# OpenMendel/MendelIHT.jl

Measured on NVIDIA B200. Metric: iht_iterations_per_sec, higher is better.
Workload: dtype f64 (sweep: f32 LUT partials per slab of 640 samples (512 without the ternary copy), f64 across slabs; top-k candidates re-scored in f64)

## Files before the change

### mendeliht.jl_b200/csrc/common.cuh

```cuda
#pragma once
#include <cuda_runtime.h>
#include <stdint.h>
#include <stdio.h>
#include <memory>
#include <string>
#include <vector>
#include <stdexcept>
#include "../../include/ihtb200.h"

namespace ihtb {

struct Error : std::runtime_error {
    int code;
    Error(int c, const std::string& m) : std::runtime_error(m), code(c) {}
};
void set_last_error(const std::string& m);
const std::string& last_error();
struct LaunchCounter {
    int64_t v = 0;
    LaunchCounter& operator++(int) { __atomic_fetch_add(&v, 1, __ATOMIC_RELAXED); return *this; }
    operator int64_t() const { return __atomic_load_n(&v, __ATOMIC_RELAXED); }
};
LaunchCounter& launch_counter();
bool debug_sync();

#define IHTB_CUDA(call)                                                                      \
    do {                                                                                     \
        cudaError_t e__ = (call);                                                            \
        if (e__ != cudaSuccess)                                                              \
            throw ::ihtb::Error(IHTB_ECUDA, std::string(#call) + ": " + cudaGetErrorString(e__)); \
    } while (0)

#define IHTB_CHECK(cond, code, msg)                                  \
    do {                                                             \
        if (!(cond)) throw ::ihtb::Error((code), (msg));             \
    } while (0)

#define IHTB_LAUNCH(kernel, grid, block, smem, stream, ...)          \
    do {                                                             \
        kernel<<<(grid), (block), (smem), (stream)>>>(__VA_ARGS__);  \
        ::ihtb::launch_counter()++;                                  \
        IHTB_CUDA(cudaGetLastError());                               \
        if (::ihtb::debug_sync()) {                                  \
            cudaError_t e2__ = cudaStreamSynchronize(stream);        \
            if (e2__ != cudaSuccess)                                 \
                throw ::ihtb::Error(IHTB_ECUDA, std::string("kernel " #kernel " failed: ") + cudaGetErrorString(e2__)); \
        }                                                            \
    } while (0)

template <typename F>
static inline int32_t guard(F&& f) {
    try {
        f();
        return IHTB_OK;
    } catch (const Error& e) {
        set_last_error(e.what());
        return e.code;
    } catch (const std::bad_alloc&) {
        set_last_error("out of host memory");
        return IHTB_ENOMEM;
    } catch (const std::exception& e) {
        set_last_error(e.what());
        return IHTB_EINVAL;
    }
}

template <typename T>
struct DBuf {
    T* p = nullptr;
    size_t n = 0;
    DBuf() = default;
    explicit DBuf(size_t count) { alloc(count); }
    DBuf(const DBuf&) = delete;
    DBuf& operator=(const DBuf&) = delete;
    ~DBuf() { release(); }
    void alloc(size_t count) {
        release();
        n = count;
        if (count) {
            cudaError_t e = cudaMalloc((void**)&p, count * sizeof(T));
            if (e != cudaSuccess) {
                p = nullptr; n = 0;
                throw Error(IHTB_ENOMEM, std::string("cudaMalloc of ") + std::to_string(count * sizeof(T)) +
                                             " bytes failed: " + cudaGetErrorString(e));
            }
        }
    }
    void release() {
        if (p) cudaFree(p);
        p = nullptr; n = 0;
    }
    void zero(cudaStream_t s) { if (n) IHTB_CUDA(cudaMemsetAsync(p, 0, n * sizeof(T), s)); }
};

template <typename T>
struct HBuf {
    T* p = nullptr;
    size_t n = 0;
    HBuf() = default;
    HBuf(const HBuf&) = delete;
    HBuf& operator=(const HBuf&) = delete;
    ~HBuf() { if (p) cudaFreeHost(p); }
    void alloc(size_t count) {
        if (p) cudaFreeHost(p);
        p = nullptr; n = count;
        if (count) IHTB_CUDA(cudaMallocHost((void**)&p, count * sizeof(T)));
    }
};

static inline int64_t ceil_div(int64_t a, int64_t b) { return (a + b - 1) / b; }

bool smem_attr_needed(const void* kernel, int device);
template <typename K>
static inline void ensure_dynamic_smem(K kernel, int bytes) {
    int dev = 0;
    IHTB_CUDA(cudaGetDevice(&dev));
    if (!smem_attr_needed(reinterpret_cast<const void*>(kernel), dev)) return;
    IHTB_CUDA(cudaFuncSetAttribute(kernel, cudaFuncAttributeMaxDynamicSharedMemorySize, bytes));
}

struct TopkFuse;
ihtb_geno* dense_new_handle(int64_t n, int64_t p, int dtype, int standardize, int32_t den = 0);
void dense_upload(ihtb_geno* g, const void* x, int64_t ld_host, int64_t j_dst, int64_t ncols);
void dense_finalize(ihtb_geno* g);
int64_t dense_stream_bytes(const ihtb_geno* g);
void dense_decode_block(const ihtb_geno* g, int64_t i0, int64_t i1, int64_t j0, int64_t j1, double* d_out);
void dense_xt_v(const ihtb_geno* g, const double* dV, int64_t m, double* dOut, cudaStream_t s, DBuf<double>* part,
                const TopkFuse* tf);
void dense_sweep_kernel_only(const ihtb_geno* g, const double* dV, DBuf<double>* part, cudaStream_t s);
void dense_x_support(const ihtb_geno* g, const int64_t* d_idx, int64_t k, const double* d_coef, int64_t m,
                     double* d_out, cudaStream_t s);
void dense_xt_gather2(const ihtb_geno* g, const int64_t* d_cols_a, int64_t n_a, const int64_t* d_cols_b, int64_t n_b,
                      const double* d_v, int64_t m, double* d_out, cudaStream_t s);
void dense_init_beta_moments(const ihtb_geno* g, const double* d_w, const double* d_wy, double* d_sx, double* d_sxx,
                             double* d_sxy, cudaStream_t s);
void dense_decode_cols(const ihtb_geno* g, const int64_t* d_cols, int64_t k, double* d_out, cudaStream_t s);
const double* geno_bound_scale(const ihtb_geno* g);
double geno_bound_coef(const ihtb_geno* g, double plink_coef);

}

enum { GENO_PLINK = 0, GENO_DENSE = 1 };

struct ihtb_geno {
    int kind = 0;
    int device = 0;
    int64_t n = 0;
    int64_t p = 0;
    int64_t j0 = 0;
    int64_t nbytes = 0;
    int64_t stride = 0;
    int64_t cs_j = 0, cs_s = 0;
    int quad = 0;
    int64_t p4 = 0;
    int center = 1, scale = 1, impute = 1;
    int sm_count = 148;
    ihtb::DBuf<uint8_t> bed;
    ihtb::DBuf<uint8_t> tern;
    int64_t tern_slabs = 0;
    ihtb::DBuf<double> mu, sinv;
    ihtb::DBuf<double> sgn;
    ihtb::DBuf<int32_t> nmiss;
    ihtb::DBuf<int64_t> miss_ptr;
    ihtb::DBuf<int32_t> miss_idx;
    int64_t total_missing = 0;
    bool ready = false;
    int dtype = 0;
    int standardize = 0;
    int32_t den = 0;
    int64_t ld = 0;
    ihtb::DBuf<uint8_t> dense;
    ihtb::DBuf<double> dscale;
    double dcoef = 0.0;
    std::shared_ptr<void> bgen_stage;
};
static inline bool geno_is_dense(const ihtb_geno* g) { return g->kind == GENO_DENSE; }

static inline void geno_require_ready(const ihtb_geno* g) {
    IHTB_CHECK(g && g->ready, IHTB_EINVAL, "genotype handle is not finalized (ihtb_geno_finalize)");
}

struct GenoView {
    const uint8_t* bed;
    int64_t cs_j, cs_s, nbytes, stride, n, p;
    int quad;
    const double* mu;
    const double* sinv;
    const int32_t* nmiss;
    int impute;
};
static inline GenoView geno_view(const ihtb_geno* g) {
    return GenoView{g->bed.p, g->cs_j, g->cs_s, g->nbytes, g->stride, g->n, g->p, g->quad, g->mu.p, g->sinv.p,
                    g->nmiss.p, g->impute};
}
__device__ __forceinline__ const uint8_t* gv_ptr(const GenoView& g, int64_t j, int64_t b) {
    if (g.quad)
        return g.bed + (b >> 7) * g.cs_s + (j >> 2) * 512 + ((b & 127) >> 2) * 16 + (j & 3) * 4 + (b & 3);
    return g.bed + j * g.cs_j + (b >> 7) * g.cs_s + (b & 127);
}

namespace ihtb {

__device__ __forceinline__ double warp_sum(double v) {
#pragma unroll
    for (int o = 16; o > 0; o >>= 1) v += __shfl_xor_sync(0xffffffffu, v, o);
    return v;
}
__device__ __forceinline__ float warp_sum(float v) {
#pragma unroll
    for (int o = 16; o > 0; o >>= 1) v += __shfl_xor_sync(0xffffffffu, v, o);
    return v;
}
__device__ __forceinline__ int warp_sum(int v) {
#pragma unroll
    for (int o = 16; o > 0; o >>= 1) v += __shfl_xor_sync(0xffffffffu, v, o);
    return v;
}

__device__ __forceinline__ double block_sum(double v, double* sh) {
    v = warp_sum(v);
    int lane = threadIdx.x & 31, w = threadIdx.x >> 5;
    __syncthreads();
    if (lane == 0) sh[w] = v;
    __syncthreads();
    int nw = (blockDim.x + 31) >> 5;
    v = (threadIdx.x < nw) ? sh[threadIdx.x] : 0.0;
    if (w == 0) v = warp_sum(v);
    return v;
}

void sweep_xt_v(const ihtb_geno* g, const double* dV, int64_t m, double* dOut, int mode, cudaStream_t s,
                double* sweep_seconds);
void x_support(const ihtb_geno* g, const int64_t* d_idx_local, int64_t k, const double* d_coef, int64_t m,
               double* d_out, cudaStream_t s);
void xt_gather(const ihtb_geno* g, const int64_t* d_cols_local, int64_t ncols, const double* d_v, int64_t m,
               const double* d_vsum , double* d_out , cudaStream_t s);
void xt_gather2(const ihtb_geno* g, const int64_t* d_cols_a, int64_t n_a, const int64_t* d_cols_b, int64_t n_b,
                const double* d_v, int64_t m, const double* d_vsum, double* d_out, cudaStream_t s, bool blocked = false);

struct TopkFuse;
void dense_xt_v(const ihtb_geno* g, const double* dV, int64_t m, double* dOut, cudaStream_t s, void* scratch_any,
                const TopkFuse* tf);
void dense_x_support(const ihtb_geno* g, const int64_t* d_idx, int64_t k, const double* d_coef, int64_t m,
                     double* d_out, cudaStream_t s);
void dense_xt_gather2(const ihtb_geno* g, const int64_t* d_cols_a, int64_t n_a, const int64_t* d_cols_b, int64_t n_b,
                      const double* d_v, int64_t m, double* d_out, cudaStream_t s);
void dense_init_beta_moments(const ihtb_geno* g, const double* d_w, const double* d_wy, double* d_sx, double* d_sxx,
                             double* d_sxy, cudaStream_t s, void* scratch_any);
void dense_decode_cols(const ihtb_geno* g, const int64_t* d_cols, int64_t k, double* d_out, cudaStream_t s);
const double* geno_bound_scale(const ihtb_geno* g);
double geno_bound_coef(const ihtb_geno* g, double plink_coef);

}
```

### mendeliht.jl_b200/csrc/fit.cu

```cuda
#include "glm.cuh"
#include "topk.cuh"
#include "comm.cuh"
#include "debias.cuh"
#include "groups.cuh"
#include "pairer.cuh"
#include <algorithm>
#include <chrono>
#include <cmath>
#include <memory>
#include <mutex>
#include <string.h>
#include <unordered_map>

namespace ihtb {
void sweep_xt_v_with_means(const ihtb_geno* g, const double* dV, const double* vbar_host, int64_t m, double* dOut,
                           int mode, cudaStream_t s, void* scratch_any, float* sweep_ms, double* d_l2 = nullptr,
                           const TopkFuse* tf = nullptr);
void* sweep_scratch_create();
void sweep_scratch_destroy(void* p);
void sweep_class_sums(const ihtb_geno* g, const double* d_v, double* d_w1, double* d_w2, double* d_wm, cudaStream_t s,
                      void* scratch_any);
}

using namespace ihtb;

static const double kFastBound = 1.0 / 262144.0;
static const double kExactBound = 1e-13;
static const double kPairBound = 3.1 / 2048.0;

struct ihtb_fit {
    const ihtb_geno* g = nullptr;
    int device = 0;
    int64_t n = 0, p = 0, q = 0;
    ihtb_comm* comm = nullptr;
    int64_t j0 = 0, p_global = 0;
    std::vector<int64_t> shard_j0;
    DBuf<int64_t> d_selall, d_pack, d_packall;
    HBuf<int64_t> h_selall, h_packall;
    int capx = 512;
    ihtb_cfg cfg{};
    cudaStream_t s = nullptr;
    std::vector<uint8_t> zkeep;
    int zkeepn = 0;
    int cap = 4096;

    DBuf<unsigned> d_done;
    DBuf<double> d_y, d_z, d_w, d_xb, d_zc, d_mu, d_r, d_xs, d_dfa, d_part, d_scal, d_small, d_coef, d_gout,
        d_vbar;
    DBuf<uint8_t> d_mask;
    DBuf<uint32_t> d_keyL, d_keyU;
    DBuf<int> d_hist;
    DBuf<int64_t> d_sel;
    DBuf<int64_t> d_idx, d_cols;
    HBuf<double> h_scal, h_gout;
    HBuf<int64_t> h_sel;
    void* sweep_scratch = nullptr;
    cudaEvent_t ev0 = nullptr, ev1 = nullptr, tm0 = nullptr, tm1 = nullptr;
    bool sweep_pending = false;
    struct FusedStep {
        std::vector<int64_t> uni_loc;
        size_t maxsupp = 0;
        int M = 0;
        int winner = -1;
    };
    FusedStep* fz = nullptr;
    DBuf<double> d_pick;
    HBuf<double> h_pick;
    SweepPairer* pairer = nullptr;
    int pair_slot = 0;
    double sweep_coef = kFastBound;
    GlmCtx glm{};
    TopkCtx tk{};

    std::vector<int64_t> idx, idx0, best_idx;
    std::vector<double> b, b0, best_b;
    std::vector<double> c, c0, best_c, df2, h_y, h_mu;
    std::vector<uint8_t> idc, idc0;
    std::unordered_map<int64_t, double> df_exact;
    std::vector<double> wt;
    DBuf<double> d_wt;
    double w_at(int64_t j) const { return wt.empty() ? 1.0 : wt[(size_t)j]; }
    void set_weights(const double* w) {
        if (!w) { wt.clear(); tk.wt = nullptr; return; }
        for (int64_t j = 0; j < p_global; ++j)
            IHTB_CHECK(w[j] > 0.0 && std::isfinite(w[j]), IHTB_EDOMAIN, "weights must be positive and finite");
        wt.assign(w, w + p_global);
        if (d_wt.n < (size_t)p) d_wt.alloc((size_t)p);
        IHTB_CUDA(cudaMemcpyAsync(d_wt.p, wt.data() + j0, (size_t)p * sizeof(double), cudaMemcpyHostToDevice, s));
        sync();
        tk.wt = d_wt.p;
    }
    std::vector<int64_t> cand_cache;
    bool df_sparse = false;
    std::vector<int64_t> dfs_idx;
    std::vector<double> dfs_val;
    double rbar = 0.0, bound = 0.0, sum_w = 0.0, sum_wy = 0.0, last_dev = 0.0, denom_next = 0.0;
    bool denom_ready = false;
    bool inited = false;

    int64_t n_sweeps = 0, n_backtracks = 0, n_cand_iter = 0, n_pair_overflow = 0;
    int last_count = 0;
    double sweep_ms_total = 0.0;
    double pve = 0.0;

    ~ihtb_fit() {
        if (sweep_scratch) sweep_scratch_destroy(sweep_scratch);
        if (ev0) cudaEventDestroy(ev0);
        if (ev1) cudaEventDestroy(ev1);
        if (tm0) cudaEventDestroy(tm0);
        if (tm1) cudaEventDestroy(tm1);
        if (s) cudaStreamDestroy(s);
    }

    void sync() { IHTB_CUDA(cudaStreamSynchronize(s)); }
    void readback_scal(int nv) {
        IHTB_CUDA(cudaMemcpyAsync(h_scal.p, d_scal.p, nv * sizeof(double), cudaMemcpyDeviceToHost, s));
        sync();
    }
    template <typename T>
    void upload(T* dst, const T* src, size_t count) {
        if (count) IHTB_CUDA(cudaMemcpyAsync(dst, src, count * sizeof(T), cudaMemcpyHostToDevice, s));
    }

    bool is_local(int64_t j) const { return j >= j0 && j < j0 + p; }
    int nranks() const { return comm ? comm->nranks : 1; }

    void support_matvec(const std::vector<int64_t>& cols, const std::vector<double>& coef, double* d_out) {
        std::vector<int64_t> ii; std::vector<double> vv;
        for (size_t t = 0; t < cols.size(); ++t)
            if (coef[t] != 0.0 && is_local(cols[t])) { ii.push_back(cols[t] - j0); vv.push_back(coef[t]); }
        if (!ii.empty()) {
            upload(d_idx.p, ii.data(), ii.size());
            upload(d_coef.p, vv.data(), vv.size());
        }
        support_matvec_dev(ii.empty() ? nullptr : d_idx.p, (int64_t)ii.size(), d_coef.p, d_out);
    }

    void support_matvec_dev(const int64_t* d_idx_loc, int64_t k_loc, const double* d_coef_loc, double* d_out) {
        support_matvec_dev_m(d_idx_loc, k_loc, d_coef_loc, 1, d_out);
    }
    void support_matvec_dev_m(const int64_t* d_idx_loc, int64_t k_loc, const double* d_coef_loc, int m, double* d_out) {
        const size_t cnt = (size_t)n * (size_t)m;
        if (!comm) {
            if (k_loc > 0) x_support(g, d_idx_loc, k_loc, d_coef_loc, m, d_out, s);
            else IHTB_CUDA(cudaMemsetAsync(d_out, 0, cnt * sizeof(double), s));
            return;
        }
        if (m == 1 && p2p_pushall_ok(comm, cnt)) {
            if (k_loc > 0) x_support_push(g, d_idx_loc, k_loc, d_coef_loc, comm, s);
            else p2p_push(comm, nullptr, cnt, s);
            p2p_reduce(comm, d_out, cnt, s);
            return;
        }
        if (p2p_mapped(comm) && cnt <= comm->red_cap) {
            double* part = p2p_partial_ptr(comm);
            if (k_loc > 0) x_support(g, d_idx_loc, k_loc, d_coef_loc, m, part, s);
            else IHTB_CUDA(cudaMemsetAsync(part, 0, cnt * sizeof(double), s));
            p2p_allreduce_2phase(comm, cnt, d_out, s);
            return;
        }
        if (k_loc > 0) x_support(g, d_idx_loc, k_loc, d_coef_loc, m, d_out, s);
        else IHTB_CUDA(cudaMemsetAsync(d_out, 0, cnt * sizeof(double), s));
        comm_allreduce_sum_f64(comm, d_out, cnt, s);
    }

    void update_xb() { support_matvec(idx, b, d_xb.p); }

    double glm_update(int add_zc) {
        upload(d_small.p, c.data(), (size_t)q);
        glm_mu(glm, d_small.p, add_zc, s);
        readback_scal(3);
        double dev = h_scal.p[0], lp = h_scal.p[1], sw = h_scal.p[2];
        last_dev = dev;
        if (cfg.dist == IHTB_NORMAL) {
            double phi = dev / (double)n;
            double sigma = std::sqrt(phi);
            return -0.5 * (dev / phi) - sw * (0.5 * std::log(2.0 * M_PI) + std::log(sigma));
        }
        return lp;
    }

    static double digamma(double x) {
        double r = 0.0;
        while (x < 6.0) { r -= 1.0 / x; x += 1.0; }
        double f = 1.0 / (x * x);
        return r + std::log(x) - 0.5 / x -
               f * (1.0 / 12 - f * (1.0 / 120 - f * (1.0 / 252 - f * (1.0 / 240 - f * (1.0 / 132)))));
    }
    static double trigamma(double x) {
        double r = 0.0;
        while (x < 6.0) { r += 1.0 / (x * x); x += 1.0; }
        double f = 1.0 / (x * x);
        return r + 1.0 / x + f / 2 + f / x * (1.0 / 6 - f * (1.0 / 30 - f * (1.0 / 42 - f * (1.0 / 30))));
    }
    void fetch_mu() {
        h_mu.resize((size_t)n);
        IHTB_CUDA(cudaMemcpyAsync(h_mu.data(), d_mu.p, n * sizeof(double), cudaMemcpyDeviceToHost, s));
        sync();
    }
    double nb_logl(double r) {
        glm.nb_r = r;
        return glm_update(1);
    }
    void mle_for_r() {
        fetch_mu();
        const std::vector<double>& y = h_y;
        double r = glm.nb_r;
        if (cfg.est_r == 1) {
            double num = 0.0, den = 0.0;
            for (int64_t i = 0; i < n; ++i) {
                for (int64_t j = 0; j <= (int64_t)y[i] - 1; ++j) num += r / (r + (double)j);
                den += std::log(r / (r + h_mu[i]));
            }
            glm.nb_r = -num / den;
            return;
        }
        auto d1 = [&](double rr) {
            double a = 0.0;
            for (int64_t i = 0; i < n; ++i)
                a += -(y[i] + rr) / (h_mu[i] + rr) - std::log(h_mu[i] + rr) + 1.0 + std::log(rr) + digamma(rr + y[i]) -
                     digamma(rr);
            return a;
        };
        auto d2 = [&](double rr) {
            double a = 0.0;
            for (int64_t i = 0; i < n; ++i)
                a += (y[i] + rr) / ((h_mu[i] + rr) * (h_mu[i] + rr)) - 2.0 / (h_mu[i] + rr) + 1.0 / rr +
                     trigamma(rr + y[i]) - trigamma(rr);
            return a;
        };
        double new_r = 1.0, stepsize = 1.0;
        for (int it = 0; it < 100; ++it) {
            double dx = d1(r), dx2 = d2(r);
            double increment = dx2 < 0 ? dx / dx2 : dx;
            new_r = r - stepsize * increment;
            double old_logl = nb_logl(r);
            for (int j = 0; j < 20; ++j) {
                if (new_r <= 0) {
                    stepsize /= 2; new_r = r - stepsize * increment;
                } else {
                    double new_logl = nb_logl(new_r);
                    if (old_logl >= new_logl) { stepsize /= 2; new_r = r - stepsize * increment; }
                    else break;
                }
            }
            if (std::fabs(r - new_r) <= 1e-6) { glm.nb_r = new_r; return; }
            r = new_r;
        }
        glm.nb_r = r;
    }
    double mu_r_logl() {
        double l = glm_update(1);
        if (cfg.est_r != 0) {
            mle_for_r();
            l = glm_update(1);
        }
        return l;
    }

    void exact_df(const std::vector<int64_t>& cols, bool exchange = true) {
        std::vector<int64_t> need;
        for (int64_t j : cols)
            if (!df_exact.count(j) && (exchange || is_local(j))) need.push_back(j);
        if (need.empty()) { if (!exchange) sync(); return; }
        IHTB_CHECK((int64_t)need.size() <= (int64_t)d_cols.n, IHTB_ENUMERIC, "too many columns to re-score");
        std::vector<int64_t> loc(need.size());
        for (size_t t = 0; t < need.size(); ++t) loc[t] = is_local(need[t]) ? need[t] - j0 : -1;
        upload(d_cols.p, loc.data(), loc.size());
        xt_gather2(g, d_cols.p, (int64_t)need.size(), nullptr, 0, d_r.p, 1, d_vbar.p, d_gout.p, s,
                   false);
        if (exchange) comm_allreduce_sum_f64(comm, d_gout.p, need.size(), s);
        IHTB_CUDA(cudaMemcpyAsync(h_gout.p, d_gout.p, need.size() * sizeof(double), cudaMemcpyDeviceToHost, s));
        sync();
        for (size_t t = 0; t < need.size(); ++t) df_exact[need[t]] = h_gout.p[t];
        n_cand_iter += (int64_t)need.size();
    }

    void score_and_sweep() {
        glm_score(glm, s, d_vbar.p);
        IHTB_CUDA(cudaMemcpyAsync(h_scal.p, d_scal.p, (2 + q) * sizeof(double), cudaMemcpyDeviceToHost, s));
        IHTB_CUDA(cudaEventRecord(ev0, s));
        sweep_coef = geno_bound_coef(g, cfg.sweep_mode == IHTB_SWEEP_FAST ? kFastBound : kExactBound);
        const double t_sw = now();
        if (pairer && cfg.sweep_mode == IHTB_SWEEP_FAST) {
            IHTB_CHECK(!grouped() && !comm, IHTB_EUNSUPPORTED, "paired sweeps serve plain single-device fits only");
            if (pairer->sweep(pair_slot, g, d_r.p, d_vbar.p, d_dfa.p, s, sweep_scratch)) {
                sweep_coef = kPairBound;
                IHTB_CUDA(cudaMemcpyAsync(h_scal.p + 3 + q, pairer->d_l2 + pair_slot, sizeof(double), cudaMemcpyDeviceToHost, s));
            }
        } else if (cfg.k > 0 && !(grouped() && !init_plain)) {
            const TopkFuse tf = topk_absdf_fuse_begin(tk, geno_bound_scale(g), d_scal.p, sweep_coef);
            sweep_xt_v_with_means(g, d_r.p, d_vbar.p, 1, d_dfa.p, cfg.sweep_mode, s, sweep_scratch, nullptr, nullptr, &tf);
        } else {
            sweep_xt_v_with_means(g, d_r.p, d_vbar.p, 1, d_dfa.p, cfg.sweep_mode, s, sweep_scratch, nullptr);
        }
        IHTB_CUDA(cudaEventRecord(ev1, s));
        ++n_sweeps;
        const double t_sel = now();
        dbg[0] += t_sel - t_sw;
        select_rescore(false);
        dbg[1] += now() - t_sel;
    }

    void select_rescore(bool rerun) {
        if (grouped() && !init_plain) {
            select_groups(rerun);
            if (!rerun) finish_sweep_scalars(sweep_coef);
            return;
        }
        df_exact.clear(); cand_cache.clear();
        df_sparse = false;
        const double coef = sweep_coef;
        std::vector<std::pair<int64_t, double>> cvals;
        const bool fused = fz != nullptr && !rerun;
        std::vector<int64_t> supp_loc;
        if (fused) supp_loc = fz->uni_loc;
        else
            for (int64_t j : idx)
                if (is_local(j)) supp_loc.push_back(j - j0);
        const int nsupp = (int)supp_loc.size();
        const int64_t* d_supp = fused ? d_idx.p : d_cols.p;
        int glaunch = 0;
        if (cfg.k > 0) {
            const int64_t ksel = cfg.k + (int64_t)(fused ? fz->maxsupp : idx.size());
            const bool paired = coef == kPairBound;
            if (tk.fused_hist) topk_candidates_absdf_finish(tk, ksel, s);
            else
                topk_candidates_absdf(tk, d_dfa.p, paired ? g->sgn.p : geno_bound_scale(g), rerun ? nullptr : d_scal.p, coef, ksel, s,
                                      bound, (paired && !rerun) ? pairer->d_l2 + pair_slot : nullptr);
            const int64_t want = sweep_coef == kPairBound ? std::max<int64_t>(ksel + 1024, last_count + last_count / 4 + 256)
                                                          : ksel + 64;
            glaunch = (int)std::min<int64_t>(comm ? capx / 2 : cap, want);
        }
        if (nsupp && !fused) upload(d_cols.p, supp_loc.data(), supp_loc.size());
        xt_gather2(g, tk.cand, glaunch, d_supp, nsupp, d_r.p, 1, d_vbar.p, d_gout.p, s);
        denom_ready = false;
        if (!rerun) {
            if (fused) {
                glm_winner_coef(d_pick.p, d_coefM.p, nsupp, d_gout.p + glaunch, d_coef.p, d_cM.p, q, d_small.p + q, s);
                support_matvec_dev(d_supp, nsupp, d_coef.p, d_xs.p);
                IHTB_CUDA(cudaMemcpyAsync(h_pick.p, d_pick.p, (size_t)(1 + fz->M) * sizeof(double), cudaMemcpyDeviceToHost, s));
                IHTB_CUDA(cudaMemcpyAsync(h_scalM.p, d_scalM.p, (size_t)(3 * fz->M) * sizeof(double), cudaMemcpyDeviceToHost, s));
            } else {
                support_matvec_dev(d_supp, nsupp, d_gout.p + glaunch, d_xs.p);
                std::vector<double> mask((size_t)q);
                for (int64_t l = 0; l < q; ++l) mask[l] = idc[l] ? 1.0 : 0.0;
                upload(d_small.p + q, mask.data(), (size_t)q);
            }
            glm_stepsize(glm, d_scal.p + 2, d_xs.p, s, d_small.p + q, d_scal.p + 2 + q);
            IHTB_CUDA(cudaMemcpyAsync(h_scal.p + 2 + q, d_scal.p + 2 + q, sizeof(double), cudaMemcpyDeviceToHost, s));
            denom_ready = true;
        }
        if (!comm) {
            IHTB_CUDA(cudaMemcpyAsync(h_sel.p, d_sel.p, (2 + glaunch) * sizeof(int64_t), cudaMemcpyDeviceToHost, s));
            IHTB_CUDA(cudaMemcpyAsync(h_gout.p, d_gout.p, (glaunch + nsupp) * sizeof(double), cudaMemcpyDeviceToHost, s));
            sync();
            const double t_host = now();
            struct Acc { double& a; double t0; ~Acc() { a += now() - t0; } } acc_host{dbg[2], t_host};
            if (fused) adopt_winner();
            const TopkState* st = reinterpret_cast<const TopkState*>(h_sel.p);
            const int count = cfg.k > 0 ? st->count : 0;
            dbg[3] += (double)std::min(count, glaunch);
            if (count > cap && coef == kPairBound && !rerun) {
                ++n_pair_overflow;
                sweep_coef = kFastBound;
                sweep_xt_v_with_means(g, d_r.p, d_vbar.p, 1, d_dfa.p, IHTB_SWEEP_FAST, s, sweep_scratch, nullptr);
                IHTB_CUDA(cudaEventRecord(ev1, s));
                select_rescore(false);
                return;
            }
            IHTB_CHECK(count <= cap, IHTB_ENUMERIC,
                       "degenerate projection: more than " + std::to_string(cap) +
                           " entries lie within the sweep error bound of the k-th largest |gradient|");
            last_count = count;
            cvals.reserve((size_t)count);
            for (int t = 0; t < std::min(count, glaunch); ++t) cvals.push_back({h_sel.p[2 + t], h_gout.p[t]});
            for (int t = 0; t < nsupp; ++t) df_exact[supp_loc[t] + j0] = h_gout.p[glaunch + t];
            if (count > glaunch) {
                IHTB_CUDA(cudaMemcpyAsync(h_sel.p, d_sel.p, (2 + count) * sizeof(int64_t), cudaMemcpyDeviceToHost, s));
                sync();
                std::vector<int64_t> rest(h_sel.p + 2 + glaunch, h_sel.p + 2 + count);
                exact_df(rest);
                for (int64_t j : rest) cvals.push_back({j, df_exact.at(j)});
            }
        } else {
            const int nr = nranks();
            const size_t blk = 2 + 2 * (size_t)capx;
            IHTB_CHECK(nsupp <= capx / 2, IHTB_ENUMERIC, "support too large for the sharded candidate exchange");
            pack_sweep_candidates(d_pack.p, reinterpret_cast<const TopkState*>(d_sel.p), tk.cand, glaunch, d_gout.p,
                                  d_supp, nsupp, d_gout.p + glaunch, j0, capx, s);
            comm_allgather_i64(comm, d_pack.p, d_packall.p, blk, s);
            IHTB_CUDA(cudaMemcpyAsync(h_packall.p, d_packall.p, nr * blk * sizeof(int64_t), cudaMemcpyDeviceToHost, s));
            sync();
            if (fused) adopt_winner();
            for (int r = 0; r < nr; ++r) {
                const int64_t* b_ = h_packall.p + (size_t)r * blk;
                IHTB_CHECK(b_[0] <= glaunch, IHTB_ENUMERIC,
                           "degenerate projection: too many local candidates within the sweep error bound");
                const int half = capx / 2;
                auto take = [&](int t, bool is_cand) {
                    const int64_t j = b_[2 + t];
                    if (j < 0) return;
                    double v;
                    memcpy(&v, &b_[2 + capx + t], sizeof(double));
                    if (is_cand) cvals.push_back({j, v});
                    else df_exact[j] = v;
                };
                for (int t = 0; t < (int)b_[0]; ++t) take(t, true);
                for (int t = 0; t < (int)b_[1]; ++t) take(half + t, false);
            }
        }
        std::sort(cvals.begin(), cvals.end());
        cvals.erase(std::unique(cvals.begin(), cvals.end(), [](const std::pair<int64_t, double>& x, const std::pair<int64_t, double>& y) {
                        return x.first == y.first; }), cvals.end());
        n_cand_iter += (int64_t)cvals.size();
        std::vector<char> keep(cvals.size(), 1);
        if ((int64_t)cvals.size() > cfg.k) {
            std::vector<std::pair<double, size_t>> outside;
            outside.reserve(cvals.size());
            for (size_t t = 0; t < cvals.size(); ++t)
                if (!std::binary_search(idx.begin(), idx.end(), cvals[t].first))
                    outside.push_back({std::fabs(cvals[t].second) * w_at(cvals[t].first), t});
            if ((int64_t)outside.size() > cfg.k) {
                std::nth_element(outside.begin(), outside.begin() + (cfg.k - 1), outside.end(),
                                 [](const std::pair<double, size_t>& x, const std::pair<double, size_t>& y) {
                                     return x.first > y.first;
                                 });
                const double thr = outside[(size_t)cfg.k - 1].first * (1.0 - 1e-12);
                std::fill(keep.begin(), keep.end(), 0);
                for (const auto& e : outside)
                    if (e.first >= thr) keep[e.second] = 1;
            }
        }
        for (size_t t = 0; t < cvals.size(); ++t)
            if (keep[t]) {
                cand_cache.push_back(cvals[t].first);
                df_exact[cvals[t].first] = cvals[t].second;
            }
        if (rerun) return;
        finish_sweep_scalars(coef);
    }

    void finish_sweep_scalars(double coef) {
        float ms = 0.f;
        IHTB_CUDA(cudaEventElapsedTime(&ms, ev0, ev1));
        sweep_ms_total += ms;
        double rsum = h_scal.p[0], rl1 = h_scal.p[1];
        for (int64_t l = 0; l < q; ++l) df2[l] = h_scal.p[2 + l];
        denom_next = h_scal.p[2 + q];
        rbar = rsum / (double)n;
        bound = coef == kPairBound ? coef * h_scal.p[3 + q]
                                   : coef * (rl1 + std::fabs(rsum));
    }

    double df_at(int64_t j) const {
        if (df_sparse) {
            auto it = std::lower_bound(dfs_idx.begin(), dfs_idx.end(), j);
            return (it != dfs_idx.end() && *it == j) ? dfs_val[it - dfs_idx.begin()] : 0.0;
        }
        return df_exact.at(j);
    }

    double stepsize() {
        std::vector<double> coef(idx.size());
        double numer = 0.0;
        for (size_t t = 0; t < idx.size(); ++t) { coef[t] = df_at(idx[t]); numer += coef[t] * coef[t]; }
        if (denom_ready && !df_sparse) {
            denom_ready = false;
            for (int64_t l = 0; l < q; ++l)
                if (idc[l]) numer += df2[l] * df2[l];
            double eta = numer / denom_next;
            if (std::isinf(eta) || std::isnan(eta)) eta = 1e-8;
            return eta;
        }
        denom_ready = false;
        support_matvec(idx, coef, d_xs.p);
        std::vector<double> d2((size_t)q);
        for (int64_t l = 0; l < q; ++l) {
            d2[l] = idc[l] ? df2[l] : 0.0;
            if (idc[l]) numer += df2[l] * df2[l];
        }
        upload(d_small.p + q, d2.data(), (size_t)q);
        glm_stepsize(glm, d_small.p + q, d_xs.p, s);
        readback_scal(1);
        double denom = h_scal.p[0];
        double eta = numer / denom;
        if (std::isinf(eta) || std::isnan(eta)) eta = 1e-8;
        return eta;
    }

    static double b_lookup(const std::vector<int64_t>& ii, const std::vector<double>& vv, int64_t j) {
        auto it = std::lower_bound(ii.begin(), ii.end(), j);
        return (it != ii.end() && *it == j) ? vv[it - ii.begin()] : 0.0;
    }

    void gradstep(double eta) {
        if (grouped()) { gradstep_group(eta); return; }
        std::vector<int64_t> cand;
        cand = df_sparse ? dfs_idx : cand_cache;
        cand.insert(cand.end(), idx0.begin(), idx0.end());
        std::sort(cand.begin(), cand.end());
        cand.erase(std::unique(cand.begin(), cand.end()), cand.end());

        struct Item { double a; int64_t pos; double v; };
        std::vector<Item> items;
        items.reserve(cand.size() + (size_t)q);
        for (int64_t j : cand) {
            double v = b_lookup(idx0, b0, j) + eta * df_at(j);
            if (!wt.empty()) {
                const double w = wt[(size_t)j], a = v * w;
                items.push_back({std::fabs(a), j, a / w});
            } else {
                items.push_back({std::fabs(v), j, v});
            }
        }
        for (int64_t l = 0; l < q; ++l) {
            c[l] = c0[l] + eta * df2[l];
            if (!zkeep[l]) items.push_back({std::fabs(c[l]), p_global + l, c[l]});
        }
        int64_t k = cfg.k;
        std::sort(items.begin(), items.end(), [](const Item& x, const Item& y) {
            return x.a > y.a || (x.a == y.a && x.pos < y.pos);
        });
        idx.clear(); b.clear();
        const double thr = project_threshold(items, k);
        std::vector<std::pair<int64_t, double>> keep;
        for (size_t t = 0; t < items.size(); ++t) {
            const bool kept = items[t].a >= thr;
            if (items[t].pos >= p_global) {
                if (!kept) c[items[t].pos - p_global] = 0.0;
            } else if (kept && items[t].v != 0.0) {
                keep.push_back({items[t].pos, items[t].v});
            }
        }
        for (int64_t l = 0; l < q; ++l) idc[l] = c[l] != 0.0;
        choose_prune(keep);
        std::sort(keep.begin(), keep.end());
        for (auto& kv : keep) { idx.push_back(kv.first); b.push_back(kv.second); }
    }

    template <typename ItemT>
    static double project_threshold(const std::vector<ItemT>& sorted_items, int64_t k) {
        if (k <= 0) return INFINITY;
        return (int64_t)sorted_items.size() >= k ? sorted_items[(size_t)k - 1].a : 0.0;
    }
    void choose_prune(std::vector<std::pair<int64_t, double>>& keep) const {
        int64_t nonzero = (int64_t)keep.size() - zkeepn;
        for (int64_t l = 0; l < q; ++l) nonzero += idc[l] ? 1 : 0;
        const int64_t limit = cfg.k + zkeepn;
        if (nonzero <= limit) return;
        std::vector<std::pair<int64_t, double>> byabs = keep;
        std::sort(byabs.begin(), byabs.end(), [](const std::pair<int64_t, double>& x, const std::pair<int64_t, double>& y) {
            return std::fabs(x.second) < std::fabs(y.second) || (std::fabs(x.second) == std::fabs(y.second) && x.first > y.first);
        });
        const size_t excess = std::min<size_t>((size_t)(nonzero - limit), byabs.size());
        for (size_t t = 0; t < excess; ++t) keep.erase(std::find(keep.begin(), keep.end(), byabs[t]));
    }

    std::unique_ptr<GroupCtx> grpctx;
    bool init_plain = false;
    bool grouped() const { return (bool)grpctx; }
    void set_groups(const int32_t* group1, int J, const int64_t* ks, int64_t n_groups) {
        if (!group1) { grpctx.reset(); return; }
        IHTB_CHECK(J >= 0, IHTB_EINVAL, "Value of J (max number of groups) must be nonnegative!");
        std::unique_ptr<GroupCtx> gc(new GroupCtx());
        std::vector<double> h_sinv((size_t)p);
        IHTB_CUDA(cudaMemcpy(h_sinv.data(), geno_bound_scale(g), (size_t)p * sizeof(double), cudaMemcpyDeviceToHost));
        gc->build(p, j0, p_global, group1, J, ks, n_groups, cfg.k, h_sinv.data());
        grpctx = std::move(gc);
    }

    void select_groups(bool rerun) {
        GroupCtx& gc = *grpctx;
        df_exact.clear(); cand_cache.clear();
        df_sparse = false; denom_ready = false;
        const double coef = sweep_coef;
        group_topk(gc, d_dfa.p, geno_bound_scale(g), rerun ? nullptr : d_scal.p, coef, bound, cfg.k, s);
        const size_t G = (size_t)gc.G, nT = 2 * G + 1;
        const int nr = nranks();
        std::vector<double> TL(G), TU(G);
        bool overflow = false;
        if (comm) {
            if (gc.d_Tall.n < nT * (size_t)nr) { gc.d_Tall.alloc(nT * (size_t)nr); gc.h_Tall.alloc(nT * (size_t)nr); }
            comm_allgather_i64(comm, reinterpret_cast<const int64_t*>(gc.d_gT.p), gc.d_Tall.p, nT, s);
            IHTB_CUDA(cudaMemcpyAsync(gc.h_Tall.p, gc.d_Tall.p, nT * (size_t)nr * sizeof(int64_t), cudaMemcpyDeviceToHost, s));
            sync();
            std::fill(TL.begin(), TL.end(), 0.0); std::fill(TU.begin(), TU.end(), 0.0);
            for (int rk = 0; rk < nr; ++rk) {
                const double* T = reinterpret_cast<const double*>(gc.h_Tall.p) + (size_t)rk * nT;
                for (size_t gi = 0; gi < G; ++gi) { TL[gi] = std::max(TL[gi], T[gi]); TU[gi] += T[G + gi]; }
                overflow = overflow || T[2 * G] != 0.0;
            }
        } else {
            IHTB_CUDA(cudaMemcpyAsync(gc.h_gT.p, gc.d_gT.p, nT * sizeof(double), cudaMemcpyDeviceToHost, s));
            sync();
            for (size_t gi = 0; gi < G; ++gi) { TL[gi] = gc.h_gT.p[gi]; TU[gi] = gc.h_gT.p[G + gi]; }
            overflow = gc.h_gT.p[2 * G] != 0.0;
        }
        IHTB_CHECK(!overflow, IHTB_ENUMERIC,
                   "degenerate group projection: too many entries of one group lie within the sweep error bound of its "
                   "2k-th largest |gradient|");
        std::vector<char> has(G, 0);
        for (int64_t j : idx) has[(size_t)gc.grp[(size_t)j]] = 1;
        std::vector<int32_t> chosen;
        std::vector<double> lows;
        for (size_t gi = 0; gi < G; ++gi) {
            if (has[gi]) chosen.push_back((int32_t)gi);
            else lows.push_back(TL[gi]);
        }
        if (gc.J > 0 && !lows.empty()) {
            const size_t need = std::min<size_t>((size_t)gc.J, lows.size());
            std::nth_element(lows.begin(), lows.begin() + (need - 1), lows.end(), std::greater<double>());
            const double thr = lows[need - 1];
            for (size_t gi = 0; gi < G; ++gi)
                if (!has[gi] && TU[gi] >= thr) chosen.push_back((int32_t)gi);
        }
        IHTB_CHECK(chosen.size() <= 65536, IHTB_ENUMERIC, "degenerate group projection: too many groups tie at the J-th norm");
        std::sort(chosen.begin(), chosen.end());
        const int nc = (int)chosen.size();
        const int64_t nsupp = (int64_t)idx.size();
        const int64_t list_slots = (int64_t)nc * gc.lcap, slots = list_slots + nsupp;
        if (slots == 0) return;
        gc.ensure_chosen(std::max(nc, 1));
        if (gc.d_oidx.n < (size_t)slots) {
            gc.d_oidx.alloc((size_t)slots); gc.d_oval.alloc((size_t)slots);
            gc.h_oidx.alloc((size_t)slots); gc.h_oval.alloc((size_t)slots);
        }
        if (nc) {
            IHTB_CUDA(cudaMemcpyAsync(gc.d_chosen.p, chosen.data(), (size_t)nc * sizeof(int32_t), cudaMemcpyHostToDevice, s));
            group_take(gc, nc, s);
        }
        std::vector<int64_t> supp_loc((size_t)nsupp);
        for (int64_t t = 0; t < nsupp; ++t) supp_loc[(size_t)t] = is_local(idx[(size_t)t]) ? idx[(size_t)t] - j0 : -1;
        upload(gc.d_oidx.p + list_slots, supp_loc.data(), (size_t)nsupp);
        xt_gather(g, gc.d_oidx.p, slots, d_r.p, 1, d_vbar.p, gc.d_oval.p, s);
        auto take = [&](int64_t t, int64_t j, double v) {
            if (j < 0) return;
            df_exact[j] = v;
            if (t < list_slots) cand_cache.push_back(j);
        };
        if (comm) {
            const size_t blk = 2 * (size_t)slots;
            if (gc.d_blk.n < blk) gc.d_blk.alloc(blk);
            if (gc.d_blkall.n < blk * (size_t)nr) { gc.d_blkall.alloc(blk * (size_t)nr); gc.h_blkall.alloc(blk * (size_t)nr); }
            group_pack(gc.d_oidx.p, gc.d_oval.p, slots, j0, gc.d_blk.p, s);
            comm_allgather_i64(comm, gc.d_blk.p, gc.d_blkall.p, blk, s);
            IHTB_CUDA(cudaMemcpyAsync(gc.h_blkall.p, gc.d_blkall.p, blk * (size_t)nr * sizeof(int64_t), cudaMemcpyDeviceToHost, s));
            sync();
            for (int rk = 0; rk < nr; ++rk) {
                const int64_t* b_ = gc.h_blkall.p + (size_t)rk * blk;
                for (int64_t t = 0; t < slots; ++t) {
                    double v;
                    memcpy(&v, &b_[slots + t], sizeof(double));
                    take(t, b_[t], v);
                }
            }
        } else {
            IHTB_CUDA(cudaMemcpyAsync(gc.h_oidx.p, gc.d_oidx.p, (size_t)slots * sizeof(int64_t), cudaMemcpyDeviceToHost, s));
            IHTB_CUDA(cudaMemcpyAsync(gc.h_oval.p, gc.d_oval.p, (size_t)slots * sizeof(double), cudaMemcpyDeviceToHost, s));
            sync();
            for (int64_t t = 0; t < slots; ++t) take(t, gc.h_oidx.p[t], gc.h_oval.p[t]);
        }
        std::sort(cand_cache.begin(), cand_cache.end());
        cand_cache.erase(std::unique(cand_cache.begin(), cand_cache.end()), cand_cache.end());
        n_cand_iter += (int64_t)cand_cache.size();
    }

    struct GItem { double a; int64_t j; double v; int g; };
    std::vector<std::pair<int64_t, double>> project_groups(std::vector<GItem>& items) const {
// ... 846 lines not shown
```

### mendeliht.jl_b200/csrc/lut_common.cuh

```cuda
#pragma once
#include "common.cuh"
#include <cuda_fp16.h>

namespace ihtb {

constexpr int LUT_TABLE_BYTES = 131072;

__device__ __forceinline__ uint32_t smem_u32(const void* p) { return (uint32_t)__cvta_generic_to_shared(p); }
__device__ __forceinline__ void mbar_init(uint32_t bar, uint32_t count) {
    asm volatile("mbarrier.init.shared::cta.b64 [%0], %1;" ::"r"(bar), "r"(count));
}
__device__ __forceinline__ void mbar_arrive(uint32_t bar) {
    asm volatile("mbarrier.arrive.shared::cta.b64 _, [%0];" ::"r"(bar) : "memory");
}
__device__ __forceinline__ void mbar_expect_tx(uint32_t bar, uint32_t bytes) {
    asm volatile("mbarrier.arrive.expect_tx.shared::cta.b64 _, [%0], %1;" ::"r"(bar), "r"(bytes) : "memory");
}
__device__ __forceinline__ void mbar_wait(uint32_t bar, uint32_t parity) {
    asm volatile(
        "{\n\t.reg .pred p;\n"
        "W_%=:\n\t"
        "mbarrier.try_wait.parity.shared::cta.b64 p, [%0], %1;\n\t"
        "@!p bra W_%=;\n\t}"
        ::"r"(bar), "r"(parity) : "memory");
}
__device__ __forceinline__ void bulk_g2s(uint32_t dst, const void* src, uint32_t bytes, uint32_t bar) {
    asm volatile("cp.async.bulk.shared::cluster.global.mbarrier::complete_tx::bytes [%0], [%1], %2, [%3];"
                 ::"r"(dst), "l"(src), "r"(bytes), "r"(bar) : "memory");
}
__device__ __forceinline__ float lds_f32(uint32_t addr) {
    float v;
    asm volatile("ld.shared.f32 %0, [%1];" : "=f"(v) : "r"(addr));
    return v;
}
__device__ __forceinline__ uint32_t lds_u32(uint32_t addr) {
    uint32_t v;
    asm volatile("ld.shared.u32 %0, [%1];" : "=r"(v) : "r"(addr));
    return v;
}
__device__ __forceinline__ uint4 lds_u128(uint32_t addr) {
    uint4 v;
    asm volatile("ld.shared.v4.u32 {%0, %1, %2, %3}, [%4];" : "=r"(v.x), "=r"(v.y), "=r"(v.z), "=r"(v.w) : "r"(addr));
    return v;
}
template <uint32_t SEL>
__device__ __forceinline__ uint32_t prmt(uint32_t a, uint32_t b) {
    uint32_t d;
    asm("prmt.b32 %0, %1, %2, %3;" : "=r"(d) : "r"(a), "r"(b), "n"(SEL));
    return d;
}
__device__ __forceinline__ void sts_u32(uint32_t addr, uint32_t v) {
    asm volatile("st.shared.u32 [%0], %1;" ::"r"(addr), "r"(v) : "memory");
}
__device__ __forceinline__ void sts_f32(uint32_t addr, float v) {
    asm volatile("st.shared.f32 [%0], %1;" ::"r"(addr), "f"(v) : "memory");
}
template <int NT>
__device__ __forceinline__ void consumer_bar() {
    asm volatile("bar.sync 1, %0;" ::"n"(NT) : "memory");
}

template <int NT>
__device__ __forceinline__ void lut_build(uint32_t tab, const double* __restrict__ v, double vbar, int64_t n,
                                          int64_t slab, int tid) {
    constexpr int PARTS = NT / 128;
    constexpr int V3_PER = 4 / PARTS;
    const int group = tid & 127, part = tid >> 7;
    const int t = group >> 5, w = group & 31;
    float u[4];
#pragma unroll
    for (int s = 0; s < 4; ++s) {
        int64_t i = slab * 512 + 16 * w + 4 * t + s;
        u[s] = (i < n) ? __double2float_rn(__dsub_rn(v[i], vbar)) : 0.0f;
    }
    auto f = [&](int s, int code) -> float { return code == 2 ? u[s] : (code == 3 ? u[s] + u[s] : 0.0f); };
    const uint32_t rowbase = tab + (uint32_t)(t >> 1) * 65536u + (uint32_t)(t & 1) * 128u + 4u * (uint32_t)w;
#pragma unroll
    for (int c3 = 0; c3 < V3_PER; ++c3) {
        const int v3 = part * V3_PER + c3;
        const float a3 = (v3 == 2) ? u[3] : ((v3 == 3) ? u[3] + u[3] : 0.0f);
        const uint32_t base3 = rowbase + (uint32_t)v3 * (64u * 256u);
#pragma unroll
        for (int v2 = 0; v2 < 4; ++v2) {
            const float a2 = a3 + f(2, v2);
#pragma unroll
            for (int v1 = 0; v1 < 4; ++v1) {
                const float a1 = a2 + f(1, v1);
#pragma unroll
                for (int v0 = 0; v0 < 4; ++v0)
                    sts_f32(base3 + (uint32_t)(v2 << 4 | v1 << 2 | v0) * 256u, a1 + f(0, v0));
            }
        }
    }
}

template <int NT>
__device__ __forceinline__ void lut_build_tern(uint32_t tab, const double* __restrict__ v, double vbar, int64_t n,
                                               int64_t slab, int tid) {
    static_assert(NT == 512, "ternary tables are built by 512 threads");
    const int group = tid & 127, d4 = tid >> 7;
    if (d4 > 2) return;
    const int t = group >> 5, w = group & 31;
    float u[5];
#pragma unroll
    for (int s = 0; s < 5; ++s) {
        int64_t i = slab * 640 + 20 * w + 5 * t + s;
        u[s] = (i < n) ? __double2float_rn(__dsub_rn(v[i], vbar)) : 0.0f;
    }
    auto f = [&](int s, int d) -> float { return d == 1 ? u[s] : (d == 2 ? u[s] + u[s] : 0.0f); };
    const uint32_t rowbase = tab + (uint32_t)(t >> 1) * 65536u + (uint32_t)(t & 1) * 128u + 4u * (uint32_t)w;
    const float a4 = (d4 == 1) ? u[4] : ((d4 == 2) ? u[4] + u[4] : 0.0f);
    const uint32_t base4 = rowbase + (uint32_t)d4 * (81u * 256u);
#pragma unroll
    for (int d3 = 0; d3 < 3; ++d3) {
        const float a3 = a4 + f(3, d3);
#pragma unroll
        for (int d2 = 0; d2 < 3; ++d2) {
            const float a2 = a3 + f(2, d2);
#pragma unroll
            for (int d1 = 0; d1 < 3; ++d1) {
                const float a1 = a2 + f(1, d1);
#pragma unroll
                for (int d0 = 0; d0 < 3; ++d0)
                    sts_f32(base4 + (uint32_t)(27 * d3 + 9 * d2 + 3 * d1 + d0) * 256u, a1 + f(0, d0));
            }
        }
    }
}

__device__ __forceinline__ void lut_build_h2_tern(uint32_t tab, const double* __restrict__ v0, const double* __restrict__ v1,
                                                  double vbar0, double vbar1, float sc0, float sc1, int64_t n, int64_t slab,
                                                  int tid) {
    const int group = tid & 127, d4 = tid >> 7;
    if (d4 > 2) return;
    const int t = group >> 5, w = group & 31;
    float a[5], b[5];
#pragma unroll
    for (int s = 0; s < 5; ++s) {
        int64_t i = slab * 640 + 20 * w + 5 * t + s;
        const float x0 = (i < n) ? __double2float_rn(__dsub_rn(v0[i], vbar0)) * sc0 : 0.0f;
        const float x1 = (i < n) ? __double2float_rn(__dsub_rn(v1[i], vbar1)) * sc1 : 0.0f;
        a[s] = (w & 16) ? x1 : x0;
        b[s] = (w & 16) ? x0 : x1;
    }
    auto fa = [&](int s, int d) -> float { return d == 1 ? a[s] : (d == 2 ? a[s] + a[s] : 0.0f); };
    auto fb = [&](int s, int d) -> float { return d == 1 ? b[s] : (d == 2 ? b[s] + b[s] : 0.0f); };
    const uint32_t rowbase = tab + (uint32_t)(t >> 1) * 65536u + (uint32_t)(t & 1) * 128u + 4u * (uint32_t)w;
    const float a4 = fa(4, d4), b4 = fb(4, d4);
    const uint32_t base4 = rowbase + (uint32_t)d4 * (81u * 256u);
#pragma unroll
    for (int d3 = 0; d3 < 3; ++d3) {
        const float a3 = a4 + fa(3, d3), b3 = b4 + fb(3, d3);
#pragma unroll
        for (int d2 = 0; d2 < 3; ++d2) {
            const float a2 = a3 + fa(2, d2), b2 = b3 + fb(2, d2);
#pragma unroll
            for (int d1 = 0; d1 < 3; ++d1) {
                const float a1 = a2 + fa(1, d1), b1 = b2 + fb(1, d1);
#pragma unroll
                for (int d0 = 0; d0 < 3; ++d0) {
                    const __half2 h = __floats2half2_rn(a1 + fa(0, d0), b1 + fb(0, d0));
                    sts_u32(base4 + (uint32_t)(27 * d3 + 9 * d2 + 3 * d1 + d0) * 256u, *reinterpret_cast<const uint32_t*>(&h));
                }
            }
        }
    }
}

__device__ __forceinline__ void lut_build_h2(uint32_t tab, const double* __restrict__ v0, const double* __restrict__ v1,
                                             double vbar0, double vbar1, float sc0, float sc1, int64_t n, int64_t slab,
                                             int tid) {
    const int group = tid & 127, part = tid >> 7;
    const int t = group >> 5, w = group & 31;
    float a[4], b[4];
#pragma unroll
    for (int s = 0; s < 4; ++s) {
        int64_t i = slab * 512 + 16 * w + 4 * t + s;
        a[s] = (i < n) ? __double2float_rn(__dsub_rn(v0[i], vbar0)) * sc0 : 0.0f;
        b[s] = (i < n) ? __double2float_rn(__dsub_rn(v1[i], vbar1)) * sc1 : 0.0f;
    }
    auto fa = [&](int s, int code) -> float { return code == 2 ? a[s] : (code == 3 ? a[s] + a[s] : 0.0f); };
    auto fb = [&](int s, int code) -> float { return code == 2 ? b[s] : (code == 3 ? b[s] + b[s] : 0.0f); };
    const uint32_t rowbase = tab + (uint32_t)(t >> 1) * 65536u + (uint32_t)(t & 1) * 128u + 4u * (uint32_t)w;
    const int v3 = part;
    const float a3 = fa(3, v3), b3 = fb(3, v3);
    const uint32_t base3 = rowbase + (uint32_t)v3 * (64u * 256u);
#pragma unroll
    for (int v2 = 0; v2 < 4; ++v2) {
        const float a2 = a3 + fa(2, v2), b2 = b3 + fb(2, v2);
#pragma unroll
        for (int v1c = 0; v1c < 4; ++v1c) {
            const float a1 = a2 + fa(1, v1c), b1 = b2 + fb(1, v1c);
#pragma unroll
            for (int v0c = 0; v0c < 4; ++v0c) {
                const __half2 h = __floats2half2_rn(a1 + fa(0, v0c), b1 + fb(0, v0c));
                sts_u32(base3 + (uint32_t)(v2 << 4 | v1c << 2 | v0c) * 256u, *reinterpret_cast<const uint32_t*>(&h));
            }
        }
    }
}

}
```

### mendeliht.jl_b200/csrc/mvfit.cu

```cuda
#include "glm.cuh"
#include "topk.cuh"
#include "comm.cuh"
#include <algorithm>
#include <chrono>
#include <cmath>
#include <map>
#include <memory>

namespace ihtb {
void sweep_xt_v_with_means(const ihtb_geno* g, const double* dV, const double* vbar_host, int64_t m, double* dOut,
                           int mode, cudaStream_t s, void* scratch_any, float* sweep_ms, double* d_l2 = nullptr,
                           const TopkFuse* tf = nullptr);
void* sweep_scratch_create();
void sweep_scratch_destroy(void* p);
void sweep_class_sums(const ihtb_geno* g, const double* d_v, double* d_w1, double* d_w2, double* d_wm, cudaStream_t s,
                      void* scratch_any);

constexpr int MV_MAXR = 20;
constexpr int MV_THREADS = 256;
static inline int mv_grid(int64_t n) {
    int64_t b = ceil_div(n, MV_THREADS);
    return (int)(b < 1 ? 1 : (b > GLM_MAX_BLOCKS ? GLM_MAX_BLOCKS : b));
}
struct MvSmall { double a[MV_MAXR * MV_MAXR]; };

__global__ void __launch_bounds__(MV_THREADS)
k_mv_resid_gram(int64_t n, int r, int64_t q, const double* __restrict__ BX, const double* __restrict__ Z,
                const double* __restrict__ C , const double* __restrict__ Y,
                const double* __restrict__ w, double* __restrict__ mu, double* __restrict__ resid,
                double* __restrict__ part) {
    __shared__ double sh[32];
    double g[MV_MAXR * (MV_MAXR + 1) / 2];
    const int ng = r * (r + 1) / 2;
    for (int e = 0; e < ng; ++e) g[e] = 0.0;
    double sw = 0.0;
    for (int64_t i = blockIdx.x * (int64_t)blockDim.x + threadIdx.x; i < n; i += (int64_t)gridDim.x * blockDim.x) {
        double rs[MV_MAXR];
        const double wi = w[i];
        for (int t = 0; t < r; ++t) {
            double cz = 0.0;
            for (int64_t l = 0; l < q; ++l) cz += C[t * q + l] * Z[i + l * n];
            double m = BX[i + (int64_t)t * n] + cz;
            mu[i + (int64_t)t * n] = m;
            rs[t] = (Y[i + (int64_t)t * n] - m) * wi;
            resid[i + (int64_t)t * n] = rs[t];
        }
        int e = 0;
        for (int a = 0; a < r; ++a)
            for (int b = a; b < r; ++b) g[e++] += rs[a] * rs[b];
        sw += wi;
    }
    const int nv = ng + 1;
    for (int e = 0; e < ng; ++e) {
        double v = block_sum(g[e], sh);
        if (threadIdx.x == 0) part[blockIdx.x * nv + e] = v;
    }
    double v = block_sum(sw, sh);
    if (threadIdx.x == 0) part[blockIdx.x * nv + ng] = v;
}

__global__ void __launch_bounds__(MV_THREADS)
k_mv_score(int64_t n, int r, int64_t q, const double* __restrict__ resid, MvSmall G, const double* __restrict__ Z,
           double* __restrict__ R1, double* __restrict__ part) {
    __shared__ double sh[32];
    double s1[MV_MAXR], sa[MV_MAXR];
    for (int t = 0; t < r; ++t) { s1[t] = 0.0; sa[t] = 0.0; }
    for (int64_t i = blockIdx.x * (int64_t)blockDim.x + threadIdx.x; i < n; i += (int64_t)gridDim.x * blockDim.x) {
        double rs[MV_MAXR];
        for (int t = 0; t < r; ++t) rs[t] = resid[i + (int64_t)t * n];
        for (int t = 0; t < r; ++t) {
            double v = 0.0;
            for (int u = 0; u < r; ++u) v += G.a[t * r + u] * rs[u];
            R1[i + (int64_t)t * n] = v;
            s1[t] += v; sa[t] += fabs(v);
        }
    }
    const int nv = 2 * r + r * (int)q;
    for (int t = 0; t < r; ++t) {
        double v = block_sum(s1[t], sh);
        if (threadIdx.x == 0) part[blockIdx.x * nv + t] = v;
        v = block_sum(sa[t], sh);
        if (threadIdx.x == 0) part[blockIdx.x * nv + r + t] = v;
    }
    for (int t = 0; t < r; ++t)
        for (int64_t l = 0; l < q; ++l) {
            double a = 0.0;
            for (int64_t i = blockIdx.x * (int64_t)blockDim.x + threadIdx.x; i < n; i += (int64_t)gridDim.x * blockDim.x)
                a += R1[i + (int64_t)t * n] * Z[i + l * n];
            a = block_sum(a, sh);
            if (threadIdx.x == 0) part[blockIdx.x * nv + 2 * r + t * (int)q + (int)l] = a;
        }
}

__global__ void __launch_bounds__(MV_THREADS)
k_mv_stepsize(int64_t n, int r, const double* __restrict__ V, const double* __restrict__ w, MvSmall U,
              double* __restrict__ part) {
    __shared__ double sh[32];
    double a = 0.0;
    for (int64_t i = blockIdx.x * (int64_t)blockDim.x + threadIdx.x; i < n; i += (int64_t)gridDim.x * blockDim.x) {
        double v[MV_MAXR];
        const double wi = w[i];
        for (int t = 0; t < r; ++t) v[t] = V[i + (int64_t)t * n] * wi;
        for (int t = 0; t < r; ++t) {
            double s = 0.0;
            for (int u = 0; u < r; ++u) s += U.a[t * r + u] * v[u];
            a += s * s;
        }
    }
    a = block_sum(a, sh);
    if (threadIdx.x == 0) part[blockIdx.x] = a;
}

__global__ void __launch_bounds__(MV_THREADS)
k_mv_moments(int64_t n, int r, const double* __restrict__ mu, const double* __restrict__ Y, MvSmall means, int pass,
             double* __restrict__ part) {
    __shared__ double sh[32];
    for (int t = 0; t < r; ++t) {
        double a = 0.0, b = 0.0;
        for (int64_t i = blockIdx.x * (int64_t)blockDim.x + threadIdx.x; i < n; i += (int64_t)gridDim.x * blockDim.x) {
            double m = mu[i + (int64_t)t * n], y = Y[i + (int64_t)t * n];
            if (pass == 0) { a += m; b += y; }
            else { double dm = m - means.a[t], dy = y - means.a[r + t]; a += dm * dm; b += dy * dy; }
        }
        a = block_sum(a, sh); b = block_sum(b, sh);
        if (threadIdx.x == 0) { part[blockIdx.x * 2 * r + t] = a; part[blockIdx.x * 2 * r + r + t] = b; }
    }
}

__global__ void k_mv_finalize(const double* __restrict__ part, int nblocks, int nv, double* __restrict__ out) {
    int v = (blockIdx.x * blockDim.x + threadIdx.x) >> 5;
    int lane = threadIdx.x & 31;
    if (v >= nv) return;
    double a = 0.0;
    for (int b = lane; b < nblocks; b += 32) a += part[b * nv + v];
    a = warp_sum(a);
    if (lane == 0) out[v] = a;
}
__global__ void k_mv_means(const double* __restrict__ scal, int r, int64_t n, double* __restrict__ out) {
    int t = threadIdx.x;
    if (t < r) out[t] = scal[t] / (double)n;
}
__global__ void k_mv_weights(int64_t n, const uint8_t* __restrict__ mask, double* __restrict__ w) {
    int64_t i = blockIdx.x * (int64_t)blockDim.x + threadIdx.x;
    if (i < n) w[i] = (mask == nullptr || mask[i]) ? 1.0 : 0.0;
}

static bool chol_lower(int r, const double* a, double* l) {
    std::fill(l, l + r * r, 0.0);
    for (int j = 0; j < r; ++j) {
        double d = a[j * r + j];
        for (int k = 0; k < j; ++k) d -= l[j * r + k] * l[j * r + k];
        if (!(d > 0.0)) return false;
        l[j * r + j] = std::sqrt(d);
        for (int i = j + 1; i < r; ++i) {
            double s = a[i * r + j];
            for (int k = 0; k < j; ++k) s -= l[i * r + k] * l[j * r + k];
            l[i * r + j] = s / l[j * r + j];
        }
    }
    return true;
}
static void spd_inverse(int r, const double* l, double* inv) {
    std::vector<double> li((size_t)r * r, 0.0);
    for (int i = 0; i < r; ++i) {
        li[i * r + i] = 1.0 / l[i * r + i];
        for (int j = 0; j < i; ++j) {
            double s = 0.0;
            for (int k = j; k < i; ++k) s -= l[i * r + k] * li[k * r + j];
            li[i * r + j] = s / l[i * r + i];
        }
    }
    for (int i = 0; i < r; ++i)
        for (int j = 0; j < r; ++j) {
            double s = 0.0;
            for (int k = std::max(i, j); k < r; ++k) s += li[k * r + i] * li[k * r + j];
            inv[i * r + j] = s;
        }
}
static bool pivoted_chol_upper(int r, const double* a_in, double* u) {
    std::vector<double> s(a_in, a_in + r * r);
    for (int i = 0; i < r; ++i)
        for (int j = 0; j < i; ++j) s[i * r + j] = s[j * r + i];
    std::fill(u, u + r * r, 0.0);
    for (int j = 0; j < r; ++j) {
        int pvt = j;
        for (int i = j + 1; i < r; ++i)
            if (s[i * r + i] > s[pvt * r + pvt]) pvt = i;
        if (pvt != j) {
            for (int c = 0; c < r; ++c) std::swap(s[j * r + c], s[pvt * r + c]);
            for (int c = 0; c < r; ++c) std::swap(s[c * r + j], s[c * r + pvt]);
            for (int c = 0; c < r; ++c) std::swap(u[c * r + j], u[c * r + pvt]);
        }
        double ajj = s[j * r + j];
        if (!(ajj > 0.0)) return false;
        ajj = std::sqrt(ajj);
        u[j * r + j] = ajj;
        for (int c = j + 1; c < r; ++c) u[j * r + c] = s[j * r + c] / ajj;
        for (int a = j + 1; a < r; ++a)
            for (int b = j + 1; b < r; ++b) s[a * r + b] -= u[j * r + a] * u[j * r + b];
    }
    return true;
}

}

using namespace ihtb;

static const double kFastBoundMv = 1.0 / 262144.0;
static const double kExactBoundMv = 1e-13;
static const double kPairBoundMv = 3.1 / 2048.0;
static const double kFastL2BoundMv = 1.0 / 1048576.0;

struct ihtb_mvfit {
    const ihtb_geno* g = nullptr;
    int device = 0;
    int64_t n = 0, p = 0, q = 0;
    int r = 0;
    ihtb_comm* comm = nullptr;
    int64_t j0 = 0, p_global = 0;
    DBuf<int64_t> d_xch, d_xchall;
    HBuf<int64_t> h_xchall;
    bool is_local(int64_t j) const { return j >= j0 && j < j0 + p; }
    ihtb_cfg cfg{};
    cudaStream_t s = nullptr;
    int cap = 4096;
    DBuf<double> d_Y, d_Z, d_w, d_BX, d_mu, d_resid, d_R1, d_V, d_dfa, d_b0d, d_part, d_scal, d_C, d_coef, d_gout,
        d_vbar, d_sval, d_bounds, d_sinvrep;
    DBuf<uint8_t> d_mask;
    DBuf<uint32_t> d_keyL, d_keyU;
    DBuf<int> d_hist;
    DBuf<int64_t> d_sel, d_idx, d_cols, d_sidx;
    HBuf<double> h_scal, h_gout, h_l2;
    DBuf<double> d_l2;
    HBuf<int64_t> h_sel;
    void* sweep_scratch = nullptr;
    cudaEvent_t ev0 = nullptr, ev1 = nullptr;
    TopkCtx tk{};

    std::map<int64_t, double> B, B0, bestB;
    std::vector<double> C, C0, bestC, df2;
    std::vector<double> Gamma, Gamma0;
    std::map<int64_t, std::vector<double>> df_exact;
    std::map<int64_t, double> dfs;
    bool df_sparse = false, inited = false;
    std::vector<double> bounds;
    std::vector<int64_t> b0d_pos;
    double n_train = 0.0;
    std::vector<double> pve;
    int64_t n_sweeps = 0, n_backtracks = 0, n_cand_iter = 0;
    double sweep_ms_total = 0.0;

    ~ihtb_mvfit() {
        if (sweep_scratch) sweep_scratch_destroy(sweep_scratch);
        if (ev0) cudaEventDestroy(ev0);
        if (ev1) cudaEventDestroy(ev1);
        if (s) cudaStreamDestroy(s);
    }
    void sync() { IHTB_CUDA(cudaStreamSynchronize(s)); }
    template <typename T>
    void upload(T* dst, const T* src, size_t count) {
        if (count) IHTB_CUDA(cudaMemcpyAsync(dst, src, count * sizeof(T), cudaMemcpyHostToDevice, s));
    }
    void finalize(int grid, int nv) {
        IHTB_LAUNCH(k_mv_finalize, (unsigned)ceil_div(nv, 4), 128, 0, s, d_part.p, grid, nv, d_scal.p);
    }
    void readback(int nv) {
        IHTB_CUDA(cudaMemcpyAsync(h_scal.p, d_scal.p, nv * sizeof(double), cudaMemcpyDeviceToHost, s));
        sync();
    }
    double phase_s[8] = {0, 0, 0, 0, 0, 0, 0, 0};
    template <typename F>
    auto timed(int ph, F&& fn) {
        auto t0 = std::chrono::steady_clock::now();
        struct Stop {
            double& acc; std::chrono::steady_clock::time_point t0;
            ~Stop() { acc += std::chrono::duration<double>(std::chrono::steady_clock::now() - t0).count(); }
        } stop{phase_s[ph], t0};
        return fn();
    }
    static std::vector<int64_t> support_cols(const std::map<int64_t, double>& M, int r) {
        std::vector<int64_t> cols;
        for (auto& kv : M)
            if (kv.second != 0.0 && (cols.empty() || cols.back() != kv.first / r)) cols.push_back(kv.first / r);
        return cols;
    }
    MvSmall small(const std::vector<double>& m) const {
        MvSmall o;
        std::fill(o.a, o.a + MV_MAXR * MV_MAXR, 0.0);
        std::copy(m.begin(), m.end(), o.a);
        return o;
    }

    void support_matmat(const std::vector<int64_t>& cols, const std::vector<double>& coef ,
                        double* d_out) {
        std::vector<int64_t> loc; std::vector<size_t> src;
        for (size_t c = 0; c < cols.size(); ++c)
            if (is_local(cols[c])) { loc.push_back(cols[c] - j0); src.push_back(c); }
        if (loc.empty()) {
            IHTB_CUDA(cudaMemsetAsync(d_out, 0, n * r * sizeof(double), s));
        } else {
            std::vector<double> cl(loc.size() * (size_t)r);
            for (int t = 0; t < r; ++t)
                for (size_t c = 0; c < loc.size(); ++c) cl[c + (size_t)t * loc.size()] = coef[src[c] + (size_t)t * cols.size()];
            upload(d_idx.p, loc.data(), loc.size());
            upload(d_coef.p, cl.data(), cl.size());
            x_support(g, d_idx.p, (int64_t)loc.size(), d_coef.p, r, d_out, s);
        }
        if (comm) comm_allreduce_sum_f64(comm, d_out, (size_t)(n * r), s);
    }
    void update_xb() {
        std::vector<int64_t> cols = support_cols(B, r);
        std::vector<double> coef(cols.size() * r, 0.0);
        for (size_t c = 0; c < cols.size(); ++c)
            for (int t = 0; t < r; ++t) {
                auto it = B.find(cols[c] * r + t);
                if (it != B.end()) coef[c + (size_t)t * cols.size()] = it->second;
            }
        support_matmat(cols, coef, d_BX.p);
    }
    std::vector<double> resid_gram() {
        upload(d_C.p, C.data(), C.size());
        int grid = mv_grid(n);
        int ng = r * (r + 1) / 2;
        IHTB_LAUNCH(k_mv_resid_gram, grid, MV_THREADS, 0, s, n, r, q, d_BX.p, d_Z.p, d_C.p, d_Y.p, d_w.p, d_mu.p,
                    d_resid.p, d_part.p);
        finalize(grid, ng + 1);
        readback(ng + 1);
        std::vector<double> G((size_t)r * r);
        int e = 0;
        for (int a = 0; a < r; ++a)
            for (int b = a; b < r; ++b) { G[a * r + b] = h_scal.p[e]; G[b * r + a] = h_scal.p[e]; ++e; }
        n_train = h_scal.p[ng];
        return G;
    }
    double solve_sigma_and_logl() {
        std::vector<double> G = resid_gram();
        std::vector<double> S((size_t)r * r), L((size_t)r * r);
        for (int e = 0; e < r * r; ++e) S[e] = G[e] / n_train;
        if (!chol_lower(r, S.data(), L.data())) return NAN;
        spd_inverse(r, L.data(), Gamma.data());
        double logdet = 0.0;
        for (int i = 0; i < r; ++i) logdet -= 2.0 * std::log(L[i * r + i]);
        double tr = 0.0;
        for (int i = 0; i < r; ++i)
            for (int j = 0; j < r; ++j) tr += Gamma[i * r + j] * G[j * r + i];
        return n_train / 2.0 * logdet - 0.5 * tr;
    }
    void exact_df(const std::vector<int64_t>& cols) {
        std::vector<int64_t> need;
        for (int64_t j : cols)
            if (!df_exact.count(j)) need.push_back(j);
        if (need.empty()) return;
        IHTB_CHECK(need.size() * r <= d_gout.n && need.size() <= d_cols.n, IHTB_ENUMERIC, "too many columns to re-score");
        std::vector<int64_t> loc(need.size());
        for (size_t c = 0; c < need.size(); ++c) loc[c] = is_local(need[c]) ? need[c] - j0 : -1;
        upload(d_cols.p, loc.data(), loc.size());
        xt_gather(g, d_cols.p, (int64_t)need.size(), d_R1.p, r, d_vbar.p, d_gout.p, s);
        if (comm) comm_allreduce_sum_f64(comm, d_gout.p, need.size() * (size_t)r, s);
        IHTB_CUDA(cudaMemcpyAsync(h_gout.p, d_gout.p, need.size() * r * sizeof(double), cudaMemcpyDeviceToHost, s));
        sync();
        for (size_t c = 0; c < need.size(); ++c) {
            std::vector<double> v((size_t)r);
            for (int t = 0; t < r; ++t) v[t] = h_gout.p[c + (size_t)t * need.size()];
            df_exact[need[c]] = v;
        }
        n_cand_iter += (int64_t)need.size();
    }
    void score_and_sweep() {
        int grid = mv_grid(n);
        int nv = 2 * r + r * (int)q;
        IHTB_LAUNCH(k_mv_score, grid, MV_THREADS, 0, s, n, r, q, d_resid.p, small(Gamma), d_Z.p, d_R1.p, d_part.p);
        finalize(grid, nv);
        IHTB_LAUNCH(k_mv_means, 1, 32, 0, s, d_scal.p, r, n, d_vbar.p);
        IHTB_CUDA(cudaMemcpyAsync(h_scal.p, d_scal.p, nv * sizeof(double), cudaMemcpyDeviceToHost, s));
        IHTB_CUDA(cudaEventRecord(ev0, s));
        const bool l2mode = cfg.sweep_mode == IHTB_SWEEP_PAIR && g->cs_j == 128;
        if (l2mode && d_l2.n < (size_t)r) { d_l2.alloc((size_t)r); h_l2.alloc((size_t)r); }
        sweep_xt_v_with_means(g, d_R1.p, d_vbar.p, r, d_dfa.p, cfg.sweep_mode, s, sweep_scratch, nullptr,
                              l2mode ? d_l2.p : nullptr);
        IHTB_CUDA(cudaEventRecord(ev1, s));
        if (l2mode) IHTB_CUDA(cudaMemcpyAsync(h_l2.p, d_l2.p, (size_t)r * sizeof(double), cudaMemcpyDeviceToHost, s));
        n_sweeps += r;
        df_exact.clear();
        df_sparse = false;
        std::vector<int64_t> cols = support_cols(B, r);
        if (!cols.empty()) exact_df(cols); else sync();
        float ms = 0.f;
        IHTB_CUDA(cudaEventElapsedTime(&ms, ev0, ev1));
        sweep_ms_total += ms;
        for (int t = 0; t < r; ++t) {
            double mean = h_scal.p[t] / (double)n;
            double ul1 = h_scal.p[r + t] + (double)n * std::fabs(mean);
            if (l2mode) bounds[t] = (t < 2 * (r / 2) ? kPairBoundMv : kFastL2BoundMv) * h_l2.p[t];
            else bounds[t] = (cfg.sweep_mode == IHTB_SWEEP_EXACT ? kExactBoundMv : kFastBoundMv) * ul1;
        }
        for (int e = 0; e < r * (int)q; ++e) df2[e] = h_scal.p[2 * r + e];
    }
    double df_entry(int64_t pos) const {
        if (df_sparse) {
            auto it = dfs.find(pos);
            return it == dfs.end() ? 0.0 : it->second;
        }
        return df_exact.at(pos / r)[pos % r];
    }
    double stepsize() {
        std::vector<int64_t> cols = support_cols(B, r);
        if (df_sparse) cols = support_cols(dfs, r);
        std::vector<double> coef(cols.size() * r, 0.0);
        double numer = 0.0;
        for (size_t c = 0; c < cols.size(); ++c)
            for (int t = 0; t < r; ++t) {
                double v = df_entry(cols[c] * r + t);
                coef[c + (size_t)t * cols.size()] = v;
                numer += v * v;
            }
        support_matmat(cols, coef, d_V.p);
        std::vector<double> U((size_t)r * r);
        IHTB_CHECK(pivoted_chol_upper(r, Gamma.data(), U.data()), IHTB_ENUMERIC,
                   "RankDeficientException in the pivoted Cholesky of the precision matrix");
        Gamma = U;
        int grid = mv_grid(n);
        IHTB_LAUNCH(k_mv_stepsize, grid, MV_THREADS, 0, s, n, r, d_V.p, d_w.p, small(U), d_part.p);
        finalize(grid, 1);
        readback(1);
        double eta = numer / h_scal.p[0];
        if (std::isinf(eta) || std::isnan(eta)) eta = 1e-8;
        return eta;
    }
    void sync_b0d() {
        if (!b0d_pos.empty()) {
            upload(d_sidx.p, b0d_pos.data(), b0d_pos.size());
            scatter_dense(d_b0d.p, d_sidx.p, nullptr, (int64_t)b0d_pos.size(), 1, s);
        }
        b0d_pos.clear();
        std::vector<double> vals;
        for (auto& kv : B0)
            if (kv.second != 0.0 && is_local(kv.first / r)) {
                b0d_pos.push_back((kv.first % r) * p + (kv.first / r - j0));
                vals.push_back(kv.second);
            }
        if (!b0d_pos.empty()) {
            upload(d_sidx.p, b0d_pos.data(), b0d_pos.size());
            upload(d_sval.p, vals.data(), vals.size());
            scatter_dense(d_b0d.p, d_sidx.p, d_sval.p, (int64_t)b0d_pos.size(), 0, s);
        }
    }
    std::vector<int64_t> device_candidate_cols(double eta) {
        std::vector<int64_t> cols = timed(5, [&] { return local_candidate_cols(eta); });
        if (!comm) return cols;
        return timed(6, [&] { return exchange_candidate_cols(cols); });
    }
    std::vector<int64_t> local_candidate_cols(double eta) {
        upload(d_bounds.p, bounds.data(), (size_t)r);
        topk_candidates_blocked(tk, d_dfa.p, d_b0d.p,
                                (cfg.sweep_mode == IHTB_SWEEP_PAIR && g->cs_j == 128) ? g->sgn.p : g->sinv.p, p,
                                d_bounds.p, eta, cfg.k, s);
        IHTB_CUDA(cudaMemcpyAsync(h_sel.p, d_sel.p, (2 + cap) * sizeof(int64_t), cudaMemcpyDeviceToHost, s));
        sync();
        const TopkState* st = reinterpret_cast<const TopkState*>(h_sel.p);
        IHTB_CHECK(st->count <= cap, IHTB_ENUMERIC, "degenerate projection: too many entries within the error bound");
        std::vector<int64_t> cols;
        for (int t = 0; t < st->count; ++t) cols.push_back(h_sel.p[2 + t] % p + j0);
        return cols;
    }
    std::vector<int64_t> exchange_candidate_cols(std::vector<int64_t> cols) {
        const size_t blk = 1 + (size_t)cap;
        std::vector<int64_t> mine(blk, -1);
        mine[0] = (int64_t)cols.size();
        std::copy(cols.begin(), cols.end(), mine.begin() + 1);
        upload(d_xch.p, mine.data(), blk);
        comm_allgather_i64(comm, d_xch.p, d_xchall.p, blk, s);
        IHTB_CUDA(cudaMemcpyAsync(h_xchall.p, d_xchall.p, (size_t)comm->nranks * blk * sizeof(int64_t), cudaMemcpyDeviceToHost, s));
        sync();
        cols.clear();
        for (int rk = 0; rk < comm->nranks; ++rk) {
            const int64_t* b_ = h_xchall.p + (size_t)rk * blk;
            cols.insert(cols.end(), b_ + 1, b_ + 1 + b_[0]);
        }
        return cols;
    }
    void gradstep(double eta) {
        std::vector<int64_t> cols;
        if (df_sparse) {
            cols = support_cols(dfs, r);
        } else {
            cols = device_candidate_cols(eta);
        }
        for (auto& kv : B0) cols.push_back(kv.first / r);
        std::sort(cols.begin(), cols.end());
        cols.erase(std::unique(cols.begin(), cols.end()), cols.end());
        if (!df_sparse) timed(7, [&] { exact_df(cols); return 0; });
        struct Item { double a; int64_t pos; double v; };
        std::vector<Item> items;
        for (int64_t j : cols)
            for (int t = 0; t < r; ++t) {
                int64_t pos = j * r + t;
                auto it = B0.find(pos);
                double v = (it == B0.end() ? 0.0 : it->second) + eta * df_entry(pos);
                items.push_back({std::fabs(v), pos, v});
            }
        std::sort(items.begin(), items.end(), [](const Item& x, const Item& y) {
            return x.a > y.a || (x.a == y.a && x.pos < y.pos);
        });
        B.clear();
        for (size_t t = 0; t < items.size() && (int64_t)t < cfg.k; ++t)
            if (items[t].v != 0.0) B[items[t].pos] = items[t].v;
        for (size_t e = 0; e < C.size(); ++e) C[e] = C0[e] + eta * df2[e];
    }
    double save_prev(double cur, double best) {
        B0 = B; C0 = C; Gamma0 = Gamma;
        if (cur > best) { bestB = B; bestC = C; }
        sync_b0d();
        return std::max(cur, best);
    }
    double check_convergence() const {
        double nrm = 0.0, b0max = 0.0;
        for (auto& kv : B) {
            auto it = B0.find(kv.first);
            nrm = std::max(nrm, std::fabs(kv.second - (it == B0.end() ? 0.0 : it->second)));
        }
        for (auto& kv : B0) {
            if (!B.count(kv.first)) nrm = std::max(nrm, std::fabs(kv.second));
            b0max = std::max(b0max, std::fabs(kv.second));
        }
        for (size_t e = 0; e < C.size(); ++e) {
            nrm = std::max(nrm, std::fabs(C[e] - C0[e]));
            b0max = std::max(b0max, std::fabs(C0[e]));
        }
        return nrm / (b0max + 1.0);
    }
    void save_best_model() {
        B = bestB; C = bestC;
        update_xb();
        resid_gram();
    }
    void compute_pve() {
        int grid = mv_grid(n);
        MvSmall means = small(std::vector<double>());
        IHTB_LAUNCH(k_mv_moments, grid, MV_THREADS, 0, s, n, r, d_mu.p, d_Y.p, means, 0, d_part.p);
        finalize(grid, 2 * r);
        readback(2 * r);
        for (int t = 0; t < 2 * r; ++t) means.a[t] = h_scal.p[t] / (double)n;
        IHTB_LAUNCH(k_mv_moments, grid, MV_THREADS, 0, s, n, r, d_mu.p, d_Y.p, means, 1, d_part.p);
        finalize(grid, 2 * r);
        readback(2 * r);
        pve.assign((size_t)r, 0.0);
        for (int t = 0; t < r; ++t) pve[t] = h_scal.p[t] / h_scal.p[r + t];
    }
    void set_weights(const uint8_t* mask) {
        const uint8_t* dm = nullptr;
        if (mask) { upload(d_mask.p, mask, (size_t)n); dm = d_mask.p; }
        IHTB_LAUNCH(k_mv_weights, (unsigned)ceil_div(n, 256), 256, 0, s, n, dm, d_w.p);
    }
    void do_init_beta(const uint8_t* train_mask, const std::vector<double>& sy) {
        DBuf<double> cls((size_t)(6 * p)), bd((size_t)(p * r)), wy((size_t)n);
        double *W1 = cls.p, *W2 = W1 + p, *Wm = W2 + p, *Y1 = Wm + p, *Y2 = Y1 + p, *Ym = Y2 + p;
        sweep_class_sums(g, d_w.p, W1, W2, Wm, s, sweep_scratch);
        ++n_sweeps;
        std::vector<double> c0sum((size_t)r, 0.0);
        for (int t = 0; t < r; ++t) {
            GlmCtx tmp{n, q, d_Z.p, d_Y.p + (size_t)t * n, d_w.p, nullptr, nullptr, nullptr, nullptr, d_part.p, d_scal.p,
                       IHTB_NORMAL, IHTB_LINK_IDENTITY, 1.0};
            init_beta_products(tmp, wy.p, s);
            sweep_class_sums(g, wy.p, Y1, Y2, Ym, s, sweep_scratch);
            ++n_sweeps;
            init_beta_solve(tmp, p, W1, W2, Wm, Y1, Y2, Ym, n_train, sy[(size_t)t], g->mu.p, g->sinv.p, g->impute,
                            bd.p + (size_t)t * p, s);
            readback(1);
            c0sum[(size_t)t] = h_scal.p[0];
        }
        if (comm) {
            upload(d_scal.p, c0sum.data(), (size_t)r);
            comm_allreduce_sum_f64(comm, d_scal.p, (size_t)r, s);
            readback(r);
            std::copy(h_scal.p, h_scal.p + r, c0sum.begin());
        }
        std::fill(C.begin(), C.end(), 0.0);
        if (q > 1) {
            std::vector<double> hY((size_t)(n * r)), hZ((size_t)(n * q));
            IHTB_CUDA(cudaMemcpyAsync(hY.data(), d_Y.p, hY.size() * sizeof(double), cudaMemcpyDeviceToHost, s));
            IHTB_CUDA(cudaMemcpyAsync(hZ.data(), d_Z.p, hZ.size() * sizeof(double), cudaMemcpyDeviceToHost, s));
            sync();
            for (int t = 0; t < r; ++t)
                for (int64_t l = 1; l < q; ++l) {
                    double sx = 0.0, sxx = 0.0, sxy = 0.0;
                    for (int64_t i = 0; i < n; ++i) {
                        if (train_mask && !train_mask[i]) continue;
                        const double z = hZ[(size_t)(i + l * n)];
                        sx += z; sxx += z * z; sxy += z * hY[(size_t)(i + (int64_t)t * n)];
                    }
                    double icpt = sy[(size_t)t], slope = sxy;
                    const double u11 = std::sqrt(n_train), u12 = sx / u11, dd = sxx - u12 * u12;
                    if (n_train > 0 && dd > 0) {
                        const double u22 = std::sqrt(dd), t1 = sy[(size_t)t] / u11, t2 = (sxy - u12 * t1) / u22;
                        slope = t2 / u22; icpt = (t1 - u12 * slope) / u11;
                    }
                    c0sum[(size_t)t] += icpt;
                    C[(size_t)(t * q + l)] = std::min(std::max(slope, -2.0), 2.0);
                }
        }
        for (int t = 0; t < r; ++t)
            C[(size_t)(t * q)] = std::min(std::max(c0sum[(size_t)t] / (double)(p_global + q - 1), -2.0), 2.0);
        std::vector<double> zeros((size_t)r, 0.0);
        upload(d_bounds.p, zeros.data(), zeros.size());
        topk_candidates_blocked(tk, bd.p, nullptr, g->sinv.p, p, d_bounds.p, 1.0, cfg.k, s);
        IHTB_CUDA(cudaMemcpyAsync(h_sel.p, d_sel.p, (2 + cap) * sizeof(int64_t), cudaMemcpyDeviceToHost, s));
        sync();
        const TopkState* st = reinterpret_cast<const TopkState*>(h_sel.p);
        IHTB_CHECK(st->count <= cap && (size_t)st->count <= d_gout.n, IHTB_ENUMERIC,
                   "degenerate projection of the initial beta (too many ties)");
        const int cnt = st->count;
        take_values(bd.p, d_sel.p + 2, cnt, d_gout.p, s);
        IHTB_CUDA(cudaMemcpyAsync(h_gout.p, d_gout.p, (size_t)cnt * sizeof(double), cudaMemcpyDeviceToHost, s));
        sync();
        struct Item { double a; int64_t pos; double v; };
        std::vector<Item> items;
        for (int e = 0; e < cnt; ++e) {
            const int64_t pos_dev = h_sel.p[2 + e], t = pos_dev / p, j = pos_dev % p + j0;
            items.push_back({std::fabs(h_gout.p[e]), j * r + t, h_gout.p[e]});
        }
        if (comm) {
            const size_t blk = 1 + (size_t)cap;
            std::vector<int64_t> pos_blk(blk, -1), val_blk(blk, 0);
            pos_blk[0] = val_blk[0] = (int64_t)items.size();
            for (size_t e = 0; e < items.size(); ++e) {
                pos_blk[1 + e] = items[e].pos;
                memcpy(&val_blk[1 + e], &items[e].v, sizeof(double));
            }
            std::vector<int64_t> all_pos((size_t)comm->nranks * blk);
            for (int pass = 0; pass < 2; ++pass) {
                upload(d_xch.p, (pass == 0 ? pos_blk : val_blk).data(), blk);
                comm_allgather_i64(comm, d_xch.p, d_xchall.p, blk, s);
                IHTB_CUDA(cudaMemcpyAsync(h_xchall.p, d_xchall.p, all_pos.size() * sizeof(int64_t), cudaMemcpyDeviceToHost, s));
                sync();
                if (pass == 0) std::copy(h_xchall.p, h_xchall.p + all_pos.size(), all_pos.begin());
            }
            items.clear();
            for (int rk = 0; rk < comm->nranks; ++rk)
                for (int64_t e = 0; e < all_pos[(size_t)rk * blk]; ++e) {
                    double v;
                    memcpy(&v, &h_xchall.p[(size_t)rk * blk + 1 + (size_t)e], sizeof(double));
                    items.push_back({std::fabs(v), all_pos[(size_t)rk * blk + 1 + (size_t)e], v});
                }
        }
        std::sort(items.begin(), items.end(), [](const Item& x, const Item& y) {
            return x.a > y.a || (x.a == y.a && x.pos < y.pos);
        });
        B.clear();
        for (size_t e = 0; e < items.size() && (int64_t)e < cfg.k; ++e)
            if (items[e].v != 0.0) B[items[e].pos] = items[e].v;
        B0 = B; C0 = C;
        update_xb();
    }

    void init(const uint8_t* train_mask, bool init_beta = false) {
        IHTB_CHECK(cfg.k >= 1, IHTB_EINVAL, "Multivariate IHT requires k >= 1!");
        B.clear(); B0.clear(); bestB.clear(); dfs.clear(); df_exact.clear(); df_sparse = false;
        C.assign((size_t)r * q, 0.0); C0 = C; bestC = C; df2.assign((size_t)r * q, 0.0);
        Gamma.assign((size_t)r * r, 0.0);
        for (int i = 0; i < r; ++i) Gamma[i * r + i] = 1.0;
        Gamma0 = Gamma;
        bounds.assign((size_t)r, 0.0);
        sync_b0d();
        set_weights(train_mask);
        IHTB_CUDA(cudaMemsetAsync(d_BX.p, 0, n * r * sizeof(double), s));
        std::vector<double> G0 = resid_gram();
        int grid = mv_grid(n);
        int nv = 2 * r + r * (int)q;
        IHTB_LAUNCH(k_mv_score, grid, MV_THREADS, 0, s, n, r, q, d_resid.p, small(Gamma), d_Z.p, d_R1.p, d_part.p);
        finalize(grid, nv);
        readback(nv);
        std::vector<double> sy((size_t)r);
        for (int t = 0; t < r; ++t) { sy[(size_t)t] = h_scal.p[t]; C[t * q + 0] = h_scal.p[t] / n_train; }
        resid_gram();
        if (init_beta) {
            do_init_beta(train_mask, sy);
            resid_gram();
        }
        score_and_sweep();
        if (init_beta) { inited = true; return; }
        std::vector<int64_t> cols = device_candidate_cols(1.0);
// ... 213 lines not shown
```

### mendeliht.jl_b200/csrc/pairer.cuh

```cuda
#pragma once
#include "common.cuh"
#include <condition_variable>
#include <mutex>

namespace ihtb {

struct SweepPairer {
    std::mutex mu;
    std::condition_variable cv;
    int active = 2;
    struct Req {
        const double* v; const double* vbar; double* out; cudaStream_t s;
    } req[2] = {};
    bool has[2] = {false, false};
    unsigned long long round = 0;
    cudaEvent_t ready[2] = {nullptr, nullptr};
    cudaEvent_t done = nullptr;
    void* scratch = nullptr;
    double* d_vbar2 = nullptr;
    double* d_l2 = nullptr;
    int64_t n_pair = 0, n_solo = 0;
    int device = 0;

    explicit SweepPairer(int device);
    ~SweepPairer();
    SweepPairer(const SweepPairer&) = delete;
    SweepPairer& operator=(const SweepPairer&) = delete;
    bool sweep(int slot, const ihtb_geno* g, const double* d_v, const double* d_vbar, double* d_out, cudaStream_t s,
               void* solo_scratch);
    void leave();
};

}
```

### mendeliht.jl_b200/csrc/sweep.cu

```cuda
#include "common.cuh"
#include "pairer.cuh"
#include "topk.cuh"
#include <stdlib.h>

namespace ihtb {

void sweep_fast_partials(const ihtb_geno* g, const double* d_v, const double* d_vbar, float* d_part, int64_t* n_slabs,
                         cudaStream_t s);
int64_t sweep_fast_num_slabs(const ihtb_geno* g);
void sweep_exact_lut_partials(const ihtb_geno* g, const double* d_v, const double* d_vbar, double* d_part, cudaStream_t s,
                              int cls = 0);
void sweep_pair_partials(const ihtb_geno* g, const double* d_v0, const double* d_v1, const double* d_vbar,
                         const float* d_scale, float* d_part, cudaStream_t s);

static bool exact_uses_lut(const ihtb_geno* g) {
    static const bool legacy = [] { const char* e = getenv("IHTB_EXACT_LEGACY"); return e && *e == '1'; }();
    return g->cs_j == 128 && !legacy;
}

constexpr int EX_THREADS = 128;
constexpr int EX_CB = 8;
constexpr int EX_COLS_PER_CTA = 512;

__global__ void __launch_bounds__(EX_THREADS)
k_sweep_exact(GenoView gv, const double* __restrict__ v, const double* __restrict__ vbar_p, double* __restrict__ part ) {
    const double vbar = *vbar_p;
    __shared__ double red[EX_THREADS / 32][EX_CB];
    const int64_t p = gv.p, n = gv.n;
    const int64_t words = gv.stride >> 2;
    const int64_t slab = blockIdx.y;
    const int64_t w = slab * EX_THREADS + threadIdx.x;
    const bool live = w < words;
    double u[16];
#pragma unroll
    for (int s = 0; s < 16; ++s) {
        int64_t i = 16 * w + s;
        u[s] = (live && i < n) ? __dsub_rn(v[i], vbar) : 0.0;
    }
    const int64_t jbeg = blockIdx.x * (int64_t)EX_COLS_PER_CTA;
    const int64_t jend = (jbeg + EX_COLS_PER_CTA < p) ? jbeg + EX_COLS_PER_CTA : p;
    const int lane = threadIdx.x & 31, warp = threadIdx.x >> 5;
    for (int64_t j0 = jbeg; j0 < jend; j0 += EX_CB) {
        uint32_t wd[EX_CB];
#pragma unroll
        for (int c = 0; c < EX_CB; ++c) {
            int64_t j = j0 + c;
            wd[c] = (live && j < jend) ? *reinterpret_cast<const uint32_t*>(gv_ptr(gv, j, 4 * w)) : 0u;
        }
        double acc[EX_CB];
#pragma unroll
        for (int c = 0; c < EX_CB; ++c) {
            double a = 0.0;
            uint32_t x = wd[c];
#pragma unroll
            for (int s = 0; s < 16; ++s) {
                uint32_t code = (x >> (2 * s)) & 3u;
                double dos = (code == 2) ? 1.0 : ((code == 3) ? 2.0 : 0.0);
                a = fma(u[s], dos, a);
            }
            acc[c] = warp_sum(a);
        }
        __syncthreads();
        if (lane == 0) {
#pragma unroll
            for (int c = 0; c < EX_CB; ++c) red[warp][c] = acc[c];
        }
        __syncthreads();
        if (threadIdx.x < EX_CB && j0 + threadIdx.x < jend) {
            double t = 0.0;
#pragma unroll
            for (int q = 0; q < EX_THREADS / 32; ++q) t += red[q][threadIdx.x];
            part[slab * p + j0 + threadIdx.x] = t;
        }
    }
}

template <typename T>
__global__ void __launch_bounds__(256)
k_sweep_epilogue(const T* __restrict__ part, int64_t n_slabs, int64_t p,
                 const double* __restrict__ mu, const double* __restrict__ sinv,
                 const int32_t* __restrict__ nmiss, const int64_t* __restrict__ miss_ptr,
                 const int32_t* __restrict__ miss_idx, const double* __restrict__ v,
                 const double* __restrict__ vbar_p,
                 int impute, double* __restrict__ out, const float* __restrict__ scale_p = nullptr,
                 TopkFuse tf = TopkFuse()) {
    __shared__ int sh[TOPK_BINS];
    const bool fuse = tf.keyL != nullptr;
    if (fuse) {
        topk_first_kernel_housekeeping(tf.hist_other, tf.st, tf.cand, tf.cand_fill);
        for (int b = threadIdx.x; b < TOPK_BINS; b += blockDim.x) sh[b] = 0;
        __syncthreads();
    }
    int64_t j = blockIdx.x * (int64_t)blockDim.x + threadIdx.x;
    if (j < p) {
        const double vbar = *vbar_p;
        double a = 0.0;
        for (int64_t s = 0; s < n_slabs; ++s) a += (double)part[s * p + j];
        if (scale_p) a /= (double)*scale_p;
        double corr = 0.0;
        int nm = nmiss[j];
        if (nm) {
            if (impute) {
                for (int64_t e = miss_ptr[j]; e < miss_ptr[j + 1]; ++e) corr += v[miss_idx[e]] - vbar;
            } else {
                corr = -vbar * (double)nm;
            }
        }
        const double df = sinv[j] * (a + mu[j] * corr);
        out[j] = df;
        if (fuse) {
            const double bound = tf.bound_coef * (tf.scal[1] + fabs(tf.scal[0]));
            const double w = tf.wt ? tf.wt[j] : 1.0;
            uint32_t kl, ku;
            topk_make_keys(0.0 + 1.0 * df, w, fabs(1.0) * tf.scale[j] * bound * w, kl, ku);
            tf.keyL[j] = kl; tf.keyU[j] = ku;
            atomicAdd(&sh[kl >> 21], 1);
        }
    }
    if (fuse) {
        __syncthreads();
        for (int b = threadIdx.x; b < TOPK_BINS; b += blockDim.x)
            if (sh[b]) atomicAdd(&tf.hist[b], sh[b]);
    }
}

__global__ void k_vec_mean(const double* __restrict__ v, int64_t n, double* __restrict__ out) {
    __shared__ double sh[32];
    double a = 0.0;
    for (int64_t i = threadIdx.x; i < n; i += blockDim.x) a += v[i];
    a = block_sum(a, sh);
    if (threadIdx.x == 0) out[0] = a / (double)n;
}

__global__ void k_pair_scale(const double* __restrict__ v0, const double* __restrict__ v1, int64_t n,
                             const double* __restrict__ vbar, float* __restrict__ scale) {
    __shared__ double sh[32];
    for (int t = 0; t < 2; ++t) {
        const double* v = t ? v1 : v0;
        const double vb = vbar[t];
        double m = 0.0;
        for (int64_t i = threadIdx.x; i < n; i += blockDim.x) m = fmax(m, fabs(v[i] - vb));
#pragma unroll
        for (int o = 16; o > 0; o >>= 1) m = fmax(m, __shfl_xor_sync(0xffffffffu, m, o));
        __syncthreads();
        if ((threadIdx.x & 31) == 0) sh[threadIdx.x >> 5] = m;
        __syncthreads();
        if (threadIdx.x == 0) {
            for (int w = 1; w < (int)(blockDim.x >> 5); ++w) m = fmax(m, sh[w]);
            int e = 0;
            if (m > 0.0 && isfinite(m)) frexp(m, &e);
            scale[t] = ldexpf(1.0f, 9 - e);
        }
    }
}

__global__ void k_l2norm(const double* __restrict__ v, int64_t n, const double* __restrict__ vbar, double* __restrict__ out) {
    __shared__ double sh[32];
    const double vb = vbar[0];
    double a = 0.0;
    for (int64_t i = threadIdx.x; i < n; i += blockDim.x) { const double u = v[i] - vb; a += u * u; }
    a = block_sum(a, sh);
    if (threadIdx.x == 0) out[0] = sqrt(a);
}

struct SweepScratch {
    DBuf<double> part64;
    DBuf<float> part32;
    DBuf<float> scale;
};

void sweep_xt_v_with_means(const ihtb_geno* g, const double* dV, const double* d_vbar, int64_t m, double* dOut,
                           int mode, cudaStream_t s, void* scratch_any, float* sweep_ms, double* d_l2 = nullptr,
                           const TopkFuse* tf = nullptr) {
    IHTB_CHECK(!tf || (m == 1 && mode != IHTB_SWEEP_PAIR), IHTB_EINVAL, "fused selection stage: one right-hand side");
    const TopkFuse fuse = tf ? *tf : TopkFuse();
    SweepScratch local;
    SweepScratch* sc = scratch_any ? reinterpret_cast<SweepScratch*>(scratch_any) : &local;
    cudaEvent_t e0 = nullptr, e1 = nullptr;
    if (sweep_ms) {
        IHTB_CUDA(cudaEventCreate(&e0)); IHTB_CUDA(cudaEventCreate(&e1));
        IHTB_CUDA(cudaEventRecord(e0, s));
    }
    if (geno_is_dense(g)) {
        dense_xt_v(g, dV, m, dOut, s, &sc->part64, tf);
    } else {
        if (d_l2)
            for (int64_t t = 0; t < m; ++t) IHTB_LAUNCH(k_l2norm, 1, 1024, 0, s, dV + t * g->n, g->n, d_vbar + t, d_l2 + t);
        for (int64_t t = 0; t < m; ++t) {
            const double* v = dV + t * g->n;
            double* out = dOut + t * g->p;
            if (mode == IHTB_SWEEP_PAIR && g->cs_j == 128 && t + 1 < m) {
                const int64_t n_slabs = sweep_fast_num_slabs(g);
                if (sc->part32.n < (size_t)(2 * n_slabs * g->p)) sc->part32.alloc((size_t)(2 * n_slabs * g->p));
                if (sc->scale.n < 2) sc->scale.alloc(2);
                IHTB_LAUNCH(k_pair_scale, 1, 1024, 0, s, v, v + g->n, g->n, d_vbar + t, sc->scale.p);
                sweep_pair_partials(g, v, v + g->n, d_vbar + t, sc->scale.p, sc->part32.p, s);
                for (int h = 0; h < 2; ++h)
                    IHTB_LAUNCH((k_sweep_epilogue<float>), (unsigned)ceil_div(g->p, 256), 256, 0, s,
                                sc->part32.p + (size_t)h * n_slabs * g->p, n_slabs, g->p, g->mu.p, g->sinv.p, g->nmiss.p,
                                g->miss_ptr.p, g->miss_idx.p, v + h * g->n, d_vbar + t + h, g->impute, out + h * g->p,
                                sc->scale.p + h);
                ++t;
                continue;
            }
            if (mode == IHTB_SWEEP_EXACT && exact_uses_lut(g)) {
                const int64_t n_slabs = g->stride / 128;
                if (sc->part64.n < (size_t)(n_slabs * g->p)) sc->part64.alloc((size_t)(n_slabs * g->p));
                sweep_exact_lut_partials(g, v, d_vbar + t, sc->part64.p, s);
                IHTB_LAUNCH((k_sweep_epilogue<double>), (unsigned)ceil_div(g->p, 256), 256, 0, s, sc->part64.p, n_slabs,
                            g->p, g->mu.p, g->sinv.p, g->nmiss.p, g->miss_ptr.p, g->miss_idx.p, v, d_vbar + t,
                            g->impute, out, (const float*)nullptr, fuse);
            } else if (mode == IHTB_SWEEP_EXACT) {
                int64_t words = g->stride >> 2;
                int64_t n_slabs = ceil_div(words, EX_THREADS);
                if (sc->part64.n < (size_t)(n_slabs * g->p)) sc->part64.alloc((size_t)(n_slabs * g->p));
                dim3 grid((unsigned)ceil_div(g->p, EX_COLS_PER_CTA), (unsigned)n_slabs);
                IHTB_LAUNCH(k_sweep_exact, grid, EX_THREADS, 0, s, geno_view(g), v, d_vbar + t, sc->part64.p);
                IHTB_LAUNCH((k_sweep_epilogue<double>), (unsigned)ceil_div(g->p, 256), 256, 0, s, sc->part64.p, n_slabs,
                            g->p, g->mu.p, g->sinv.p, g->nmiss.p, g->miss_ptr.p, g->miss_idx.p, v, d_vbar + t,
                            g->impute, out, (const float*)nullptr, fuse);
            } else {
                int64_t n_slabs = sweep_fast_num_slabs(g);
                if (sc->part32.n < (size_t)(n_slabs * g->p)) sc->part32.alloc((size_t)(n_slabs * g->p));
                sweep_fast_partials(g, v, d_vbar + t, sc->part32.p, &n_slabs, s);
                IHTB_LAUNCH((k_sweep_epilogue<float>), (unsigned)ceil_div(g->p, 256), 256, 0, s, sc->part32.p, n_slabs,
                            g->p, g->mu.p, g->sinv.p, g->nmiss.p, g->miss_ptr.p, g->miss_idx.p, v, d_vbar + t,
                            g->impute, out, (const float*)nullptr, fuse);
            }
        }
    }
    if (sweep_ms) {
        IHTB_CUDA(cudaEventRecord(e1, s));
        IHTB_CUDA(cudaEventSynchronize(e1));
        IHTB_CUDA(cudaEventElapsedTime(sweep_ms, e0, e1));
        cudaEventDestroy(e0); cudaEventDestroy(e1);
    }
}

__global__ void k_copy2(const double* __restrict__ a, const double* __restrict__ b, double* __restrict__ out) {
    out[0] = a[0]; out[1] = b[0];
}

SweepPairer::SweepPairer(int dev) : device(dev) {
    IHTB_CUDA(cudaSetDevice(dev));
    for (int i = 0; i < 2; ++i) IHTB_CUDA(cudaEventCreateWithFlags(&ready[i], cudaEventDisableTiming));
    IHTB_CUDA(cudaEventCreateWithFlags(&done, cudaEventDisableTiming));
    IHTB_CUDA(cudaMalloc((void**)&d_vbar2, 2 * sizeof(double)));
    IHTB_CUDA(cudaMalloc((void**)&d_l2, 2 * sizeof(double)));
    scratch = new SweepScratch();
}
SweepPairer::~SweepPairer() {
    cudaSetDevice(device);
    cudaDeviceSynchronize();
    for (int i = 0; i < 2; ++i) if (ready[i]) cudaEventDestroy(ready[i]);
    if (done) cudaEventDestroy(done);
    if (d_vbar2) cudaFree(d_vbar2);
    if (d_l2) cudaFree(d_l2);
    delete reinterpret_cast<SweepScratch*>(scratch);
}

void SweepPairer::leave() {
    std::lock_guard<std::mutex> lk(mu);
    --active;
    cv.notify_all();
}

bool SweepPairer::sweep(int slot, const ihtb_geno* g, const double* d_v, const double* d_vbar, double* d_out,
                        cudaStream_t s, void* solo_scratch) {
    const int other = slot ^ 1;
    IHTB_CUDA(cudaEventRecord(ready[slot], s));
    std::unique_lock<std::mutex> lk(mu);
    if (active >= 2 && !geno_is_dense(g) && g->cs_j == 128) {
        req[slot] = Req{d_v, d_vbar, d_out, s};
        has[slot] = true;
        if (has[other]) {
            const Req a = req[0], b = req[1];
            SweepScratch* sc = reinterpret_cast<SweepScratch*>(scratch);
            const int64_t n_slabs = sweep_fast_num_slabs(g);
            if (sc->part32.n < (size_t)(2 * n_slabs * g->p)) sc->part32.alloc((size_t)(2 * n_slabs * g->p));
            if (sc->scale.n < 2) sc->scale.alloc(2);
            IHTB_CUDA(cudaStreamWaitEvent(s, ready[other], 0));
            IHTB_LAUNCH(k_copy2, 1, 1, 0, s, a.vbar, b.vbar, d_vbar2);
            IHTB_LAUNCH(k_pair_scale, 1, 1024, 0, s, a.v, b.v, g->n, d_vbar2, sc->scale.p);
            IHTB_LAUNCH(k_l2norm, 1, 1024, 0, s, a.v, g->n, d_vbar2, d_l2);
            IHTB_LAUNCH(k_l2norm, 1, 1024, 0, s, b.v, g->n, d_vbar2 + 1, d_l2 + 1);
            sweep_pair_partials(g, a.v, b.v, d_vbar2, sc->scale.p, sc->part32.p, s);
            const Req* rq[2] = {&a, &b};
            for (int h = 0; h < 2; ++h)
                IHTB_LAUNCH((k_sweep_epilogue<float>), (unsigned)ceil_div(g->p, 256), 256, 0, s,
                            sc->part32.p + (size_t)h * n_slabs * g->p, n_slabs, g->p, g->mu.p, g->sinv.p, g->nmiss.p,
                            g->miss_ptr.p, g->miss_idx.p, rq[h]->v, d_vbar2 + h, g->impute, rq[h]->out, sc->scale.p + h);
            IHTB_CUDA(cudaEventRecord(done, s));
            has[0] = has[1] = false;
            ++round;
            ++n_pair;
            cv.notify_all();
            return true;
        }
        const unsigned long long r0 = round;
        cv.wait(lk, [&] { return round != r0 || active < 2; });
        if (round != r0) {
            IHTB_CUDA(cudaStreamWaitEvent(s, done, 0));
            return true;
        }
        has[slot] = false;
    }
    ++n_solo;
    lk.unlock();
    sweep_xt_v_with_means(g, d_v, d_vbar, 1, d_out, IHTB_SWEEP_FAST, s, solo_scratch, nullptr, nullptr);
    return false;
}

void* sweep_scratch_create() { return new SweepScratch(); }
void sweep_scratch_destroy(void* p) { delete reinterpret_cast<SweepScratch*>(p); }

}

using namespace ihtb;

extern "C" int32_t ihtb_xt_v(const ihtb_geno* g, const double* V, int64_t m, double* out, int32_t sweep_mode) {
    return guard([&] {
        IHTB_CHECK(g && V && out && m >= 1, IHTB_EINVAL, "bad argument");
        geno_require_ready(g);
        IHTB_CHECK(sweep_mode == IHTB_SWEEP_FAST || sweep_mode == IHTB_SWEEP_EXACT || sweep_mode == IHTB_SWEEP_PAIR,
                   IHTB_EINVAL, "bad sweep_mode");
        IHTB_CUDA(cudaSetDevice(g->device));
        DBuf<double> dV((size_t)(g->n * m)), dOut((size_t)(g->p * m)), dmean((size_t)m);
        IHTB_CUDA(cudaMemcpy(dV.p, V, g->n * m * sizeof(double), cudaMemcpyHostToDevice));
        for (int64_t t = 0; t < m; ++t)
            IHTB_LAUNCH(k_vec_mean, 1, 1024, 0, 0, dV.p + t * g->n, g->n, dmean.p + t);
        sweep_xt_v_with_means(g, dV.p, dmean.p, m, dOut.p, sweep_mode, 0, nullptr, nullptr, nullptr);
        IHTB_CUDA(cudaMemcpy(out, dOut.p, g->p * m * sizeof(double), cudaMemcpyDeviceToHost));
    });
}

namespace ihtb {
void sweep_fast_kernel_only(const ihtb_geno* g, const double* d_v, const double* d_vbar, float* d_part, cudaStream_t s);
__global__ void k_fill_vec(double* v, int64_t n, uint64_t seed) {
    int64_t i = blockIdx.x * (int64_t)blockDim.x + threadIdx.x;
    if (i >= n) return;
    uint64_t x = seed + (uint64_t)i * 0x9E3779B97F4A7C15ull;
    x ^= x >> 30; x *= 0xBF58476D1CE4E5B9ull; x ^= x >> 27; x *= 0x94D049BB133111EBull; x ^= x >> 31;
    v[i] = ((double)(x >> 11) * (1.0 / 9007199254740992.0) - 0.5) * 2.0;
}
}

extern "C" int32_t ihtb_sweep_bench(const ihtb_geno* g, int32_t sweep_mode, int32_t warmup, int32_t reps,
                                    double* ms_kernel, double* ms_total) {
    return guard([&] {
        IHTB_CHECK(g && reps >= 1 && warmup >= 0, IHTB_EINVAL, "bad argument");
        geno_require_ready(g);
        IHTB_CUDA(cudaSetDevice(g->device));
        cudaStream_t s;
        IHTB_CUDA(cudaStreamCreateWithFlags(&s, cudaStreamNonBlocking));
        const int64_t mrhs = sweep_mode == IHTB_SWEEP_PAIR ? 2 : 1;
        DBuf<double> dV((size_t)(g->n * mrhs)), dOut((size_t)(g->p * mrhs));
        IHTB_LAUNCH(k_fill_vec, (unsigned)ceil_div(g->n * mrhs, 256), 256, 0, s, dV.p, g->n * mrhs, 12345ull);
        DBuf<double> dmean((size_t)mrhs);
        for (int64_t t = 0; t < mrhs; ++t) IHTB_LAUNCH(k_vec_mean, 1, 1024, 0, s, dV.p + t * g->n, g->n, dmean.p + t);
        SweepScratch sc;
        cudaEvent_t e0, e1;
        IHTB_CUDA(cudaEventCreate(&e0)); IHTB_CUDA(cudaEventCreate(&e1));
        for (int i = 0; i < warmup; ++i)
            sweep_xt_v_with_means(g, dV.p, dmean.p, mrhs, dOut.p, sweep_mode, s, &sc, nullptr, nullptr);
        IHTB_CUDA(cudaEventRecord(e0, s));
        for (int i = 0; i < reps; ++i)
            sweep_xt_v_with_means(g, dV.p, dmean.p, mrhs, dOut.p, sweep_mode, s, &sc, nullptr, nullptr);
        IHTB_CUDA(cudaEventRecord(e1, s));
        IHTB_CUDA(cudaEventSynchronize(e1));
        float ms = 0.f;
        IHTB_CUDA(cudaEventElapsedTime(&ms, e0, e1));
        if (ms_total) *ms_total = ms / reps;
        if (ms_kernel) {
            *ms_kernel = 0.0;
            if (geno_is_dense(g)) {
                IHTB_CUDA(cudaEventRecord(e0, s));
                for (int i = 0; i < reps; ++i) dense_sweep_kernel_only(g, dV.p, &sc.part64, s);
                IHTB_CUDA(cudaEventRecord(e1, s));
                IHTB_CUDA(cudaEventSynchronize(e1));
                IHTB_CUDA(cudaEventElapsedTime(&ms, e0, e1));
                *ms_kernel = ms / reps;
            } else if (sweep_mode == IHTB_SWEEP_PAIR) {
                IHTB_CHECK(g->cs_j == 128, IHTB_EUNSUPPORTED, "the pair sweep needs a tiled layout");
                IHTB_CUDA(cudaEventRecord(e0, s));
                for (int i = 0; i < reps; ++i)
                    sweep_pair_partials(g, dV.p, dV.p + g->n, dmean.p, sc.scale.p, sc.part32.p, s);
                IHTB_CUDA(cudaEventRecord(e1, s));
                IHTB_CUDA(cudaEventSynchronize(e1));
                IHTB_CUDA(cudaEventElapsedTime(&ms, e0, e1));
                *ms_kernel = ms / reps;
            } else if (sweep_mode == IHTB_SWEEP_FAST) {
                IHTB_CUDA(cudaEventRecord(e0, s));
                for (int i = 0; i < reps; ++i) sweep_fast_kernel_only(g, dV.p, dmean.p, sc.part32.p, s);
                IHTB_CUDA(cudaEventRecord(e1, s));
                IHTB_CUDA(cudaEventSynchronize(e1));
                IHTB_CUDA(cudaEventElapsedTime(&ms, e0, e1));
                *ms_kernel = ms / reps;
            } else if (exact_uses_lut(g)) {
                IHTB_CUDA(cudaEventRecord(e0, s));
                for (int i = 0; i < reps; ++i) sweep_exact_lut_partials(g, dV.p, dmean.p, sc.part64.p, s);
                IHTB_CUDA(cudaEventRecord(e1, s));
                IHTB_CUDA(cudaEventSynchronize(e1));
                IHTB_CUDA(cudaEventElapsedTime(&ms, e0, e1));
                *ms_kernel = ms / reps;
            } else {
                int64_t words = g->stride >> 2;
                int64_t n_slabs = ceil_div(words, EX_THREADS);
                dim3 grid((unsigned)ceil_div(g->p, EX_COLS_PER_CTA), (unsigned)n_slabs);
                IHTB_CUDA(cudaEventRecord(e0, s));
                for (int i = 0; i < reps; ++i)
                    IHTB_LAUNCH(k_sweep_exact, grid, EX_THREADS, 0, s, geno_view(g), dV.p, dmean.p, sc.part64.p);
                IHTB_CUDA(cudaEventRecord(e1, s));
                IHTB_CUDA(cudaEventSynchronize(e1));
                IHTB_CUDA(cudaEventElapsedTime(&ms, e0, e1));
                *ms_kernel = ms / reps;
            }
        }
        cudaEventDestroy(e0); cudaEventDestroy(e1);
        cudaStreamDestroy(s);
    });
}

namespace ihtb {

__global__ void __launch_bounds__(EX_THREADS)
k_sweep_class_exact(GenoView gv, const double* __restrict__ v, double* __restrict__ part1, double* __restrict__ part2) {
    __shared__ double red[EX_THREADS / 32][2 * EX_CB];
    const int64_t p = gv.p, n = gv.n;
    const int64_t words = gv.stride >> 2;
    const int64_t slab = blockIdx.y;
    const int64_t w = slab * EX_THREADS + threadIdx.x;
    const bool live = w < words;
    double u[16];
#pragma unroll
    for (int s = 0; s < 16; ++s) {
        int64_t i = 16 * w + s;
        u[s] = (live && i < n) ? v[i] : 0.0;
    }
    const int64_t jbeg = blockIdx.x * (int64_t)EX_COLS_PER_CTA;
    const int64_t jend = (jbeg + EX_COLS_PER_CTA < p) ? jbeg + EX_COLS_PER_CTA : p;
    const int lane = threadIdx.x & 31, warp = threadIdx.x >> 5;
    for (int64_t j0 = jbeg; j0 < jend; j0 += EX_CB) {
        double a1[EX_CB], a2[EX_CB];
#pragma unroll
        for (int c = 0; c < EX_CB; ++c) {
            int64_t j = j0 + c;
            uint32_t x = (live && j < jend) ? *reinterpret_cast<const uint32_t*>(gv_ptr(gv, j, 4 * w)) : 0u;
            double s1 = 0.0, s2 = 0.0;
#pragma unroll
            for (int s = 0; s < 16; ++s) {
                uint32_t code = (x >> (2 * s)) & 3u;
                s1 += (code == 2) ? u[s] : 0.0;
                s2 += (code == 3) ? u[s] : 0.0;
            }
            a1[c] = warp_sum(s1);
            a2[c] = warp_sum(s2);
        }
        __syncthreads();
        if (lane == 0) {
#pragma unroll
            for (int c = 0; c < EX_CB; ++c) { red[warp][c] = a1[c]; red[warp][EX_CB + c] = a2[c]; }
        }
        __syncthreads();
        if (threadIdx.x < 2 * EX_CB) {
            int c = threadIdx.x % EX_CB;
            if (j0 + c < jend) {
                double t = 0.0;
#pragma unroll
                for (int q = 0; q < EX_THREADS / 32; ++q) t += red[q][threadIdx.x];
                (threadIdx.x < EX_CB ? part1 : part2)[slab * p + j0 + c] = t;
            }
        }
    }
}

__global__ void k_class_epilogue(const double* __restrict__ part1, const double* __restrict__ part2, int64_t n_slabs,
                                 int64_t p, const int64_t* __restrict__ miss_ptr, const int32_t* __restrict__ miss_idx,
                                 const double* __restrict__ v, double* __restrict__ out1, double* __restrict__ out2,
                                 double* __restrict__ outm) {
    int64_t j = blockIdx.x * (int64_t)blockDim.x + threadIdx.x;
    if (j >= p) return;
    double a = 0.0, b = 0.0, m = 0.0;
    for (int64_t s = 0; s < n_slabs; ++s) { a += part1[s * p + j]; b += part2[s * p + j]; }
    for (int64_t e = miss_ptr[j]; e < miss_ptr[j + 1]; ++e) m += v[miss_idx[e]];
    out1[j] = a; out2[j] = b; outm[j] = m;
}

void sweep_class_sums(const ihtb_geno* g, const double* d_v, double* d_w1, double* d_w2, double* d_wm, cudaStream_t s,
                      void* scratch_any) {
    SweepScratch* sc = reinterpret_cast<SweepScratch*>(scratch_any);
    if (exact_uses_lut(g)) {
        const int64_t ns = g->stride / 128;
        if (sc->part64.n < (size_t)(2 * ns * g->p)) sc->part64.alloc((size_t)(2 * ns * g->p));
        double* q1 = sc->part64.p;
        double* q2 = sc->part64.p + ns * g->p;
        sweep_exact_lut_partials(g, d_v, nullptr, q1, s, 1);
        sweep_exact_lut_partials(g, d_v, nullptr, q2, s, 2);
        IHTB_LAUNCH(k_class_epilogue, (unsigned)ceil_div(g->p, 256), 256, 0, s, q1, q2, ns, g->p, g->miss_ptr.p,
                    g->miss_idx.p, d_v, d_w1, d_w2, d_wm);
        return;
    }
    int64_t words = g->stride >> 2;
    int64_t n_slabs = ceil_div(words, EX_THREADS);
    if (sc->part64.n < (size_t)(2 * n_slabs * g->p)) sc->part64.alloc((size_t)(2 * n_slabs * g->p));
    double* p1 = sc->part64.p;
    double* p2 = sc->part64.p + n_slabs * g->p;
    dim3 grid((unsigned)ceil_div(g->p, EX_COLS_PER_CTA), (unsigned)n_slabs);
    IHTB_LAUNCH(k_sweep_class_exact, grid, EX_THREADS, 0, s, geno_view(g), d_v, p1, p2);
    IHTB_LAUNCH(k_class_epilogue, (unsigned)ceil_div(g->p, 256), 256, 0, s, p1, p2, n_slabs, g->p, g->miss_ptr.p,
                g->miss_idx.p, d_v, d_w1, d_w2, d_wm);
}

}
```

### mendeliht.jl_b200/csrc/sweep_lut.cu

```cuda
#include "lut_common.cuh"
#include <stdlib.h>

namespace ihtb {

constexpr int LUT_STAGE_COLS = 128;
constexpr int LUT_STAGE_BYTES = LUT_STAGE_COLS * 128;
constexpr int LUT_MAX_STAGES = 8;
constexpr int LUT_MAX_GROUPS = 4;
constexpr uint32_t LUT_BAR_BYTES = 8u * (LUT_MAX_GROUPS + 1) * LUT_MAX_STAGES;
constexpr int LUT_SMEM_BYTES = 232448;

struct LutPlan {
    uint32_t bar_full, bar_empty;
    uint32_t tab;
    uint32_t lo0, hi0;
    int n_lo, n_stages;
    __device__ __forceinline__ uint32_t stage(int s) const {
        return (s < n_lo) ? lo0 + (uint32_t)s * LUT_STAGE_BYTES : hi0 + (uint32_t)(s - n_lo) * LUT_STAGE_BYTES;
    }
};
__device__ __forceinline__ LutPlan lut_plan(uint32_t base, uint32_t bytes) {
    LutPlan pl;
    uint32_t end = base + bytes;
    pl.tab = (base + 65535u) & ~65535u;
    pl.bar_full = 0; pl.bar_empty = 0; pl.n_stages = 0;
    uint32_t lo = (base + 127u) & ~127u, lo_end = pl.tab;
    uint32_t hi = pl.tab + LUT_TABLE_BYTES, hi_end = end;
    if (lo + LUT_BAR_BYTES <= lo_end) { pl.bar_full = lo; lo += LUT_BAR_BYTES; }
    else { pl.bar_full = hi; hi += LUT_BAR_BYTES; }
    pl.bar_empty = pl.bar_full + 8u * LUT_MAX_GROUPS * LUT_MAX_STAGES;
    lo = (lo + 511u) & ~511u; hi = (hi + 511u) & ~511u;
    pl.lo0 = lo; pl.hi0 = hi;
    pl.n_lo = (lo_end > lo) ? (int)((lo_end - lo) / LUT_STAGE_BYTES) : 0;
    if (pl.n_lo > LUT_MAX_STAGES) pl.n_lo = LUT_MAX_STAGES;
    int n_hi = (hi_end > hi) ? (int)((hi_end - hi) / LUT_STAGE_BYTES) : 0;
    pl.n_stages = pl.n_lo + n_hi;
    if (pl.n_stages > LUT_MAX_STAGES) pl.n_stages = LUT_MAX_STAGES;
    return pl;
}

template <int CW, int G, bool QUAD, bool H2, bool TERN>
__global__ void __launch_bounds__((CW + 1) * 32, 1)
k_sweep_lut(const uint8_t* __restrict__ bed, int64_t cs_j, int64_t cs_s, int64_t p, int64_t p_out, int64_t n,
            int64_t n_slabs, const double* __restrict__ v, const double* __restrict__ v1,
            const double* __restrict__ vbar_p, const float* __restrict__ scale_p, float* __restrict__ part,
            uint32_t dyn_bytes) {
    const double vbar = vbar_p[0];
    const double vbar1 = H2 ? vbar_p[1] : 0.0;
    const float sc0 = H2 ? scale_p[0] : 1.0f, sc1 = H2 ? scale_p[1] : 1.0f;
    constexpr bool COL = TERN && !H2;
    constexpr int WPG = CW / G;
    constexpr int CPW = LUT_STAGE_COLS / WPG;
    static_assert(G <= LUT_MAX_GROUPS, "barrier block holds LUT_MAX_GROUPS full barriers per stage");
    static_assert(!QUAD || CPW % 4 == 0, "quad layout: a warp owns whole quads");
    static_assert(!H2 || (CW == 16 && CPW == 16), "pair sweep: 512 table builders, 16 columns per warp");
    static_assert(!TERN || (QUAD && CW == 16), "ternary tiles: quad layout, 512 table builders");
    static_assert(!COL || CPW == 32, "one column per lane: 32 columns per warp");
    extern __shared__ __align__(128) uint8_t smem_raw[];
    const LutPlan pl = lut_plan(smem_u32(smem_raw), dyn_bytes);
    const int warp = threadIdx.x >> 5, lane = threadIdx.x & 31;
    const int S = pl.n_stages;
    int period = S;
    while (period % G != 0) period += S;

    const int64_t n_cblocks = (p + LUT_STAGE_COLS - 1) / LUT_STAGE_COLS;
    const int64_t units = n_slabs * n_cblocks;
    const int64_t u_beg = units * (int64_t)blockIdx.x / gridDim.x;
    const int64_t u_end = units * (int64_t)(blockIdx.x + 1) / gridDim.x;
    if (u_beg >= u_end) return;
    const int64_t slab_beg = u_beg / n_cblocks, slab_end = (u_end - 1) / n_cblocks;
    const int ncb = (int)n_cblocks;

    if (threadIdx.x == 0) {
        for (int s = 0; s < S; ++s) {
            for (int g = 0; g < G; ++g) mbar_init(pl.bar_full + 8u * (g * LUT_MAX_STAGES + s), 1);
            mbar_init(pl.bar_empty + 8u * s, WPG);
        }
        asm volatile("fence.mbarrier_init.release.cluster;" ::: "memory");
    }
    __syncthreads();

    if (warp == CW) {
        int st = 0; uint32_t ph = 0;
        int grp_of = 0;
        for (int64_t slab = slab_beg; slab <= slab_end; ++slab) {
            const int cb0 = (slab == slab_beg) ? (int)(u_beg - slab * n_cblocks) : 0;
            const int cb1 = (slab == slab_end) ? (int)(u_end - slab * n_cblocks) : ncb;
            for (int cb = cb0; cb < cb1; ++cb) {
                const int64_t j0 = (int64_t)cb * LUT_STAGE_COLS;
                const int ncols = (int)((p - j0 < LUT_STAGE_COLS) ? (p - j0) : LUT_STAGE_COLS);
                const uint32_t fullbar = pl.bar_full + 8u * (uint32_t)(grp_of * LUT_MAX_STAGES + st);
                mbar_wait(pl.bar_empty + 8u * st, ph ^ 1u);
                const uint8_t* src = bed + j0 * cs_j + slab * cs_s;
                if (cs_j == 128) {
                    if (lane == 0) {
                        mbar_expect_tx(fullbar, (uint32_t)ncols * 128u);
                        bulk_g2s(pl.stage(st), src, (uint32_t)ncols * 128u, fullbar);
                    }
                } else {
                    if (lane == 0) mbar_expect_tx(fullbar, (uint32_t)ncols * 128u);
                    __syncwarp();
                    for (int c = lane; c < ncols; c += 32)
                        bulk_g2s(pl.stage(st) + 128u * c, src + (int64_t)c * cs_j, 128u, fullbar);
                }
                if (++st == S) { st = 0; ph ^= 1u; }
                if (++grp_of == G) grp_of = 0;
            }
        }
    } else {
        const int tid = threadIdx.x;
        const int grp = warp / WPG, wg = warp % WPG;
        uint32_t lb[4];
#pragma unroll
        for (int t = 0; t < 4; ++t)
            lb[t] = pl.tab + (uint32_t)(t >> 1) * 65536u + (uint32_t)(t & 1) * 128u + 4u * (uint32_t)lane;
        constexpr int NACC = H2 ? 2 * CPW : CPW;
        constexpr int LPC = 32 / NACC > 0 ? 32 / NACC : 1;
        const int vidx = TERN ? (lane & (NACC - 1)) : lane / LPC;
        const int col = wg * CPW + vidx % CPW;
        const bool writer = TERN ? (lane < NACC) : (lane & (LPC - 1)) == 0;
        const uint32_t lqs = TERN ? ((((uint32_t)lane >> 2) & 3u) << 9) : 0u;
        const uint32_t lane_off = (uint32_t)(wg * CPW) * 128u + (QUAD ? 16u : 4u) * (uint32_t)lane;
        const uint32_t w0 = 8u * ((uint32_t)lane & 3u) + ((uint32_t)lane >> 2);
        const uint32_t col_off = (uint32_t)(wg * CPW) * 128u + ((uint32_t)lane >> 2) * 512u + 16u * w0 +
                                 4u * (((uint32_t)lane & 3u) ^ (w0 & 3u));
        const uint32_t y0 = 4u * w0 | (128u + 4u * w0) << 8 | (pl.tab >> 16) << 16 | ((pl.tab >> 16) + 1u) << 24;
        int st = grp % S, ip = grp % period; uint32_t ph = (uint32_t)((grp / period) & 1);
        const uint32_t my_full = pl.bar_full + 8u * (uint32_t)(grp * LUT_MAX_STAGES);
        int i_next = grp;
        int i_base = 0;
        for (int64_t slab = slab_beg; slab <= slab_end; ++slab) {
            const int cb0 = (slab == slab_beg) ? (int)(u_beg - slab * n_cblocks) : 0;
            const int cb1 = (slab == slab_end) ? (int)(u_end - slab * n_cblocks) : ncb;
            consumer_bar<CW * 32>();
            if (H2 && TERN) lut_build_h2_tern(pl.tab, v, v1, vbar, vbar1, sc0, sc1, n, slab, tid);
            else if (H2) lut_build_h2(pl.tab, v, v1, vbar, vbar1, sc0, sc1, n, slab, tid);
            else if (TERN) lut_build_tern<CW * 32>(pl.tab, v, vbar, n, slab, tid);
            else lut_build<CW * 32>(pl.tab, v, vbar, n, slab, tid);
            consumer_bar<CW * 32>();
            float* __restrict__ outp = part + ((int64_t)(H2 ? vidx / CPW : 0) * n_slabs + slab) * p_out + col;
            const int i_end = i_base + (cb1 - cb0);
            for (; i_next < i_end; i_next += G) {
                const int cb = cb0 + (i_next - i_base);
                mbar_wait(my_full + 8u * st, ph);
                float sum;
                if constexpr (COL) {
                    const uint32_t a0 = pl.stage(st) + col_off;
                    uint32_t wd[32];
#pragma unroll
                    for (int s = 0; s < 32; ++s) wd[s] = lds_u32(a0 ^ (16u * s + 4u * (s & 3)));
                    __syncwarp();
                    if (lane == 0) mbar_arrive(pl.bar_empty + 8u * st);
                    float ws[32];
#pragma unroll
                    for (int s = 0; s < 32; ++s) {
                        const uint32_t y = y0 ^ (uint32_t)(4 * s * 0x0101);
                        const float t0 = lds_f32(prmt<0xE604u>(wd[s], y));
                        const float t1 = lds_f32(prmt<0xE615u>(wd[s], y));
                        const float t2 = lds_f32(prmt<0xF724u>(wd[s], y));
                        const float t3 = lds_f32(prmt<0xF735u>(wd[s], y));
                        ws[s] = (t0 + t1) + (t2 + t3);
                    }
#pragma unroll
                    for (int k = 0, done = 0; k < 5; ++k) {
                        const int b = (k < 4) ? (8 >> k) : 16;
#pragma unroll
                        for (int s = 0; s < 32; ++s)
                            if ((s & (done | b)) == 0) ws[s] = ws[s] + ws[s | b];
                        done |= b;
                    }
                    sum = ws[0];
                } else {
                    const uint32_t colbase = pl.stage(st) + lane_off;
                    float acc[NACC];
                    uint4 q4 = make_uint4(0u, 0u, 0u, 0u);
#pragma unroll
                    for (int c = 0; c < CPW; ++c) {
                        uint32_t w;
                        if (QUAD) {
                            if ((c & 3) == 0) q4 = lds_u128(colbase + ((512u * (c >> 2)) ^ lqs));
                            w = (c & 3) == 0 ? q4.x : (c & 3) == 1 ? q4.y : (c & 3) == 2 ? q4.z : q4.w;
                        } else {
                            w = lds_u32(colbase + 128u * c);
                        }
                        if (!H2) {
                            const float t0 = lds_f32(__byte_perm(w, lb[0], 0x7604));
                            const float t1 = lds_f32(__byte_perm(w, lb[1], 0x7614));
                            const float t2 = lds_f32(__byte_perm(w, lb[2], 0x7624));
                            const float t3 = lds_f32(__byte_perm(w, lb[3], 0x7634));
                            acc[c] = (t0 + t1) + (t2 + t3);
                        } else {
                            const uint32_t r0 = lds_u32(__byte_perm(w, lb[0], 0x7604));
                            const uint32_t r1 = lds_u32(__byte_perm(w, lb[1], 0x7614));
                            const uint32_t r2 = lds_u32(__byte_perm(w, lb[2], 0x7624));
                            const uint32_t r3 = lds_u32(__byte_perm(w, lb[3], 0x7634));
                            const __half2 h = __hadd2(__hadd2(*reinterpret_cast<const __half2*>(&r0), *reinterpret_cast<const __half2*>(&r1)),
                                                      __hadd2(*reinterpret_cast<const __half2*>(&r2), *reinterpret_cast<const __half2*>(&r3)));
                            const float2 f = __half22float2(h);
                            acc[c] = f.x;
                            acc[(H2 ? CPW : 0) + c] = f.y;
                        }
                    }
                    __syncwarp();
                    if (lane == 0) mbar_arrive(pl.bar_empty + 8u * st);
                    if (TERN) {
                        int o = NACC / 2;
#pragma unroll
                        for (int h = NACC / 2; h >= 1; h >>= 1, o >>= 1) {
#pragma unroll
                            for (int c = 0; c < h; ++c) acc[c] = acc[c] + __shfl_xor_sync(0xffffffffu, acc[c + h], o);
                        }
                    } else {
                        int o = 16;
#pragma unroll
                        for (int h = NACC / 2; h >= 1; h >>= 1, o >>= 1) {
                            const bool upper = (lane & o) != 0;
#pragma unroll
                            for (int c = 0; c < h; ++c) {
                                const float send = upper ? acc[c] : acc[c + h];
                                const float keep = upper ? acc[c + h] : acc[c];
                                acc[c] = keep + __shfl_xor_sync(0xffffffffu, send, o);
                            }
                        }
#pragma unroll
                        for (int oo = 16 / NACC; oo >= 1; oo >>= 1) acc[0] += __shfl_xor_sync(0xffffffffu, acc[0], oo);
                    }
                    sum = acc[0];
                }
                const int jj = cb * LUT_STAGE_COLS + col;
                if (writer && jj < (int)p_out) outp[cb * LUT_STAGE_COLS] = sum;
                st += G; while (st >= S) st -= S;
                ip += G; if (ip >= period) { ip -= period; ph ^= 1u; }
            }
            i_base = i_end;
        }
    }
}

bool sweep_tmem_enabled(const ihtb_geno* g);
bool sweep_uses_tern(const ihtb_geno* g) { return g->tern.p != nullptr && g->quad && !sweep_tmem_enabled(g); }
int64_t sweep_fast_num_slabs(const ihtb_geno* g) { return sweep_uses_tern(g) ? g->tern_slabs : g->stride / 128; }

bool sweep_tmem_enabled(const ihtb_geno* g);
void sweep_tmem_partials(const ihtb_geno* g, const double* d_v, const double* d_vbar, float* d_part, cudaStream_t s);
void sweep_tmem_pair_partials(const ihtb_geno* g, const double* d_v0, const double* d_v1, const double* d_vbar,
                              const float* d_scale, float* d_part, cudaStream_t s);

template <bool QUAD, bool H2, bool TERN = false>
static void launch_lut(const ihtb_geno* g, const double* d_v, const double* d_v1, const double* d_vbar,
                       const float* d_scale, float* d_part, cudaStream_t s) {
    constexpr int G = (TERN && !H2) ? 4 : 2;
    ensure_dynamic_smem(k_sweep_lut<16, G, QUAD, H2, TERN>, LUT_SMEM_BYTES);
    const int64_t n_slabs = TERN ? g->tern_slabs : g->stride / 128;
    const int64_t n_cblocks = ceil_div(g->p4, LUT_STAGE_COLS);
    int64_t units = n_slabs * n_cblocks;
    int grid = g->sm_count;
    if (units < grid) grid = (int)units;
    IHTB_CHECK(g->p < (int64_t(1) << 31) - 256, IHTB_EDIM, "more than 2^31 SNP columns on one GPU");
    IHTB_LAUNCH((k_sweep_lut<16, G, QUAD, H2, TERN>), grid, 17 * 32, LUT_SMEM_BYTES, s, TERN ? g->tern.p : g->bed.p, g->cs_j,
                g->cs_s, g->p4, g->p, g->n, n_slabs, d_v, d_v1, d_vbar, d_scale, d_part, (uint32_t)LUT_SMEM_BYTES);
}

void sweep_fast_partials(const ihtb_geno* g, const double* d_v, const double* d_vbar, float* d_part, int64_t* n_slabs_out,
                         cudaStream_t s) {
    if (n_slabs_out) *n_slabs_out = sweep_fast_num_slabs(g);
    if (sweep_tmem_enabled(g)) { sweep_tmem_partials(g, d_v, d_vbar, d_part, s); return; }
    if (sweep_uses_tern(g)) launch_lut<true, false, true>(g, d_v, nullptr, d_vbar, nullptr, d_part, s);
    else if (g->quad) launch_lut<true, false>(g, d_v, nullptr, d_vbar, nullptr, d_part, s);
    else launch_lut<false, false>(g, d_v, nullptr, d_vbar, nullptr, d_part, s);
}

void sweep_fast_kernel_only(const ihtb_geno* g, const double* d_v, const double* d_vbar, float* d_part, cudaStream_t s) {
    sweep_fast_partials(g, d_v, d_vbar, d_part, nullptr, s);
}

void sweep_pair_partials(const ihtb_geno* g, const double* d_v0, const double* d_v1, const double* d_vbar,
                         const float* d_scale, float* d_part, cudaStream_t s) {
    IHTB_CHECK(g->cs_j == 128, IHTB_EUNSUPPORTED, "the pair sweep needs a tiled layout");
    if (sweep_tmem_enabled(g)) { sweep_tmem_pair_partials(g, d_v0, d_v1, d_vbar, d_scale, d_part, s); return; }
    if (sweep_uses_tern(g)) launch_lut<true, true, true>(g, d_v0, d_v1, d_vbar, d_scale, d_part, s);
    else if (g->quad) launch_lut<true, true>(g, d_v0, d_v1, d_vbar, d_scale, d_part, s);
    else launch_lut<false, true>(g, d_v0, d_v1, d_vbar, d_scale, d_part, s);
}

}
```

### mendeliht.jl_b200/csrc/sweep_tmem.cu

```cuda
#include "lut_common.cuh"
#include <cuda_fp16.h>
#include <stdlib.h>

namespace ihtb {

constexpr int TM_CW = 16;
constexpr int TM_THREADS = (TM_CW + 2) * 32;
constexpr int TM_STAGE_COLS = 128;
constexpr int TM_STAGE_BYTES = TM_STAGE_COLS * 128;
constexpr int TM_UNIT_COLS = 256;
constexpr int TM_SLOTS = 8;
constexpr int TM_MAX_STAGES = 6;
constexpr int TM_SMEM_BYTES = 232448;

__device__ __forceinline__ void mbar_arrive_plain(uint32_t bar) {
    asm volatile("mbarrier.arrive.shared::cta.b64 _, [%0];" ::"r"(bar) : "memory");
}
__device__ __forceinline__ void tc_fence_before() { asm volatile("tcgen05.fence::before_thread_sync;" ::: "memory"); }
__device__ __forceinline__ void tc_fence_after() { asm volatile("tcgen05.fence::after_thread_sync;" ::: "memory"); }
__device__ __forceinline__ void tc_commit(uint32_t bar) {
    asm volatile("tcgen05.commit.cta_group::1.mbarrier::arrive::one.shared::cluster.b64 [%0];" ::"r"(bar) : "memory");
}
__device__ __forceinline__ void tc_cp_128x256b(uint32_t taddr, uint64_t desc) {
    asm volatile("tcgen05.cp.cta_group::1.128x256b [%0], %1;" ::"r"(taddr), "l"(desc) : "memory");
}

struct TmPlan {
    uint32_t bars;
    uint32_t tab, lo0, hi0;
    int n_lo, n_stages;
    __device__ __forceinline__ uint32_t stage(int s) const {
        return (s < n_lo) ? lo0 + (uint32_t)s * TM_STAGE_BYTES : hi0 + (uint32_t)(s - n_lo) * TM_STAGE_BYTES;
    }
    __device__ __forceinline__ uint32_t smem_full(int s) const { return bars + 8u * (uint32_t)s; }
    __device__ __forceinline__ uint32_t smem_empty(int s) const { return bars + 8u * (uint32_t)(TM_MAX_STAGES + s); }
    __device__ __forceinline__ uint32_t tmem_full(int t) const { return bars + 8u * (uint32_t)(2 * TM_MAX_STAGES + t); }
    __device__ __forceinline__ uint32_t tmem_empty(int t) const { return bars + 8u * (uint32_t)(2 * TM_MAX_STAGES + TM_SLOTS + t); }
    __device__ __forceinline__ uint32_t tmem_word() const { return bars + 8u * (uint32_t)(2 * TM_MAX_STAGES + 2 * TM_SLOTS); }
};
__device__ __forceinline__ TmPlan tm_plan(uint32_t base, uint32_t bytes) {
    TmPlan pl;
    const uint32_t end = base + bytes;
    pl.tab = (base + 65535u) & ~65535u;
    uint32_t lo = (base + 1023u) & ~1023u;
    pl.bars = lo; lo += 1024u;
    pl.lo0 = lo;
    pl.n_lo = (pl.tab > lo) ? (int)((pl.tab - lo) / TM_STAGE_BYTES) : 0;
    pl.hi0 = pl.tab + LUT_TABLE_BYTES;
    const int n_hi = (end > pl.hi0) ? (int)((end - pl.hi0) / TM_STAGE_BYTES) : 0;
    pl.n_stages = pl.n_lo + n_hi;
    if (pl.n_stages > TM_MAX_STAGES) pl.n_stages = TM_MAX_STAGES;
    return pl;
}

template <bool H2>
__global__ void __launch_bounds__(TM_THREADS, 1)
k_sweep_tmem(const uint8_t* __restrict__ bed, int64_t cs_s, int64_t p4, int64_t p_out, int64_t n, int64_t n_slabs,
             const double* __restrict__ v, const double* __restrict__ v1, const double* __restrict__ vbar_p,
             const float* __restrict__ scale_p, float* __restrict__ part, uint32_t dyn_bytes) {
    const double vbar = vbar_p[0];
    const double vbar1 = H2 ? vbar_p[1] : 0.0;
    const float sc0 = H2 ? scale_p[0] : 1.0f, sc1 = H2 ? scale_p[1] : 1.0f;
    extern __shared__ __align__(1024) uint8_t smem_raw[];
    const TmPlan pl = tm_plan(smem_u32(smem_raw), dyn_bytes);
    const int warp = threadIdx.x >> 5, lane = threadIdx.x & 31;
    const int S = pl.n_stages;

    const int64_t ncb = (p4 + TM_UNIT_COLS - 1) / TM_UNIT_COLS;
    const int64_t units = n_slabs * ncb;
    const int64_t u_beg = units * (int64_t)blockIdx.x / gridDim.x;
    const int64_t u_end = units * (int64_t)(blockIdx.x + 1) / gridDim.x;
    const int64_t slab_beg = u_beg / ncb;

    if (threadIdx.x == 0) {
        for (int s = 0; s < S; ++s) { mbar_init(pl.smem_full(s), 1); mbar_init(pl.smem_empty(s), 1); }
        for (int t = 0; t < TM_SLOTS; ++t) { mbar_init(pl.tmem_full(t), 1); mbar_init(pl.tmem_empty(t), TM_CW); }
        asm volatile("fence.mbarrier_init.release.cluster;" ::: "memory");
    }
    if (warp == TM_CW + 1) {
        asm volatile("tcgen05.alloc.cta_group::1.sync.aligned.shared::cta.b32 [%0], 512;" ::"r"(pl.tmem_word()) : "memory");
        asm volatile("tcgen05.relinquish_alloc_permit.cta_group::1.sync.aligned;" ::: "memory");
    }
    tc_fence_before();
    __syncthreads();
    tc_fence_after();
    const uint32_t tbase = lds_u32(pl.tmem_word());

    if (u_beg < u_end) {
        if (warp == TM_CW) {
            if (lane == 0) {
                int st = 0; uint32_t ph = 0;
                int64_t slab = slab_beg, cb = u_beg - slab_beg * ncb;
                for (int64_t u = u_beg; u < u_end; ++u) {
                    for (int h = 0; h < 2; ++h) {
                        const int64_t j0 = cb * TM_UNIT_COLS + (int64_t)h * TM_STAGE_COLS;
                        int64_t ncols = p4 - j0;
                        ncols = ncols < 0 ? 0 : (ncols > TM_STAGE_COLS ? TM_STAGE_COLS : ncols);
                        mbar_wait(pl.smem_empty(st), ph ^ 1u);
                        if (ncols > 0) {
                            mbar_expect_tx(pl.smem_full(st), (uint32_t)ncols * 128u);
                            bulk_g2s(pl.stage(st), bed + slab * cs_s + j0 * 128, (uint32_t)ncols * 128u, pl.smem_full(st));
                        } else {
                            mbar_arrive_plain(pl.smem_full(st));
                        }
                        if (++st == S) { st = 0; ph ^= 1u; }
                    }
                    if (++cb == ncb) { cb = 0; ++slab; }
                }
            }
        } else if (warp == TM_CW + 1) {
            if (lane == 0) {
                int st = 0; uint32_t ph = 0;
                int ts = 0; uint32_t tph = 0;
                const uint64_t desc_hi = ((uint64_t)(2048u >> 4) << 16) | ((uint64_t)(128u >> 4) << 32) | ((uint64_t)1 << 46);
                for (int64_t u = u_beg; u < u_end; ++u) {
                    mbar_wait(pl.tmem_empty(ts), tph ^ 1u);
                    for (int h = 0; h < 2; ++h) {
                        mbar_wait(pl.smem_full(st), ph);
                        tc_fence_after();
                        const uint32_t sbase = pl.stage(st);
#pragma unroll
                        for (int c = 0; c < 4; ++c)
                            tc_cp_128x256b(tbase + (uint32_t)(64 * ts + 32 * h + 8 * c),
                                           desc_hi | (uint64_t)(((sbase + 4096u * c) >> 4) & 0x3FFFu));
                        tc_commit(pl.smem_empty(st));
                        if (++st == S) { st = 0; ph ^= 1u; }
                    }
                    tc_commit(pl.tmem_full(ts));
                    if (++ts == TM_SLOTS) { ts = 0; tph ^= 1u; }
                }
            }
        } else {
            const int tid = threadIdx.x;
            const int g = warp & 3, j = warp >> 2;
            uint32_t lb[4];
#pragma unroll
            for (int t = 0; t < 4; ++t)
                lb[t] = pl.tab + (uint32_t)(t >> 1) * 65536u + (uint32_t)(t & 1) * 128u + 4u * (uint32_t)lane;
            constexpr int NACC = H2 ? 32 : 16;
            constexpr int LPC = 32 / NACC;
            const int vidx = lane / LPC;
            const int a_idx = vidx & 15;
            const int col = 64 * j + 16 * (a_idx >> 2) + 4 * g + (a_idx & 3);
            const bool writer = (lane & (LPC - 1)) == 0;
            const uint32_t tlane = tbase + ((uint32_t)(32 * g) << 16) + (uint32_t)(16 * j);
            int ts = 0; uint32_t tph = 0;
            int64_t slab = slab_beg, cb = u_beg - slab_beg * ncb;
            bool need_build = true;
            for (int64_t u = u_beg; u < u_end; ++u) {
                if (need_build) {
                    consumer_bar<TM_CW * 32>();
                    if (H2) lut_build_h2(pl.tab, v, v1, vbar, vbar1, sc0, sc1, n, slab, tid);
                    else lut_build<TM_CW * 32>(pl.tab, v, vbar, n, slab, tid);
                    consumer_bar<TM_CW * 32>();
                    need_build = false;
                }
                mbar_wait(pl.tmem_full(ts), tph);
                tc_fence_after();
                uint32_t w[16];
                asm volatile(
                    "tcgen05.ld.sync.aligned.32x32b.x16.b32 {%0, %1, %2, %3, %4, %5, %6, %7, %8, %9, %10, %11, %12, %13, %14, %15}, [%16];"
                    : "=r"(w[0]), "=r"(w[1]), "=r"(w[2]), "=r"(w[3]), "=r"(w[4]), "=r"(w[5]), "=r"(w[6]), "=r"(w[7]),
                      "=r"(w[8]), "=r"(w[9]), "=r"(w[10]), "=r"(w[11]), "=r"(w[12]), "=r"(w[13]), "=r"(w[14]), "=r"(w[15])
                    : "r"(tlane + (uint32_t)(64 * ts)));
                asm volatile("tcgen05.wait::ld.sync.aligned;" ::: "memory");
                tc_fence_before();
                __syncwarp();
                if (lane == 0) mbar_arrive(pl.tmem_empty(ts));
                float acc[NACC];
#pragma unroll
                for (int c = 0; c < 16; ++c) {
                    if (!H2) {
                        const float t0 = lds_f32(__byte_perm(w[c], lb[0], 0x7604));
                        const float t1 = lds_f32(__byte_perm(w[c], lb[1], 0x7614));
                        const float t2 = lds_f32(__byte_perm(w[c], lb[2], 0x7624));
                        const float t3 = lds_f32(__byte_perm(w[c], lb[3], 0x7634));
                        acc[c] = (t0 + t1) + (t2 + t3);
                    } else {
                        const uint32_t r0 = lds_u32(__byte_perm(w[c], lb[0], 0x7604));
                        const uint32_t r1 = lds_u32(__byte_perm(w[c], lb[1], 0x7614));
                        const uint32_t r2 = lds_u32(__byte_perm(w[c], lb[2], 0x7624));
                        const uint32_t r3 = lds_u32(__byte_perm(w[c], lb[3], 0x7634));
                        const __half2 hs = __hadd2(__hadd2(*reinterpret_cast<const __half2*>(&r0), *reinterpret_cast<const __half2*>(&r1)),
                                                   __hadd2(*reinterpret_cast<const __half2*>(&r2), *reinterpret_cast<const __half2*>(&r3)));
                        const float2 f = __half22float2(hs);
                        acc[c] = f.x;
                        acc[(H2 ? 16 : 0) + c] = f.y;
                    }
                }
                int o = 16;
#pragma unroll
                for (int h = NACC / 2; h >= 1; h >>= 1, o >>= 1) {
                    const bool upper = (lane & o) != 0;
#pragma unroll
                    for (int c = 0; c < h; ++c) {
                        const float send = upper ? acc[c] : acc[c + h];
                        const float keep = upper ? acc[c + h] : acc[c];
                        acc[c] = keep + __shfl_xor_sync(0xffffffffu, send, o);
                    }
                }
#pragma unroll
                for (int oo = 16 / NACC; oo >= 1; oo >>= 1) acc[0] += __shfl_xor_sync(0xffffffffu, acc[0], oo);
                const int64_t jj = cb * TM_UNIT_COLS + col;
                if (writer && jj < p_out) part[((int64_t)(H2 ? vidx >> 4 : 0) * n_slabs + slab) * p_out + jj] = acc[0];
                if (++ts == TM_SLOTS) { ts = 0; tph ^= 1u; }
                if (++cb == ncb) { cb = 0; ++slab; need_build = true; }
            }
        }
    }
    tc_fence_before();
    __syncthreads();
    if (warp == TM_CW + 1) {
        __syncwarp();
        tc_fence_after();
        asm volatile("tcgen05.dealloc.cta_group::1.sync.aligned.b32 %0, 512;" ::"r"(tbase) : "memory");
    }
}

template <bool H2>
static void launch_tmem(const ihtb_geno* g, const double* d_v, const double* d_v1, const double* d_vbar,
                        const float* d_scale, float* d_part, cudaStream_t s) {
    ensure_dynamic_smem(k_sweep_tmem<H2>, TM_SMEM_BYTES);
    const int64_t n_slabs = g->stride / 128;
    const int64_t units = n_slabs * ceil_div(g->p4, TM_UNIT_COLS);
    int grid = g->sm_count;
    if (units < grid) grid = (int)units;
    IHTB_CHECK(g->p < (int64_t(1) << 31) - 256, IHTB_EDIM, "more than 2^31 SNP columns on one GPU");
    IHTB_LAUNCH((k_sweep_tmem<H2>), grid, TM_THREADS, TM_SMEM_BYTES, s, g->bed.p, g->cs_s, g->p4, g->p, g->n, n_slabs,
                d_v, d_v1, d_vbar, d_scale, d_part, (uint32_t)TM_SMEM_BYTES);
}

bool sweep_tmem_enabled(const ihtb_geno* g) {
    const char* e = getenv("IHTB_SWEEP_TMEM");
    return g->quad && e && *e == '1';
}
void sweep_tmem_partials(const ihtb_geno* g, const double* d_v, const double* d_vbar, float* d_part, cudaStream_t s) {
    launch_tmem<false>(g, d_v, nullptr, d_vbar, nullptr, d_part, s);
}
void sweep_tmem_pair_partials(const ihtb_geno* g, const double* d_v0, const double* d_v1, const double* d_vbar,
                              const float* d_scale, float* d_part, cudaStream_t s) {
    launch_tmem<true>(g, d_v0, d_v1, d_vbar, d_scale, d_part, s);
}

}
```

Baseline: 926.4.

## Accumulate sweep slab partials into fixed-point int64 atomics instead of f32 partial arrays

```diff
diff --git a/_probe/prof.py b/_probe/prof.py
--- /dev/null
+++ b/_probe/prof.py
@@ -0,0 +1,37 @@
+import ctypes as C, json, os, sys, time
+sys.path.insert(0, os.getcwd())
+import numpy as np
+import bench
+import mendeliht_jl_b200 as m
+from mendeliht_jl_b200 import synth
+from torch.profiler import profile, ProfilerActivity
+lib = m.load(); m._lib.check(lib.ihtb_set_device(0))
+n, p, k = bench.N_SAMPLES, bench.P_PER_GPU, bench.K_SPARSITY
+bed = np.empty((p, (n + 3) // 4), dtype=np.uint8)
+m._lib.check(lib.ihtb_synth_host(n, p, 0, bench.SEED, 0.0, bed.ctypes.data_as(C.POINTER(C.c_uint8))))
+g = m.B200SnpLinAlg.from_bed_columns(bed, n); del bed
+y, z, _, _, _ = synth.simulate_response(bench.SEED + 1, n, p, k, bench.DIST, geno_seed=bench.SEED)
+v = m.IHTVariable(g, z, y, k, bench.DIST, bench.LINK)
+for _ in range(2):
+    v.init_iht_indices(None); v.fit(trace_cap=0)
+with profile(activities=[ProfilerActivity.CUDA]) as prof:
+    v.init_iht_indices(None); res, _ = v.fit(trace_cap=0)
+ev = [e for e in prof.events() if e.device_type.name == "CUDA"]
+ev.sort(key=lambda e: e.time_range.start)
+iters = int(res.iter)
+tot = {}
+for e in ev:
+    d = tot.setdefault(e.name[:70], [0, 0.0]); d[0] += 1; d[1] += e.time_range.end - e.time_range.start
+span = ev[-1].time_range.end - ev[0].time_range.start
+busy = sum(e.time_range.end - e.time_range.start for e in ev)
+print(json.dumps({"iters": iters, "span_us": span, "busy_us": busy, "per_iter_span_us": span / iters, "per_iter_busy_us": busy / iters}))
+for name, (c, t) in sorted(tot.items(), key=lambda x: -x[1][1])[:25]:
+    print(f"{name:72s} n={c:5d} tot_us={t:10.1f} per_iter_us={t/iters:8.2f} avg_us={t/c:8.2f}")
+gap = {}
+for a, b in zip(ev, ev[1:]):
+    gp = b.time_range.start - a.time_range.end
+    if gp > 0:
+        d = gap.setdefault(b.name[:70], [0, 0.0]); d[0] += 1; d[1] += gp
+print("idle before kernel (us per iteration):")
+for name, (c, t) in sorted(gap.items(), key=lambda x: -x[1][1])[:15]:
+    print(f"  {name:72s} n={c:5d} per_iter_us={t/iters:8.2f}")
diff --git a/mendeliht.jl_b200/csrc/common.cuh b/mendeliht.jl_b200/csrc/common.cuh
--- a/mendeliht.jl_b200/csrc/common.cuh
+++ b/mendeliht.jl_b200/csrc/common.cuh
@@ -109,6 +109,11 @@
 };
 
 static inline int64_t ceil_div(int64_t a, int64_t b) { return (a + b - 1) / b; }
+
+struct AbsSums {
+    const double* sum = nullptr;
+    const double* abs = nullptr;
+};
 
 bool smem_attr_needed(const void* kernel, int device);
 template <typename K>
diff --git a/mendeliht.jl_b200/csrc/fit.cu b/mendeliht.jl_b200/csrc/fit.cu
--- a/mendeliht.jl_b200/csrc/fit.cu
+++ b/mendeliht.jl_b200/csrc/fit.cu
@@ -13,8 +13,8 @@
 #include <unordered_map>
 
 namespace ihtb {
-void sweep_xt_v_with_means(const ihtb_geno* g, const double* dV, const double* vbar_host, int64_t m, double* dOut,
-                           int mode, cudaStream_t s, void* scratch_any, float* sweep_ms, double* d_l2 = nullptr,
+void sweep_xt_v_with_means(const ihtb_geno* g, const double* dV, const double* d_vbar, AbsSums ab, int64_t m,
+                           double* dOut, int mode, cudaStream_t s, void* scratch_any, float* sweep_ms, double* d_l2 = nullptr,
                            const TopkFuse* tf = nullptr);
 void* sweep_scratch_create();
 void sweep_scratch_destroy(void* p);
@@ -276,6 +276,13 @@
         n_cand_iter += (int64_t)need.size();
     }
 
+    AbsSums score_abs() const {
+        AbsSums a;
+        a.sum = d_scal.p;
+        a.abs = d_scal.p + 1;
+        return a;
+    }
+
     void score_and_sweep() {
         glm_score(glm, s, d_vbar.p);
         IHTB_CUDA(cudaMemcpyAsync(h_scal.p, d_scal.p, (2 + q) * sizeof(double), cudaMemcpyDeviceToHost, s));
@@ -284,15 +291,16 @@
         const double t_sw = now();
         if (pairer && cfg.sweep_mode == IHTB_SWEEP_FAST) {
             IHTB_CHECK(!grouped() && !comm, IHTB_EUNSUPPORTED, "paired sweeps serve plain single-device fits only");
-            if (pairer->sweep(pair_slot, g, d_r.p, d_vbar.p, d_dfa.p, s, sweep_scratch)) {
+            if (pairer->sweep(pair_slot, g, d_r.p, d_vbar.p, score_abs(), d_dfa.p, s, sweep_scratch)) {
                 sweep_coef = kPairBound;
                 IHTB_CUDA(cudaMemcpyAsync(h_scal.p + 3 + q, pairer->d_l2 + pair_slot, sizeof(double), cudaMemcpyDeviceToHost, s));
             }
         } else if (cfg.k > 0 && !(grouped() && !init_plain)) {
             const TopkFuse tf = topk_absdf_fuse_begin(tk, geno_bound_scale(g), d_scal.p, sweep_coef);
-            sweep_xt_v_with_means(g, d_r.p, d_vbar.p, 1, d_dfa.p, cfg.sweep_mode, s, sweep_scratch, nullptr, nullptr, &tf);
+            sweep_xt_v_with_means(g, d_r.p, d_vbar.p, score_abs(), 1, d_dfa.p, cfg.sweep_mode, s, sweep_scratch, nullptr,
+                                  nullptr, &tf);
         } else {
-            sweep_xt_v_with_means(g, d_r.p, d_vbar.p, 1, d_dfa.p, cfg.sweep_mode, s, sweep_scratch, nullptr);
+            sweep_xt_v_with_means(g, d_r.p, d_vbar.p, score_abs(), 1, d_dfa.p, cfg.sweep_mode, s, sweep_scratch, nullptr);
         }
         IHTB_CUDA(cudaEventRecord(ev1, s));
         ++n_sweeps;
@@ -364,7 +372,7 @@
             if (count > cap && coef == kPairBound && !rerun) {
                 ++n_pair_overflow;
                 sweep_coef = kFastBound;
-                sweep_xt_v_with_means(g, d_r.p, d_vbar.p, 1, d_dfa.p, IHTB_SWEEP_FAST, s, sweep_scratch, nullptr);
+                sweep_xt_v_with_means(g, d_r.p, d_vbar.p, score_abs(), 1, d_dfa.p, IHTB_SWEEP_FAST, s, sweep_scratch, nullptr);
                 IHTB_CUDA(cudaEventRecord(ev1, s));
                 select_rescore(false);
                 return;
diff --git a/mendeliht.jl_b200/csrc/lut_common.cuh b/mendeliht.jl_b200/csrc/lut_common.cuh
--- a/mendeliht.jl_b200/csrc/lut_common.cuh
+++ b/mendeliht.jl_b200/csrc/lut_common.cuh
@@ -5,6 +5,18 @@
 namespace ihtb {
 
 constexpr int LUT_TABLE_BYTES = 131072;
+
+constexpr int ACC_EXP_MIN = -100, ACC_EXP_MAX = 200;
+__device__ __forceinline__ double acc_bound(AbsSums a, int t) { return a.abs[t] + (a.sum ? fabs(a.sum[t]) : 0.0); }
+__device__ __forceinline__ int acc_exp(double A) {
+    const int bexp = (int)((__double_as_longlong(A) >> 52) & 0x7FF);
+    if (!(A > 0.0) || bexp == 0x7FF) return 0;
+    return min(max(bexp - 1020, ACC_EXP_MIN), ACC_EXP_MAX);
+}
+__device__ __forceinline__ double pow2(int e) { return __longlong_as_double((long long)(1023 + e) << 52); }
+__device__ __forceinline__ void acc_add(int64_t* acc, float x, double qs) {
+    atomicAdd(reinterpret_cast<unsigned long long*>(acc), (unsigned long long)__double2ll_rn((double)x * qs));
+}
 
 __device__ __forceinline__ uint32_t smem_u32(const void* p) { return (uint32_t)__cvta_generic_to_shared(p); }
 __device__ __forceinline__ void mbar_init(uint32_t bar, uint32_t count) {
diff --git a/mendeliht.jl_b200/csrc/mvfit.cu b/mendeliht.jl_b200/csrc/mvfit.cu
--- a/mendeliht.jl_b200/csrc/mvfit.cu
+++ b/mendeliht.jl_b200/csrc/mvfit.cu
@@ -8,8 +8,8 @@
 #include <memory>
 
 namespace ihtb {
-void sweep_xt_v_with_means(const ihtb_geno* g, const double* dV, const double* vbar_host, int64_t m, double* dOut,
-                           int mode, cudaStream_t s, void* scratch_any, float* sweep_ms, double* d_l2 = nullptr,
+void sweep_xt_v_with_means(const ihtb_geno* g, const double* dV, const double* d_vbar, AbsSums ab, int64_t m,
+                           double* dOut, int mode, cudaStream_t s, void* scratch_any, float* sweep_ms, double* d_l2 = nullptr,
                            const TopkFuse* tf = nullptr);
 void* sweep_scratch_create();
 void sweep_scratch_destroy(void* p);
@@ -376,7 +376,10 @@
         IHTB_CUDA(cudaEventRecord(ev0, s));
         const bool l2mode = cfg.sweep_mode == IHTB_SWEEP_PAIR && g->cs_j == 128;
         if (l2mode && d_l2.n < (size_t)r) { d_l2.alloc((size_t)r); h_l2.alloc((size_t)r); }
-        sweep_xt_v_with_means(g, d_R1.p, d_vbar.p, r, d_dfa.p, cfg.sweep_mode, s, sweep_scratch, nullptr,
+        AbsSums ab;
+        ab.sum = d_scal.p;
+        ab.abs = d_scal.p + r;
+        sweep_xt_v_with_means(g, d_R1.p, d_vbar.p, ab, r, d_dfa.p, cfg.sweep_mode, s, sweep_scratch, nullptr,
                               l2mode ? d_l2.p : nullptr);
         IHTB_CUDA(cudaEventRecord(ev1, s));
         if (l2mode) IHTB_CUDA(cudaMemcpyAsync(h_l2.p, d_l2.p, (size_t)r * sizeof(double), cudaMemcpyDeviceToHost, s));
diff --git a/mendeliht.jl_b200/csrc/pairer.cuh b/mendeliht.jl_b200/csrc/pairer.cuh
--- a/mendeliht.jl_b200/csrc/pairer.cuh
+++ b/mendeliht.jl_b200/csrc/pairer.cuh
@@ -26,8 +26,8 @@
     ~SweepPairer();
     SweepPairer(const SweepPairer&) = delete;
     SweepPairer& operator=(const SweepPairer&) = delete;
-    bool sweep(int slot, const ihtb_geno* g, const double* d_v, const double* d_vbar, double* d_out, cudaStream_t s,
-               void* solo_scratch);
+    bool sweep(int slot, const ihtb_geno* g, const double* d_v, const double* d_vbar, AbsSums ab, double* d_out,
+               cudaStream_t s, void* solo_scratch);
     void leave();
 };
 
diff --git a/mendeliht.jl_b200/csrc/sweep.cu b/mendeliht.jl_b200/csrc/sweep.cu
--- a/mendeliht.jl_b200/csrc/sweep.cu
+++ b/mendeliht.jl_b200/csrc/sweep.cu
@@ -1,17 +1,16 @@
-#include "common.cuh"
+#include "lut_common.cuh"
 #include "pairer.cuh"
 #include "topk.cuh"
 #include <stdlib.h>
 
 namespace ihtb {
 
-void sweep_fast_partials(const ihtb_geno* g, const double* d_v, const double* d_vbar, float* d_part, int64_t* n_slabs,
-                         cudaStream_t s);
-int64_t sweep_fast_num_slabs(const ihtb_geno* g);
+void sweep_fast_accumulate(const ihtb_geno* g, const double* d_v, const double* d_vbar, AbsSums ab, int64_t* d_acc,
+                           cudaStream_t s);
 void sweep_exact_lut_partials(const ihtb_geno* g, const double* d_v, const double* d_vbar, double* d_part, cudaStream_t s,
                               int cls = 0);
-void sweep_pair_partials(const ihtb_geno* g, const double* d_v0, const double* d_v1, const double* d_vbar,
-                         const float* d_scale, float* d_part, cudaStream_t s);
+void sweep_pair_accumulate(const ihtb_geno* g, const double* d_v0, const double* d_v1, const double* d_vbar,
+                           const float* d_scale, const double* d_abs, int64_t* d_acc, cudaStream_t s);
 
 static bool exact_uses_lut(const ihtb_geno* g) {
     static const bool legacy = [] { const char* e = getenv("IHTB_EXACT_LEGACY"); return e && *e == '1'; }();
@@ -75,9 +74,15 @@
     }
 }
 
-template <typename T>
+struct SweepSums {
+    const double* part = nullptr;
+    int64_t n_slabs = 0;
+    int64_t* acc = nullptr;
+    AbsSums ab;
+};
+
 __global__ void __launch_bounds__(256)
-k_sweep_epilogue(const T* __restrict__ part, int64_t n_slabs, int64_t p,
+k_sweep_epilogue(SweepSums src, int64_t p,
                  const double* __restrict__ mu, const double* __restrict__ sinv,
                  const int32_t* __restrict__ nmiss, const int64_t* __restrict__ miss_ptr,
                  const int32_t* __restrict__ miss_idx, const double* __restrict__ v,
@@ -95,7 +100,13 @@
     if (j < p) {
         const double vbar = *vbar_p;
         double a = 0.0;
-        for (int64_t s = 0; s < n_slabs; ++s) a += (double)part[s * p + j];
+        if (src.acc) {
+            const double A = acc_bound(src.ab, 0);
+            a = isfinite(A) ? (double)src.acc[j] * pow2(acc_exp(A) - 62) : __longlong_as_double(0x7FF8000000000000ll);
+            src.acc[j] = 0;
+        } else {
+            for (int64_t s = 0; s < src.n_slabs; ++s) a += src.part[s * p + j];
+        }
         if (scale_p) a /= (double)*scale_p;
         double corr = 0.0;
         int nm = nmiss[j];
@@ -124,32 +135,45 @@
     }
 }
 
-__global__ void k_vec_mean(const double* __restrict__ v, int64_t n, double* __restrict__ out) {
+__global__ void k_vec_mean(const double* __restrict__ v, int64_t n, double* __restrict__ out, double* __restrict__ abs) {
     __shared__ double sh[32];
+    __shared__ double mean;
     double a = 0.0;
     for (int64_t i = threadIdx.x; i < n; i += blockDim.x) a += v[i];
     a = block_sum(a, sh);
-    if (threadIdx.x == 0) out[0] = a / (double)n;
+    if (threadIdx.x == 0) { mean = a / (double)n; out[0] = mean; }
+    __syncthreads();
+    const double vb = mean;
+    a = 0.0;
+    for (int64_t i = threadIdx.x; i < n; i += blockDim.x) a += fabs(v[i] - vb);
+    a = block_sum(a, sh);
+    if (threadIdx.x == 0) abs[0] = a;
 }
 
 __global__ void k_pair_scale(const double* __restrict__ v0, const double* __restrict__ v1, int64_t n,
-                             const double* __restrict__ vbar, float* __restrict__ scale) {
-    __shared__ double sh[32];
+                             const double* __restrict__ vbar, float* __restrict__ scale, double* __restrict__ abs) {
+    __shared__ double sh[32], sa[32];
     for (int t = 0; t < 2; ++t) {
         const double* v = t ? v1 : v0;
         const double vb = vbar[t];
-        double m = 0.0;
-        for (int64_t i = threadIdx.x; i < n; i += blockDim.x) m = fmax(m, fabs(v[i] - vb));
+        double m = 0.0, a = 0.0;
+        for (int64_t i = threadIdx.x; i < n; i += blockDim.x) {
+            const double u = fabs(v[i] - vb);
+            m = fmax(m, u);
+            a += u;
+        }
 #pragma unroll
         for (int o = 16; o > 0; o >>= 1) m = fmax(m, __shfl_xor_sync(0xffffffffu, m, o));
-        __syncthreads();
-        if ((threadIdx.x & 31) == 0) sh[threadIdx.x >> 5] = m;
+        a = warp_sum(a);
+        __syncthreads();
+        if ((threadIdx.x & 31) == 0) { sh[threadIdx.x >> 5] = m; sa[threadIdx.x >> 5] = a; }
         __syncthreads();
         if (threadIdx.x == 0) {
-            for (int w = 1; w < (int)(blockDim.x >> 5); ++w) m = fmax(m, sh[w]);
+            for (int w = 1; w < (int)(blockDim.x >> 5); ++w) { m = fmax(m, sh[w]); a += sa[w]; }
             int e = 0;
             if (m > 0.0 && isfinite(m)) frexp(m, &e);
             scale[t] = ldexpf(1.0f, 9 - e);
+            abs[t] = a * (double)scale[t];
         }
     }
 }
@@ -165,13 +189,44 @@
 
 struct SweepScratch {
     DBuf<double> part64;
-    DBuf<float> part32;
+    DBuf<int64_t> acc;
+    bool acc_dirty = false;
     DBuf<float> scale;
+    DBuf<double> pabs;
+    int64_t* acc_begin(size_t count, cudaStream_t s) {
+        if (acc.n < count) { acc.alloc(count); acc_dirty = true; }
+        if (acc_dirty) acc.zero(s);
+        acc_dirty = true;
+        return acc.p;
+    }
+    void acc_done() { acc_dirty = false; }
 };
 
-void sweep_xt_v_with_means(const ihtb_geno* g, const double* dV, const double* d_vbar, int64_t m, double* dOut,
-                           int mode, cudaStream_t s, void* scratch_any, float* sweep_ms, double* d_l2 = nullptr,
-                           const TopkFuse* tf = nullptr) {
+static void launch_epilogue(const ihtb_geno* g, const SweepSums& src, const double* v, const double* d_vbar, double* out,
+                            const float* scale, const TopkFuse& tf, cudaStream_t s) {
+    IHTB_LAUNCH(k_sweep_epilogue, (unsigned)ceil_div(g->p, 256), 256, 0, s, src, g->p, g->mu.p, g->sinv.p, g->nmiss.p,
+                g->miss_ptr.p, g->miss_idx.p, v, d_vbar, g->impute, out, scale, tf);
+}
+
+static void pair_sweep(const ihtb_geno* g, const double* v0, const double* v1, const double* d_vbar2, double* out0,
+                       double* out1, SweepScratch* sc, cudaStream_t s) {
+    if (sc->scale.n < 2) sc->scale.alloc(2);
+    if (sc->pabs.n < 2) sc->pabs.alloc(2);
+    IHTB_LAUNCH(k_pair_scale, 1, 1024, 0, s, v0, v1, g->n, d_vbar2, sc->scale.p, sc->pabs.p);
+    int64_t* acc = sc->acc_begin((size_t)(2 * g->p), s);
+    sweep_pair_accumulate(g, v0, v1, d_vbar2, sc->scale.p, sc->pabs.p, acc, s);
+    for (int h = 0; h < 2; ++h) {
+        SweepSums src;
+        src.acc = acc + (size_t)h * g->p;
+        src.ab.abs = sc->pabs.p + h;
+        launch_epilogue(g, src, h ? v1 : v0, d_vbar2 + h, h ? out1 : out0, sc->scale.p + h, TopkFuse(), s);
+    }
+    sc->acc_done();
+}
+
+void sweep_xt_v_with_means(const ihtb_geno* g, const double* dV, const double* d_vbar, AbsSums ab, int64_t m,
+                           double* dOut, int mode, cudaStream_t s, void* scratch_any, float* sweep_ms,
+                           double* d_l2 = nullptr, const TopkFuse* tf = nullptr) {
     IHTB_CHECK(!tf || (m == 1 && mode != IHTB_SWEEP_PAIR), IHTB_EINVAL, "fused selection stage: one right-hand side");
     const TopkFuse fuse = tf ? *tf : TopkFuse();
     SweepScratch local;
@@ -190,42 +245,33 @@
             const double* v = dV + t * g->n;
             double* out = dOut + t * g->p;
             if (mode == IHTB_SWEEP_PAIR && g->cs_j == 128 && t + 1 < m) {
-                const int64_t n_slabs = sweep_fast_num_slabs(g);
-                if (sc->part32.n < (size_t)(2 * n_slabs * g->p)) sc->part32.alloc((size_t)(2 * n_slabs * g->p));
-                if (sc->scale.n < 2) sc->scale.alloc(2);
-                IHTB_LAUNCH(k_pair_scale, 1, 1024, 0, s, v, v + g->n, g->n, d_vbar + t, sc->scale.p);
-                sweep_pair_partials(g, v, v + g->n, d_vbar + t, sc->scale.p, sc->part32.p, s);
-                for (int h = 0; h < 2; ++h)
-                    IHTB_LAUNCH((k_sweep_epilogue<float>), (unsigned)ceil_div(g->p, 256), 256, 0, s,
-                                sc->part32.p + (size_t)h * n_slabs * g->p, n_slabs, g->p, g->mu.p, g->sinv.p, g->nmiss.p,
-                                g->miss_ptr.p, g->miss_idx.p, v + h * g->n, d_vbar + t + h, g->impute, out + h * g->p,
-                                sc->scale.p + h);
+                pair_sweep(g, v, v + g->n, d_vbar + t, out, out + g->p, sc, s);
                 ++t;
                 continue;
             }
+            SweepSums src;
             if (mode == IHTB_SWEEP_EXACT && exact_uses_lut(g)) {
                 const int64_t n_slabs = g->stride / 128;
                 if (sc->part64.n < (size_t)(n_slabs * g->p)) sc->part64.alloc((size_t)(n_slabs * g->p));
                 sweep_exact_lut_partials(g, v, d_vbar + t, sc->part64.p, s);
-                IHTB_LAUNCH((k_sweep_epilogue<double>), (unsigned)ceil_div(g->p, 256), 256, 0, s, sc->part64.p, n_slabs,
-                            g->p, g->mu.p, g->sinv.p, g->nmiss.p, g->miss_ptr.p, g->miss_idx.p, v, d_vbar + t,
-                            g->impute, out, (const float*)nullptr, fuse);
+                src.part = sc->part64.p; src.n_slabs = n_slabs;
+                launch_epilogue(g, src, v, d_vbar + t, out, nullptr, fuse, s);
             } else if (mode == IHTB_SWEEP_EXACT) {
                 int64_t words = g->stride >> 2;
                 int64_t n_slabs = ceil_div(words, EX_THREADS);
                 if (sc->part64.n < (size_t)(n_slabs * g->p)) sc->part64.alloc((size_t)(n_slabs * g->p));
                 dim3 grid((unsigned)ceil_div(g->p, EX_COLS_PER_CTA), (unsigned)n_slabs);
                 IHTB_LAUNCH(k_sweep_exact, grid, EX_THREADS, 0, s, geno_view(g), v, d_vbar + t, sc->part64.p);
-                IHTB_LAUNCH((k_sweep_epilogue<double>), (unsigned)ceil_div(g->p, 256), 256, 0, s, sc->part64.p, n_slabs,
-                            g->p, g->mu.p, g->sinv.p, g->nmiss.p, g->miss_ptr.p, g->miss_idx.p, v, d_vbar + t,
-                            g->impute, out, (const float*)nullptr, fuse);
+                src.part = sc->part64.p; src.n_slabs = n_slabs;
+                launch_epilogue(g, src, v, d_vbar + t, out, nullptr, fuse, s);
             } else {
-                int64_t n_slabs = sweep_fast_num_slabs(g);
-                if (sc->part32.n < (size_t)(n_slabs * g->p)) sc->part32.alloc((size_t)(n_slabs * g->p));
-                sweep_fast_partials(g, v, d_vbar + t, sc->part32.p, &n_slabs, s);
-                IHTB_LAUNCH((k_sweep_epilogue<float>), (unsigned)ceil_div(g->p, 256), 256, 0, s, sc->part32.p, n_slabs,
-                            g->p, g->mu.p, g->sinv.p, g->nmiss.p, g->miss_ptr.p, g->miss_idx.p, v, d_vbar + t,
-                            g->impute, out, (const float*)nullptr, fuse);
+                IHTB_CHECK(ab.abs != nullptr, IHTB_EINVAL, "table sweep without a bound of sum |v - mean|");
+                src.ab.sum = ab.sum ? ab.sum + t : nullptr;
+                src.ab.abs = ab.abs + t;
+                src.acc = sc->acc_begin((size_t)g->p, s);
+                sweep_fast_accumulate(g, v, d_vbar + t, src.ab, src.acc, s);
+                launch_epilogue(g, src, v, d_vbar + t, out, nullptr, fuse, s);
+                sc->acc_done();
             }
         }
     }
@@ -265,7 +311,7 @@
     cv.notify_all();
 }
 
-bool SweepPairer::sweep(int slot, const ihtb_geno* g, const double* d_v, const double* d_vbar, double* d_out,
+bool SweepPairer::sweep(int slot, const ihtb_geno* g, const double* d_v, const double* d_vbar, AbsSums ab, double* d_out,
                         cudaStream_t s, void* solo_scratch) {
     const int other = slot ^ 1;
     IHTB_CUDA(cudaEventRecord(ready[slot], s));
@@ -276,20 +322,11 @@
         if (has[other]) {
             const Req a = req[0], b = req[1];
             SweepScratch* sc = reinterpret_cast<SweepScratch*>(scratch);
-            const int64_t n_slabs = sweep_fast_num_slabs(g);
-            if (sc->part32.n < (size_t)(2 * n_slabs * g->p)) sc->part32.alloc((size_t)(2 * n_slabs * g->p));
-            if (sc->scale.n < 2) sc->scale.alloc(2);
             IHTB_CUDA(cudaStreamWaitEvent(s, ready[other], 0));
             IHTB_LAUNCH(k_copy2, 1, 1, 0, s, a.vbar, b.vbar, d_vbar2);
-            IHTB_LAUNCH(k_pair_scale, 1, 1024, 0, s, a.v, b.v, g->n, d_vbar2, sc->scale.p);
             IHTB_LAUNCH(k_l2norm, 1, 1024, 0, s, a.v, g->n, d_vbar2, d_l2);
             IHTB_LAUNCH(k_l2norm, 1, 1024, 0, s, b.v, g->n, d_vbar2 + 1, d_l2 + 1);
-            sweep_pair_partials(g, a.v, b.v, d_vbar2, sc->scale.p, sc->part32.p, s);
-            const Req* rq[2] = {&a, &b};
-            for (int h = 0; h < 2; ++h)
-                IHTB_LAUNCH((k_sweep_epilogue<float>), (unsigned)ceil_div(g->p, 256), 256, 0, s,
-                            sc->part32.p + (size_t)h * n_slabs * g->p, n_slabs, g->p, g->mu.p, g->sinv.p, g->nmiss.p,
-                            g->miss_ptr.p, g->miss_idx.p, rq[h]->v, d_vbar2 + h, g->impute, rq[h]->out, sc->scale.p + h);
+            pair_sweep(g, a.v, b.v, d_vbar2, a.out, b.out, sc, s);
             IHTB_CUDA(cudaEventRecord(done, s));
             has[0] = has[1] = false;
             ++round;
@@ -307,7 +344,7 @@
     }
     ++n_solo;
     lk.unlock();
-    sweep_xt_v_with_means(g, d_v, d_vbar, 1, d_out, IHTB_SWEEP_FAST, s, solo_scratch, nullptr, nullptr);
+    sweep_xt_v_with_means(g, d_v, d_vbar, ab, 1, d_out, IHTB_SWEEP_FAST, s, solo_scratch, nullptr, nullptr);
     return false;
 }
 
@@ -325,17 +362,18 @@
         IHTB_CHECK(sweep_mode == IHTB_SWEEP_FAST || sweep_mode == IHTB_SWEEP_EXACT || sweep_mode == IHTB_SWEEP_PAIR,
                    IHTB_EINVAL, "bad sweep_mode");
         IHTB_CUDA(cudaSetDevice(g->device));
-        DBuf<double> dV((size_t)(g->n * m)), dOut((size_t)(g->p * m)), dmean((size_t)m);
+        DBuf<double> dV((size_t)(g->n * m)), dOut((size_t)(g->p * m)), dmean((size_t)m), dabs((size_t)m);
         IHTB_CUDA(cudaMemcpy(dV.p, V, g->n * m * sizeof(double), cudaMemcpyHostToDevice));
         for (int64_t t = 0; t < m; ++t)
-            IHTB_LAUNCH(k_vec_mean, 1, 1024, 0, 0, dV.p + t * g->n, g->n, dmean.p + t);
-        sweep_xt_v_with_means(g, dV.p, dmean.p, m, dOut.p, sweep_mode, 0, nullptr, nullptr, nullptr);
+            IHTB_LAUNCH(k_vec_mean, 1, 1024, 0, 0, dV.p + t * g->n, g->n, dmean.p + t, dabs.p + t);
+        AbsSums ab;
+        ab.abs = dabs.p;
+        sweep_xt_v_with_means(g, dV.p, dmean.p, ab, m, dOut.p, sweep_mode, 0, nullptr, nullptr, nullptr);
         IHTB_CUDA(cudaMemcpy(out, dOut.p, g->p * m * sizeof(double), cudaMemcpyDeviceToHost));
     });
 }
 
 namespace ihtb {
-void sweep_fast_kernel_only(const ihtb_geno* g, const double* d_v, const double* d_vbar, float* d_part, cudaStream_t s);
 __global__ void k_fill_vec(double* v, int64_t n, uint64_t seed) {
     int64_t i = blockIdx.x * (int64_t)blockDim.x + threadIdx.x;
     if (i >= n) return;
@@ -356,16 +394,19 @@
         const int64_t mrhs = sweep_mode == IHTB_SWEEP_PAIR ? 2 : 1;
         DBuf<double> dV((size_t)(g->n * mrhs)), dOut((size_t)(g->p * mrhs));
         IHTB_LAUNCH(k_fill_vec, (unsigned)ceil_div(g->n * mrhs, 256), 256, 0, s, dV.p, g->n * mrhs, 12345ull);
-        DBuf<double> dmean((size_t)mrhs);
-        for (int64_t t = 0; t < mrhs; ++t) IHTB_LAUNCH(k_vec_mean, 1, 1024, 0, s, dV.p + t * g->n, g->n, dmean.p + t);
+        DBuf<double> dmean((size_t)mrhs), dabs((size_t)mrhs);
+        for (int64_t t = 0; t < mrhs; ++t)
+            IHTB_LAUNCH(k_vec_mean, 1, 1024, 0, s, dV.p + t * g->n, g->n, dmean.p + t, dabs.p + t);
+        AbsSums ab;
+        ab.abs = dabs.p;
         SweepScratch sc;
         cudaEvent_t e0, e1;
         IHTB_CUDA(cudaEventCreate(&e0)); IHTB_CUDA(cudaEventCreate(&e1));
         for (int i = 0; i < warmup; ++i)
-            sweep_xt_v_with_means(g, dV.p, dmean.p, mrhs, dOut.p, sweep_mode, s, &sc, nullptr, nullptr);
+            sweep_xt_v_with_means(g, dV.p, dmean.p, ab, mrhs, dOut.p, sweep_mode, s, &sc, nullptr, nullptr);
         IHTB_CUDA(cudaEventRecord(e0, s));
         for (int i = 0; i < reps; ++i)
-            sweep_xt_v_with_means(g, dV.p, dmean.p, mrhs, dOut.p, sweep_mode, s, &sc, nullptr, nullptr);
+            sweep_xt_v_with_means(g, dV.p, dmean.p, ab, mrhs, dOut.p, sweep_mode, s, &sc, nullptr, nullptr);
         IHTB_CUDA(cudaEventRecord(e1, s));
         IHTB_CUDA(cudaEventSynchronize(e1));
         float ms = 0.f;
@@ -384,18 +425,20 @@
                 IHTB_CHECK(g->cs_j == 128, IHTB_EUNSUPPORTED, "the pair sweep needs a tiled layout");
                 IHTB_CUDA(cudaEventRecord(e0, s));
                 for (int i = 0; i < reps; ++i)
-                    sweep_pair_partials(g, dV.p, dV.p + g->n, dmean.p, sc.scale.p, sc.part32.p, s);
+                    sweep_pair_accumulate(g, dV.p, dV.p + g->n, dmean.p, sc.scale.p, sc.pabs.p, sc.acc.p, s);
                 IHTB_CUDA(cudaEventRecord(e1, s));
                 IHTB_CUDA(cudaEventSynchronize(e1));
                 IHTB_CUDA(cudaEventElapsedTime(&ms, e0, e1));
                 *ms_kernel = ms / reps;
+                sc.acc.zero(s);
             } else if (sweep_mode == IHTB_SWEEP_FAST) {
                 IHTB_CUDA(cudaEventRecord(e0, s));
-                for (int i = 0; i < reps; ++i) sweep_fast_kernel_only(g, dV.p, dmean.p, sc.part32.p, s);
+                for (int i = 0; i < reps; ++i) sweep_fast_accumulate(g, dV.p, dmean.p, ab, sc.acc.p, s);
                 IHTB_CUDA(cudaEventRecord(e1, s));
                 IHTB_CUDA(cudaEventSynchronize(e1));
                 IHTB_CUDA(cudaEventElapsedTime(&ms, e0, e1));
                 *ms_kernel = ms / reps;
+                sc.acc.zero(s);
             } else if (exact_uses_lut(g)) {
                 IHTB_CUDA(cudaEventRecord(e0, s));
                 for (int i = 0; i < reps; ++i) sweep_exact_lut_partials(g, dV.p, dmean.p, sc.part64.p, s);
diff --git a/mendeliht.jl_b200/csrc/sweep_lut.cu b/mendeliht.jl_b200/csrc/sweep_lut.cu
--- a/mendeliht.jl_b200/csrc/sweep_lut.cu
+++ b/mendeliht.jl_b200/csrc/sweep_lut.cu
@@ -43,7 +43,7 @@
 __global__ void __launch_bounds__((CW + 1) * 32, 1)
 k_sweep_lut(const uint8_t* __restrict__ bed, int64_t cs_j, int64_t cs_s, int64_t p, int64_t p_out, int64_t n,
             int64_t n_slabs, const double* __restrict__ v, const double* __restrict__ v1,
-            const double* __restrict__ vbar_p, const float* __restrict__ scale_p, float* __restrict__ part,
+            const double* __restrict__ vbar_p, const float* __restrict__ scale_p, AbsSums ab, int64_t* __restrict__ tot,
             uint32_t dyn_bytes) {
     const double vbar = vbar_p[0];
     const double vbar1 = H2 ? vbar_p[1] : 0.0;
@@ -125,6 +125,9 @@
         const uint32_t col_off = (uint32_t)(wg * CPW) * 128u + ((uint32_t)lane >> 2) * 512u + 16u * w0 +
                                  4u * (((uint32_t)lane & 3u) ^ (w0 & 3u));
         const uint32_t y0 = 4u * w0 | (128u + 4u * w0) << 8 | (pl.tab >> 16) << 16 | ((pl.tab >> 16) + 1u) << 24;
+        const int rhs = H2 ? vidx / CPW : 0;
+        const double qs = pow2(62 - acc_exp(acc_bound(ab, rhs)));
+        int64_t* __restrict__ outp = tot + (int64_t)rhs * p_out + col;
         int st = grp % S, ip = grp % period; uint32_t ph = (uint32_t)((grp / period) & 1);
         const uint32_t my_full = pl.bar_full + 8u * (uint32_t)(grp * LUT_MAX_STAGES);
         int i_next = grp;
@@ -138,7 +141,6 @@
             else if (TERN) lut_build_tern<CW * 32>(pl.tab, v, vbar, n, slab, tid);
             else lut_build<CW * 32>(pl.tab, v, vbar, n, slab, tid);
             consumer_bar<CW * 32>();
-            float* __restrict__ outp = part + ((int64_t)(H2 ? vidx / CPW : 0) * n_slabs + slab) * p_out + col;
             const int i_end = i_base + (cb1 - cb0);
             for (; i_next < i_end; i_next += G) {
                 const int cb = cb0 + (i_next - i_base);
@@ -228,7 +230,7 @@
                     sum = acc[0];
                 }
                 const int jj = cb * LUT_STAGE_COLS + col;
-                if (writer && jj < (int)p_out) outp[cb * LUT_STAGE_COLS] = sum;
+                if (writer && jj < (int)p_out) acc_add(outp + cb * LUT_STAGE_COLS, sum, qs);
                 st += G; while (st >= S) st -= S;
                 ip += G; if (ip >= period) { ip -= period; ph ^= 1u; }
             }
@@ -239,16 +241,15 @@
 
 bool sweep_tmem_enabled(const ihtb_geno* g);
 bool sweep_uses_tern(const ihtb_geno* g) { return g->tern.p != nullptr && g->quad && !sweep_tmem_enabled(g); }
-int64_t sweep_fast_num_slabs(const ihtb_geno* g) { return sweep_uses_tern(g) ? g->tern_slabs : g->stride / 128; }
-
-bool sweep_tmem_enabled(const ihtb_geno* g);
-void sweep_tmem_partials(const ihtb_geno* g, const double* d_v, const double* d_vbar, float* d_part, cudaStream_t s);
-void sweep_tmem_pair_partials(const ihtb_geno* g, const double* d_v0, const double* d_v1, const double* d_vbar,
-                              const float* d_scale, float* d_part, cudaStream_t s);
+
+void sweep_tmem_accumulate(const ihtb_geno* g, const double* d_v, const double* d_vbar, AbsSums ab, int64_t* d_acc,
+                           cudaStream_t s);
+void sweep_tmem_pair_accumulate(const ihtb_geno* g, const double* d_v0, const double* d_v1, const double* d_vbar,
+                                const float* d_scale, const double* d_abs, int64_t* d_acc, cudaStream_t s);
 
 template <bool QUAD, bool H2, bool TERN = false>
 static void launch_lut(const ihtb_geno* g, const double* d_v, const double* d_v1, const double* d_vbar,
-                       const float* d_scale, float* d_part, cudaStream_t s) {
+                       const float* d_scale, AbsSums ab, int64_t* d_acc, cudaStream_t s) {
     constexpr int G = (TERN && !H2) ? 4 : 2;
     ensure_dynamic_smem(k_sweep_lut<16, G, QUAD, H2, TERN>, LUT_SMEM_BYTES);
     const int64_t n_slabs = TERN ? g->tern_slabs : g->stride / 128;
@@ -258,29 +259,26 @@
     if (units < grid) grid = (int)units;
     IHTB_CHECK(g->p < (int64_t(1) << 31) - 256, IHTB_EDIM, "more than 2^31 SNP columns on one GPU");
     IHTB_LAUNCH((k_sweep_lut<16, G, QUAD, H2, TERN>), grid, 17 * 32, LUT_SMEM_BYTES, s, TERN ? g->tern.p : g->bed.p, g->cs_j,
-                g->cs_s, g->p4, g->p, g->n, n_slabs, d_v, d_v1, d_vbar, d_scale, d_part, (uint32_t)LUT_SMEM_BYTES);
-}
-
-void sweep_fast_partials(const ihtb_geno* g, const double* d_v, const double* d_vbar, float* d_part, int64_t* n_slabs_out,
-                         cudaStream_t s) {
-    if (n_slabs_out) *n_slabs_out = sweep_fast_num_slabs(g);
-    if (sweep_tmem_enabled(g)) { sweep_tmem_partials(g, d_v, d_vbar, d_part, s); return; }
-    if (sweep_uses_tern(g)) launch_lut<true, false, true>(g, d_v, nullptr, d_vbar, nullptr, d_part, s);
-    else if (g->quad) launch_lut<true, false>(g, d_v, nullptr, d_vbar, nullptr, d_part, s);
-    else launch_lut<false, false>(g, d_v, nullptr, d_vbar, nullptr, d_part, s);
-}
-
-void sweep_fast_kernel_only(const ihtb_geno* g, const double* d_v, const double* d_vbar, float* d_part, cudaStream_t s) {
-    sweep_fast_partials(g, d_v, d_vbar, d_part, nullptr, s);
-}
-
-void sweep_pair_partials(const ihtb_geno* g, const double* d_v0, const double* d_v1, const double* d_vbar,
-                         const float* d_scale, float* d_part, cudaStream_t s) {
+                g->cs_s, g->p4, g->p, g->n, n_slabs, d_v, d_v1, d_vbar, d_scale, ab, d_acc, (uint32_t)LUT_SMEM_BYTES);
+}
+
+void sweep_fast_accumulate(const ihtb_geno* g, const double* d_v, const double* d_vbar, AbsSums ab, int64_t* d_acc,
+                           cudaStream_t s) {
+    if (sweep_tmem_enabled(g)) { sweep_tmem_accumulate(g, d_v, d_vbar, ab, d_acc, s); return; }
+    if (sweep_uses_tern(g)) launch_lut<true, false, true>(g, d_v, nullptr, d_vbar, nullptr, ab, d_acc, s);
+    else if (g->quad) launch_lut<true, false>(g, d_v, nullptr, d_vbar, nullptr, ab, d_acc, s);
+    else launch_lut<false, false>(g, d_v, nullptr, d_vbar, nullptr, ab, d_acc, s);
+}
+
+void sweep_pair_accumulate(const ihtb_geno* g, const double* d_v0, const double* d_v1, const double* d_vbar,
+                           const float* d_scale, const double* d_abs, int64_t* d_acc, cudaStream_t s) {
     IHTB_CHECK(g->cs_j == 128, IHTB_EUNSUPPORTED, "the pair sweep needs a tiled layout");
-    if (sweep_tmem_enabled(g)) { sweep_tmem_pair_partials(g, d_v0, d_v1, d_vbar, d_scale, d_part, s); return; }
-    if (sweep_uses_tern(g)) launch_lut<true, true, true>(g, d_v0, d_v1, d_vbar, d_scale, d_part, s);
-    else if (g->quad) launch_lut<true, true>(g, d_v0, d_v1, d_vbar, d_scale, d_part, s);
-    else launch_lut<false, true>(g, d_v0, d_v1, d_vbar, d_scale, d_part, s);
-}
-
-}
+    if (sweep_tmem_enabled(g)) { sweep_tmem_pair_accumulate(g, d_v0, d_v1, d_vbar, d_scale, d_abs, d_acc, s); return; }
+    AbsSums ab;
+    ab.abs = d_abs;
+    if (sweep_uses_tern(g)) launch_lut<true, true, true>(g, d_v0, d_v1, d_vbar, d_scale, ab, d_acc, s);
+    else if (g->quad) launch_lut<true, true>(g, d_v0, d_v1, d_vbar, d_scale, ab, d_acc, s);
+    else launch_lut<false, true>(g, d_v0, d_v1, d_vbar, d_scale, ab, d_acc, s);
+}
+
+}
diff --git a/mendeliht.jl_b200/csrc/sweep_tmem.cu b/mendeliht.jl_b200/csrc/sweep_tmem.cu
--- a/mendeliht.jl_b200/csrc/sweep_tmem.cu
+++ b/mendeliht.jl_b200/csrc/sweep_tmem.cu
@@ -57,7 +57,7 @@
 __global__ void __launch_bounds__(TM_THREADS, 1)
 k_sweep_tmem(const uint8_t* __restrict__ bed, int64_t cs_s, int64_t p4, int64_t p_out, int64_t n, int64_t n_slabs,
              const double* __restrict__ v, const double* __restrict__ v1, const double* __restrict__ vbar_p,
-             const float* __restrict__ scale_p, float* __restrict__ part, uint32_t dyn_bytes) {
+             const float* __restrict__ scale_p, AbsSums ab, int64_t* __restrict__ tot, uint32_t dyn_bytes) {
     const double vbar = vbar_p[0];
     const double vbar1 = H2 ? vbar_p[1] : 0.0;
     const float sc0 = H2 ? scale_p[0] : 1.0f, sc1 = H2 ? scale_p[1] : 1.0f;
@@ -144,6 +144,8 @@
             const int col = 64 * j + 16 * (a_idx >> 2) + 4 * g + (a_idx & 3);
             const bool writer = (lane & (LPC - 1)) == 0;
             const uint32_t tlane = tbase + ((uint32_t)(32 * g) << 16) + (uint32_t)(16 * j);
+            const int rhs = H2 ? vidx >> 4 : 0;
+            const double qs = pow2(62 - acc_exp(acc_bound(ab, rhs)));
             int ts = 0; uint32_t tph = 0;
             int64_t slab = slab_beg, cb = u_beg - slab_beg * ncb;
             bool need_build = true;
@@ -202,7 +204,7 @@
 #pragma unroll
                 for (int oo = 16 / NACC; oo >= 1; oo >>= 1) acc[0] += __shfl_xor_sync(0xffffffffu, acc[0], oo);
                 const int64_t jj = cb * TM_UNIT_COLS + col;
-                if (writer && jj < p_out) part[((int64_t)(H2 ? vidx >> 4 : 0) * n_slabs + slab) * p_out + jj] = acc[0];
+                if (writer && jj < p_out) acc_add(tot + (int64_t)rhs * p_out + jj, acc[0], qs);
                 if (++ts == TM_SLOTS) { ts = 0; tph ^= 1u; }
                 if (++cb == ncb) { cb = 0; ++slab; need_build = true; }
             }
@@ -219,7 +221,7 @@
 
 template <bool H2>
 static void launch_tmem(const ihtb_geno* g, const double* d_v, const double* d_v1, const double* d_vbar,
-                        const float* d_scale, float* d_part, cudaStream_t s) {
+                        const float* d_scale, AbsSums ab, int64_t* d_acc, cudaStream_t s) {
     ensure_dynamic_smem(k_sweep_tmem<H2>, TM_SMEM_BYTES);
     const int64_t n_slabs = g->stride / 128;
     const int64_t units = n_slabs * ceil_div(g->p4, TM_UNIT_COLS);
@@ -227,19 +229,22 @@
     if (units < grid) grid = (int)units;
     IHTB_CHECK(g->p < (int64_t(1) << 31) - 256, IHTB_EDIM, "more than 2^31 SNP columns on one GPU");
     IHTB_LAUNCH((k_sweep_tmem<H2>), grid, TM_THREADS, TM_SMEM_BYTES, s, g->bed.p, g->cs_s, g->p4, g->p, g->n, n_slabs,
-                d_v, d_v1, d_vbar, d_scale, d_part, (uint32_t)TM_SMEM_BYTES);
+                d_v, d_v1, d_vbar, d_scale, ab, d_acc, (uint32_t)TM_SMEM_BYTES);
 }
 
 bool sweep_tmem_enabled(const ihtb_geno* g) {
     const char* e = getenv("IHTB_SWEEP_TMEM");
     return g->quad && e && *e == '1';
 }
-void sweep_tmem_partials(const ihtb_geno* g, const double* d_v, const double* d_vbar, float* d_part, cudaStream_t s) {
-    launch_tmem<false>(g, d_v, nullptr, d_vbar, nullptr, d_part, s);
-}
-void sweep_tmem_pair_partials(const ihtb_geno* g, const double* d_v0, const double* d_v1, const double* d_vbar,
-                              const float* d_scale, float* d_part, cudaStream_t s) {
-    launch_tmem<true>(g, d_v0, d_v1, d_vbar, d_scale, d_part, s);
-}
-
-}
+void sweep_tmem_accumulate(const ihtb_geno* g, const double* d_v, const double* d_vbar, AbsSums ab, int64_t* d_acc,
+                           cudaStream_t s) {
+    launch_tmem<false>(g, d_v, nullptr, d_vbar, nullptr, ab, d_acc, s);
+}
+void sweep_tmem_pair_accumulate(const ihtb_geno* g, const double* d_v0, const double* d_v1, const double* d_vbar,
+                                const float* d_scale, const double* d_abs, int64_t* d_acc, cudaStream_t s) {
+    AbsSums ab;
+    ab.abs = d_abs;
+    launch_tmem<true>(g, d_v0, d_v1, d_vbar, d_scale, ab, d_acc, s);
+}
+
+}
```

Result: faster. 944.4 (median of 6 runs) (+1.9%).
